# ktncktnc/diffusion-forcing-transformer

Hardware: AMD Instinct MI355X
Metric: denoised latent frames/sec, DFoT RE10K 8f & 200f rollout @1/2/4/8 GPU (higher is better)
Workload: dtype bf16

## Files before the change

diffusion-forcing-transformer_amd/backbone.py:

```python
from __future__ import annotations

import ctypes as C
import math
from typing import Dict, Optional, Sequence, Tuple

import torch
from torch import nn

from . import capi, ops


def _get(cfg, key, default=None):
    if isinstance(cfg, dict):
        return cfg.get(key, default)
    return getattr(cfg, key, default) if not hasattr(cfg, "get") else cfg.get(key, default)


class _Node(nn.Module):
    """Anonymous container so that dotted reference key names map onto a module tree."""


class UViT3DPose(nn.Module):
    def __init__(self, cfg, x_shape: Sequence[int], max_tokens: int, external_cond_dim: int = 0,
                 external_cond_type: str = "action", external_cond_num_classes: Optional[int] = None,
                 use_causal_mask: bool = False, **kwargs):
        super().__init__()
        block_types = list(_get(cfg, "block_types", ["ResBlock", "ResBlock", "TransformerBlock", "TransformerBlock"]))
        if block_types != ["ResBlock", "ResBlock", "TransformerBlock", "TransformerBlock"]:
            raise ValueError(f"unsupported block_types {block_types}")
        if _get(cfg, "pos_emb_type", "rope") != "rope":
            raise ValueError("only pos_emb_type='rope' is supported")
        if not _get(cfg, "use_fourier_noise_embedding", True):
            raise ValueError("only the Fourier noise-level embedding (continuous diffusion) is supported")
        cond = _get(cfg, "conditioning", None)
        cond_dim = _get(cond, "dim", None) if cond is not None else None
        self.cfg = cfg
        self.x_shape = tuple(x_shape)
        self.max_tokens = self.temporal_length = int(max_tokens)
        self.external_cond_dim = int(cond_dim or 180)
        self.use_causal_mask = use_causal_mask
        c = capi.UViTConfig()
        c.channels[:] = list(_get(cfg, "channels"))
        c.emb_channels = int(_get(cfg, "emb_channels"))
        c.num_updown_blocks[:] = list(_get(cfg, "num_updown_blocks"))
        c.num_mid_blocks = int(_get(cfg, "num_mid_blocks"))
        c.num_heads = int(_get(cfg, "num_heads"))
        c.in_channels = int(self.x_shape[0])
        c.resolution = int(self.x_shape[-1])
        c.max_tokens = self.max_tokens
        c.cond_dim = self.external_cond_dim
        c.noise_dim = 256
        c.rope_theta = 10000.0
        c.eps = 1e-6
        if int(_get(cfg, "patch_size", 2)) != 2:
            raise ValueError("only patch_size=2 is supported")
        self._ccfg = c
        self._handle = C.c_void_p()
        capi.check(capi.lib.dfot_uvit_create(C.byref(c), C.byref(self._handle)))
        self._names = []
        self._persistent_buffers = {"noise_level_pos_embedding.timesteps.freqs",
                                    "noise_level_pos_embedding.timesteps.phases"}
        shape = (C.c_int64 * 4)()
        ndim = C.c_int()
        for i in range(capi.lib.dfot_uvit_num_params(self._handle)):
            name = capi.lib.dfot_uvit_param_name(self._handle, i).decode()
            capi.check(capi.lib.dfot_uvit_param_shape(self._handle, i, shape, C.byref(ndim)))
            self._register(name, tuple(shape[k] for k in range(ndim.value)))
            self._names.append(name)
        self._synced: Optional[Tuple] = None
        self._reserved = 0
        self._op_key: Optional[int] = None
        self._cond_key = None
        self._cond_refs = None
        self._cond_gen = None
        self._cond_flag = None
        self.cond_cache_stats = {"builds": 0, "identity_hits": 0, "content_hits": 0}
        self._train_names = None
        self._trainer = None
        self._trainer_sig = None
        self.live_frames = None
        self.fresh_frames = None
        self._fresh_key = None
        self._train_stamp = 0
        self._dropout_generator: Optional[torch.Generator] = None

    def _register(self, name: str, shape: Tuple[int, ...]) -> None:
        *path, leaf = name.split(".")
        node: nn.Module = self
        for part in path:
            if part not in node._modules:
                node.add_module(part, _Node())
            node = node._modules[part]
        t = torch.zeros(shape, dtype=torch.float32)
        if name in self._persistent_buffers:
            node.register_buffer(leaf, t, persistent=True)
        else:
            node.register_parameter(leaf, nn.Parameter(t))

    def _tensors(self) -> Dict[str, torch.Tensor]:
        sd = dict(self.named_parameters())
        sd.update(dict(self.named_buffers()))
        return sd

    def reset_parameters(self, seed: int = 0) -> None:
        g = torch.Generator().manual_seed(seed)
        with torch.no_grad():
            for name, t in self._tensors().items():
                leaf = name.rsplit(".", 1)[-1]
                if leaf == "freqs":
                    t.copy_(2 * math.pi * torch.randn(t.shape, generator=g))
                elif leaf == "phases":
                    t.copy_(2 * math.pi * torch.rand(t.shape, generator=g))
                elif any(s in name for s in (".attn_out.", ".mlp_out.2.", ".out_rest.1.", "project_output")):
                    t.zero_()
                elif leaf == "bias":
                    t.zero_()
                elif t.ndim == 1:
                    t.fill_(1.0)
                else:
                    fan_in = math.prod(t.shape[1:])
                    bound = 1.0 / math.sqrt(fan_in)
                    t.copy_((torch.rand(t.shape, generator=g) * 2 - 1) * bound)

    def _signature(self) -> Tuple:
        return tuple((t.data_ptr(), t._version) for t in self._tensors().values())

    def sync_weights(self, force: bool = False) -> None:
        sig = self._signature()
        if not force and sig == self._synced:
            return
        tensors = self._tensors()
        s = capi.stream_ptr()
        for name in self._names:
            t = tensors[name]
            if not t.is_cuda:
                raise RuntimeError(f"parameter {name} is on {t.device}; move the module to the GPU first")
            src = t.detach().to(torch.float32).contiguous()
            shape = (C.c_int64 * src.ndim)(*src.shape)
            capi.check(capi.lib.dfot_uvit_load_weight(self._handle, name.encode(), capi.ptr(src), shape, src.ndim, s))
        capi.check(capi.lib.dfot_uvit_finalize(self._handle, s))
        self._synced = sig
        self.reserve_generation = getattr(self, "reserve_generation", 0) + 1

    def set_option(self, key: str, value: int) -> None:
        self.reserve_generation = getattr(self, "reserve_generation", 0) + 1
        capi.check(capi.lib.dfot_uvit_set_option(self._handle, key.encode(), int(value)))

    def query(self, key: str) -> float:
        self.sync_weights()
        val = C.c_double()
        capi.check(capi.lib.dfot_uvit_query(self._handle, key.encode(), C.byref(val)))
        return float(val.value)

    def attn_timing(self):
        tot, n = C.c_double(), C.c_int64()
        capi.check(capi.lib.dfot_uvit_attn_timing(self._handle, C.byref(tot), C.byref(n)))
        return tot.value, n.value

    def init_random(self, seed: int = 0, zero_init_scale: float = 0.3) -> None:
        g = torch.Generator().manual_seed(seed)
        with torch.no_grad():
            for name, t in self._tensors().items():
                leaf = name.rsplit(".", 1)[-1]
                if leaf == "freqs":
                    v = 2 * math.pi * torch.randn(t.shape, generator=g)
                elif leaf == "phases":
                    v = 2 * math.pi * torch.rand(t.shape, generator=g)
                elif leaf == "bias":
                    v = 0.02 * torch.randn(t.shape, generator=g)
                elif t.ndim == 1:
                    v = 1.0 + 0.1 * torch.randn(t.shape, generator=g)
                else:
                    fan_in = t.shape[0] if name.startswith("project_output") else math.prod(t.shape[1:])
                    v = torch.randn(t.shape, generator=g) / math.sqrt(fan_in)
                    if any(s in name for s in (".attn_out.", ".mlp_out.2.", ".out_rest.1.", "project_output")):
                        v = v * zero_init_scale
                t.copy_(v.to(t.device))

    def reserve(self, batch: int) -> None:
        if batch > self._reserved:
            torch.cuda.synchronize()
            capi.check(capi.lib.dfot_uvit_reserve(self._handle, int(batch)))
            self._reserved = batch
            self.reserve_generation = getattr(self, "reserve_generation", 0) + 1
            self._cond_key = None

    def forward(self, x: torch.Tensor, noise_levels: torch.Tensor, external_cond: Optional[torch.Tensor] = None,
                external_cond_mask: Optional[torch.Tensor] = None) -> torch.Tensor:
        assert external_cond is not None, "External condition (camera pose) is required for U-ViT3DPose model."
        if self._op_key is None:
            self._op_key = ops.register_model(self)
        if torch.is_grad_enabled() and (x.requires_grad or any(p.requires_grad for p in self.parameters())):
            if self._train_names is None:
                self._train_names = [n for n, _ in self.named_parameters()]
            params = [p for _, p in self.named_parameters()]
            return torch.ops.dfot.uvit3d_pose_forward_train(x, noise_levels, external_cond, external_cond_mask, params, self._op_key)
        return torch.ops.dfot.uvit3d_pose_forward(x, noise_levels, external_cond, external_cond_mask, self._op_key)

    def _train_engine(self, params):
        from . import uvit_train
        sig = tuple((t.data_ptr(), t._version) for t in params) + tuple((b.data_ptr(), b._version) for _, b in self.named_buffers())
        if self._trainer is None:
            cfg = dict(channels=list(self._ccfg.channels), emb_channels=int(self._ccfg.emb_channels), patch_size=2,
                       block_types=["ResBlock", "ResBlock", "TransformerBlock", "TransformerBlock"],
                       num_updown_blocks=list(self._ccfg.num_updown_blocks), num_mid_blocks=int(self._ccfg.num_mid_blocks),
                       num_heads=int(self._ccfg.num_heads), in_channels=int(self._ccfg.in_channels), resolution=int(self._ccfg.resolution),
                       max_tokens=self.max_tokens, cond_dim=self.external_cond_dim, noise_dim=int(self._ccfg.noise_dim),
                       eps=float(self._ccfg.eps), rope_theta=float(self._ccfg.rope_theta),
                       block_dropouts=list(_get(self.cfg, "block_dropouts", [0.0] * 4) or [0.0] * 4))
            sd = {n: t for n, t in zip(self._train_names, params)}
            sd.update(dict(self.named_buffers()))
            ordered = {n: sd[n] for n in self._names}
            self._trainer = uvit_train.UViT3DPoseTrainer(ordered, cfg)
            self._trainer_sig = sig
        elif sig != self._trainer_sig:
            with torch.no_grad():
                for n, t in zip(self._train_names, params):
                    self._trainer.p[n].copy_(t)
                for n, b in self.named_buffers():
                    self._trainer.p[n].copy_(b)
            self._trainer.sync()
            self._trainer_sig = sig
        return self._trainer

    def _train_forward_impl(self, x, noise_levels, external_cond, external_cond_mask, params):
        assert x.shape[1] == self.temporal_length, (
            f"Temporal length of U-ViT is set to {self.temporal_length}, but input has temporal length {x.shape[1]}.")
        dev = params[0].device
        if dev.type != "cuda":
            raise RuntimeError(f"the backbone's parameters are on {dev}; move the module to the GPU first (there is no CPU path)")
        capi.require_device(dev, x=x, noise_levels=noise_levels, external_cond=external_cond, external_cond_mask=external_cond_mask)
        eng = self._train_engine(params)
        drop = external_cond_mask
        pdrop = float(_get(self.cfg, "external_cond_dropout", 0.0) or 0.0)
        if drop is None and self.training and pdrop > 0:
            drop = torch.rand(x.shape[0], device=dev) < pdrop
        eng.dropout_generator = self._dropout_generator if self.training else None
        self._train_stamp += 1
        with torch.no_grad():
            return eng.forward(x, noise_levels, external_cond, drop).to(x.dtype)

    def _train_backward_impl(self, grad_out, params, stamp=None, want_dx=False):
        eng = self._trainer
        if eng is None:
            raise RuntimeError("backward without a training forward")
        if stamp is not None and stamp != self._train_stamp:
            raise RuntimeError(
                f"UViT3DPose: backward of training forward #{stamp}, but forward #{self._train_stamp} has run since and overwritten the "
                "saved activations (one engine per module). Run backward after each forward (accumulate gradients as forward/backward "
                "pairs); two forwards of one module inside one loss are not supported.")
        with torch.no_grad():
            grads = eng.backward(grad_out, input_grad=want_dx)
        out = [grads[n].to(p.dtype).reshape(p.shape) if n in grads else torch.zeros_like(p) for n, p in zip(self._train_names, params)]
        if want_dx:
            out.append(eng.dx_in.to(grad_out.dtype))
        return out

    def _cond_content_equal(self, cond: torch.Tensor, mask: Optional[torch.Tensor]) -> bool:
        if self._cond_key is None or self._cond_refs is None:
            return False
        kept, kept_mask = self._cond_refs
        _, version, shape, synced, mask_key = self._cond_key
        if synced != self._synced or self._cond_gen != self.reserve_generation:
            return False
        if kept._version != version or (kept_mask is not None and kept_mask._version != mask_key[1]):
            return False
        for t in (cond, kept):
            if t.dtype != torch.float32 or not t.is_contiguous():
                return False
        if cond.device != kept.device or tuple(cond.shape) != shape:
            return False
        if (mask is None) != (kept_mask is None):
            return False
        if mask is not None and (mask.dtype != kept_mask.dtype or mask.shape != kept_mask.shape or mask.device != kept_mask.device
                                 or not mask.is_contiguous() or not kept_mask.is_contiguous()):
            return False
        if torch.cuda.is_current_stream_capturing():
            return False
        if self._cond_flag is None or self._cond_flag.device != cond.device:
            self._cond_flag = torch.zeros(1, dtype=torch.int32, device=cond.device)
        flag = self._cond_flag
        flag.zero_()
        s = capi.stream_ptr()
        capi.check(capi.lib.dfot_op_equal_bits(capi.ptr(kept), capi.ptr(cond), cond.numel() * cond.element_size(), capi.ptr(flag), s))
        if mask is not None:
            capi.check(capi.lib.dfot_op_equal_bits(capi.ptr(kept_mask), capi.ptr(mask), mask.numel() * mask.element_size(), capi.ptr(flag), s))
        return int(flag.item()) == 0

    def _forward_impl(self, x: torch.Tensor, noise_levels: torch.Tensor, external_cond: Optional[torch.Tensor] = None,
                      external_cond_mask: Optional[torch.Tensor] = None) -> torch.Tensor:
        assert x.shape[1] == self.temporal_length, (
            f"Temporal length of U-ViT is set to {self.temporal_length}, but input has temporal length {x.shape[1]}.")
        assert external_cond is not None, "External condition (camera pose) is required for U-ViT3DPose model."
        b = x.shape[0]
        if tuple(x.shape[2:]) != self.x_shape:
            raise ValueError(f"x has frame shape {tuple(x.shape[2:])}, expected {self.x_shape}")
        if tuple(external_cond.shape) != (b, self.temporal_length, self.external_cond_dim, *self.x_shape[1:]):
            raise ValueError(f"external_cond has shape {tuple(external_cond.shape)}")
        if external_cond_mask is not None:
            assert external_cond_mask.ndim == 1, "embedding mask should be of shape (B,)"
        if tuple(noise_levels.shape) != (b, self.temporal_length):
            raise ValueError(f"noise_levels has shape {tuple(noise_levels.shape)}, expected {(b, self.temporal_length)}")
        dev = next(self.parameters()).device
        if dev.type != "cuda":
            raise RuntimeError(f"the backbone's parameters are on {dev}; move the module to the GPU first (there is no CPU path)")
        capi.require_device(dev, x=x, noise_levels=noise_levels, external_cond=external_cond, external_cond_mask=external_cond_mask)
        self.sync_weights()
        self.reserve(b)
        xf = x.detach().to(torch.float32).contiguous()
        kf = noise_levels.detach().to(torch.float32).contiguous()
        key = (external_cond.data_ptr(), external_cond._version, tuple(external_cond.shape), self._synced,
               None if external_cond_mask is None else (external_cond_mask.data_ptr(), external_cond_mask._version))
        if key == self._cond_key:
            self.cond_cache_stats["identity_hits"] += 1
        else:
            if self._cond_content_equal(external_cond, external_cond_mask):
                self.cond_cache_stats["content_hits"] += 1
            else:
                cf = external_cond.detach().to(torch.float32).contiguous()
                mf = None if external_cond_mask is None else external_cond_mask.to(torch.uint8).contiguous()
                capi.check(capi.lib.dfot_uvit_set_conditions(self._handle, capi.ptr(cf, torch.float32, "external_cond"),
                                                             capi.ptr(mf, torch.uint8, "external_cond_mask"), b, capi.stream_ptr()))
                self.cond_cache_stats["builds"] += 1
            self._cond_key = key
            self._cond_refs = (external_cond, external_cond_mask)
            self._cond_gen = self.reserve_generation
        out = torch.empty_like(xf)
        live = self.live_frames
        if live is not None:
            if tuple(live.shape) != (b, self.temporal_length) or live.dtype != torch.uint8 or not live.is_contiguous():
                raise ValueError(f"live_frames must be a contiguous uint8 tensor of shape {(b, self.temporal_length)}")
            capi.require_device(dev, live_frames=live)
        fresh = self.fresh_frames
        if fresh is not None:
            if tuple(fresh.shape) != (b, self.temporal_length) or fresh.dtype != torch.uint8 or not fresh.is_contiguous():
                raise ValueError(f"fresh_frames must be a contiguous uint8 tensor of shape {(b, self.temporal_length)}")
            capi.require_device(dev, fresh_frames=fresh)
            if key != self._fresh_key:
                fresh = None
        capi.check(capi.lib.dfot_uvit_forward_cached_masks(self._handle, capi.ptr(xf, torch.float32, "x"),
                                                           capi.ptr(kf, torch.float32, "noise_levels"), capi.ptr(out), b,
                                                           capi.ptr(live, torch.uint8, "live_frames"),
                                                           capi.ptr(fresh, torch.uint8, "fresh_frames"), capi.stream_ptr()))
        self._fresh_key = key
        return out.to(x.dtype)

    def read_tap(self, name: str, channels: int, level: int, batch: int) -> torch.Tensor:
        r = self.x_shape[-1] // 2 // (2 ** level)
        out = torch.empty(batch * self.temporal_length, channels, r, r, device="cuda", dtype=torch.float32)
        capi.check(capi.lib.dfot_uvit_read_tap(self._handle, name.encode(), capi.ptr(out), out.numel(), capi.stream_ptr()))
        return out

    def __del__(self):
        try:
            if getattr(self, "_handle", None) and self._handle.value:
                capi.lib.dfot_uvit_destroy(self._handle)
                self._handle = C.c_void_p()
        except Exception:
            pass
```

diffusion-forcing-transformer_amd/capi.py:

```python
from __future__ import annotations

import ctypes as C
import os

_HERE = os.path.dirname(os.path.abspath(__file__))
LIB_PATH = os.environ.get("DFOT_LIB", os.path.join(_HERE, "libdfot_hip.so"))

OK, ERR_ARG, ERR_SHAPE, ERR_HIP, ERR_STATE, ERR_NAME = range(6)


class DfotError(RuntimeError):
    def __init__(self, code: int, message: str):
        super().__init__(f"libdfot_hip error {code}: {message}")
        self.code = code


class UViTConfig(C.Structure):
    _fields_ = [
        ("channels", C.c_int32 * 4), ("emb_channels", C.c_int32), ("num_updown_blocks", C.c_int32 * 3),
        ("num_mid_blocks", C.c_int32), ("num_heads", C.c_int32), ("in_channels", C.c_int32),
        ("resolution", C.c_int32), ("max_tokens", C.c_int32), ("cond_dim", C.c_int32), ("noise_dim", C.c_int32),
        ("rope_theta", C.c_float), ("eps", C.c_float),
    ]


class DiTConfig(C.Structure):
    _fields_ = [
        ("hidden_size", C.c_int32), ("depth", C.c_int32), ("num_heads", C.c_int32), ("patch_size", C.c_int32),
        ("in_channels", C.c_int32), ("height", C.c_int32), ("width", C.c_int32), ("max_tokens", C.c_int32),
        ("mlp_hidden", C.c_int32), ("noise_dim", C.c_int32), ("timesteps", C.c_int32),
        ("rope_theta", C.c_float), ("eps", C.c_float),
        ("variant", C.c_int32), ("embed_col_dim", C.c_int32), ("num_col_heads", C.c_int32), ("num_row_heads", C.c_int32),
        ("temporal_mlp_hidden", C.c_int32), ("use_bias", C.c_int32),
        ("cond_type", C.c_int32), ("cond_dim", C.c_int32), ("num_classes", C.c_int32), ("cond_dropout", C.c_int32),
        ("use_temporal_rope", C.c_int32),
    ]


class DiTConfigF(DiTConfig):
    _fields_ = [("fourier_noise", C.c_int32)]


COND_NONE, COND_ACTION, COND_LABEL = 0, 1, 2


_P, _I, _L, _F = C.c_void_p, C.c_int, C.c_int64, C.c_float
_I32 = C.c_int32


class GemmDesc(C.Structure):
    _fields_ = [
        ("amode", _I32), ("epi", _I32), ("variant", _I32),
        ("A", _P), ("lda", _L), ("W", _P), ("ldw", _L),
        ("M", _I32), ("N", _I32), ("K", _I32), ("H", _I32), ("Wd", _I32), ("Cin", _I32),
        ("live", _P), ("bias", _P), ("bias_rows", _I32),
        ("out_f32", _P), ("out_bf16", _P), ("ldo", _L),
        ("resid", _P), ("resid_bf", _P),
        ("gate", _P), ("gate_index", _P), ("ldg", _L), ("gate_rows", _I32),
        ("act", _I32), ("pre_act", _P), ("raw", _P), ("ldraw", _L), ("tr_rows", _I32),
        ("gn_part", _P), ("gn_rows_per_bt", _I32), ("gn_cpg", _I32),
        ("out2", _P), ("ldo2", _L), ("split", _I32),
        ("q", _P), ("k", _P), ("v", _P),
        ("qw", _P), ("kw", _P), ("rope_cs", _P),
        ("heads", _I32), ("d", _I32), ("ntok", _I32), ("qscale", _F), ("dstride", _I32), ("eps", _F),
        ("ksplit", _I32), ("slice_stride", _L),
    ]


SIGNATURES = {
    "dfot_last_error": (C.c_char_p, []),
    "dfot_version": (_I, []),
    "dfot_uvit_create": (_I, [C.POINTER(UViTConfig), C.POINTER(_P)]),
    "dfot_uvit_destroy": (_I, [_P]),
    "dfot_uvit_num_params": (_I, [_P]),
    "dfot_uvit_param_name": (C.c_char_p, [_P, _I]),
    "dfot_uvit_param_shape": (_I, [_P, _I, C.POINTER(_L), C.POINTER(_I)]),
    "dfot_uvit_load_weight": (_I, [_P, C.c_char_p, _P, C.POINTER(_L), _I, _P]),
    "dfot_uvit_finalize": (_I, [_P, _P]),
    "dfot_uvit_reserve": (_I, [_P, _I]),
    "dfot_uvit_workspace_bytes": (C.c_size_t, [_P]),
    "dfot_uvit_set_option": (_I, [_P, C.c_char_p, _I]),
    "dfot_uvit_query": (_I, [_P, C.c_char_p, C.POINTER(C.c_double)]),
    "dfot_uvit_attn_timing": (_I, [_P, C.POINTER(C.c_double), C.POINTER(_L)]),
    "dfot_uvit_forward": (_I, [_P, _P, _P, _P, _P, _P, _I, _P]),
    "dfot_uvit_set_conditions": (_I, [_P, _P, _P, _I, _P]),
    "dfot_uvit_forward_cached": (_I, [_P, _P, _P, _P, _I, _P]),
    "dfot_uvit_forward_cached_live": (_I, [_P, _P, _P, _P, _I, _P, _P]),
    "dfot_uvit_forward_cached_masks": (_I, [_P, _P, _P, _P, _I, _P, _P, _P]),
    "dfot_uvit_read_tap": (_I, [_P, C.c_char_p, _P, C.c_size_t, _P]),
    "dfot_dit_create": (_I, [C.POINTER(DiTConfig), C.POINTER(_P)]),
    "dfot_dit_create_f": (_I, [C.POINTER(DiTConfigF), C.POINTER(_P)]),
    "dfot_dit_destroy": (_I, [_P]),
    "dfot_dit_num_params": (_I, [_P]),
    "dfot_dit_param_name": (C.c_char_p, [_P, _I]),
    "dfot_dit_param_shape": (_I, [_P, _I, C.POINTER(_L), C.POINTER(_I)]),
    "dfot_dit_load_weight": (_I, [_P, C.c_char_p, _P, C.POINTER(_L), _I, _P]),
    "dfot_dit_finalize": (_I, [_P, _P]),
    "dfot_dit_reserve": (_I, [_P, _I]),
    "dfot_dit_workspace_bytes": (C.c_size_t, [_P]),
    "dfot_dit_set_option": (_I, [_P, C.c_char_p, _I]),
    "dfot_dit_attn_timing": (_I, [_P, C.POINTER(C.c_double), C.POINTER(_L)]),
    "dfot_dit_forward": (_I, [_P, _P, _P, _P, _I, _I, _P]),
    "dfot_dit_forward_cond": (_I, [_P, _P, _P, _P, _P, _P, _P, _I, _I, _P]),
    "dfot_dit_forward_f": (_I, [_P, _P, _P, _P, _P, _P, _P, _I, _I, _P]),
    "dfot_dit_read_tap": (_I, [_P, C.c_char_p, _P, C.c_size_t, _P]),
    "dfot_dit_train_create": (_I, [C.POINTER(DiTConfig), C.POINTER(_P)]),
    "dfot_dit_train_create_f": (_I, [C.POINTER(DiTConfigF), C.POINTER(_P)]),
    "dfot_dit_train_destroy": (_I, [_P]),
    "dfot_dit_train_num_params": (_I, [_P]),
    "dfot_dit_train_param_name": (C.c_char_p, [_P, _I]),
    "dfot_dit_train_param_shape": (_I, [_P, _I, C.POINTER(_L), C.POINTER(_I)]),
    "dfot_dit_train_param_offset": (_L, [_P, _I]),
    "dfot_dit_train_total_numel": (_L, [_P]),
    "dfot_dit_train_workspace_bytes": (C.c_size_t, [_P]),
    "dfot_dit_train_attach": (_I, [_P, _P, _P]),
    "dfot_dit_train_reserve": (_I, [_P, _I]),
    "dfot_dit_train_sync_weights": (_I, [_P, _P]),
    "dfot_dit_train_forward": (_I, [_P, _P, _P, _P, _I, _I, _P]),
    "dfot_dit_train_forward_cond": (_I, [_P, _P, _P, _P, _P, _P, _P, _I, _I, _P]),
    "dfot_dit_train_load_buffer": (_I, [_P, C.c_char_p, _P, _L, _P]),
    "dfot_dit_train_forward_f": (_I, [_P, _P, _P, _P, _P, _P, _P, _I, _I, _P]),
    "dfot_dit_train_input_grad": (_I, [_P, _P, _P]),
    "dfot_dit_train_backward": (_I, [_P, _P, _P]),
    "dfot_vloss_grad": (_I, [_P] * 7 + [_I, _I, _L, _I, _P]),
    "dfot_sumsq": (_I, [_P, _L, _P, _P]),
    "dfot_adamw_step": (_I, [_P, _P, _P, _P, _L, _F, _F, _F, _F, _F, _I, _P, _F, _P, _F, _P]),
    "dfot_ray_encode": (_I, [_P, _P, _I, _I, _I, _P]),
    "dfot_ray_encode_normalized": (_I, [_P, _P, _I, _I, _I, _P]),
    "dfot_hg_prepare": (_I, [_P, _P, _P, _P, _P, _I, _I, _I, _L, _P]),
    "dfot_ddim_compose": (_I, [_P] * 11 + [_I, _I, _I, _L, _P]),
    "dfot_ddim_compose_tokw": (_I, [_P] * 11 + [_I, _I, _I, _L, _P]),
    "dfot_ddim_noise": (_I, [_P] * 5 + [_I, _I, _I, _L, _I, _P]),
    "dfot_vpred_loss": (_I, [_P] * 9 + [_I, _I, _L, _P]),
    "dfot_vpred_loss_scratch_floats": (_L, [_I, _I, _L]),
    "dfot_vspace_loss": (_I, [_P] * 9 + [_I, _I, _L, _P]),
    "dfot_op_gemm": (_I, [_P, _I, _P, _P, _P, _I, _I, _I, _I, _P]),
    "dfot_op_conv3x3": (_I, [_P, _P, _P, _P, _I, _I, _I, _I, _I, _I, _P]),
    "dfot_op_gemm_ex": (_I, [C.POINTER(GemmDesc), _P]),
    "dfot_op_gemm_desc_bytes": (_L, []),
    "dfot_op_attention": (_I, [_P, _P, _P, _P, _I, _I, _I, _I, _I, _I, _P]),
    "dfot_op_attention_padded": (_I, [_P, _P, _P, _P, _I, _I, _I, _I, _I, _P]),
    "dfot_op_attention_temporal": (_I, [_P, _P, _P, _P, _I, _I, _I, _I, _I, _I, _P]),
    "dfot_op_matrix_attention_rope": (_I, [_P, _P, _P, _I, _I, _I, _I, _I, _I, _F, _P]),
    "dfot_op_matrix_attention": (_I, [_P, _P, _I, _I, _I, _I, _I, _I, _F, _P]),
    "dfot_op_attention_bwd": (_I, [_P, _P, _P, _P, _P, _I, _P, _P, _P, _I, _I, _I, _I, _P]),
    "dfot_op_conv3x3_bwd": (_I, [_P, _P, _P, _P, _P, _P, _I, _I, _I, _I, _I, _P]),
    "dfot_op_conv3x3_bwd2": (_I, [_P, _P, _P, _P, _P, _P, _P, _I, _I, _I, _I, _I, _P]),
    "dfot_op_gn_silu_bwd": (_I, [_P, _P, _P, _P, _P, _F, _P, _P, _P, _P, _I, _I, _I, _P]),
    "dfot_op_rms_film_bwd": (_I, [_P, _P, _P, _P, _F, _P, _P, _P, _L, _I, _I, _P]),
    "dfot_op_rms_film_bwd_res": (_I, [_P, _P, _P, _P, _F, _P, _P, _P, _P, _P, _L, _I, _P]),
    "dfot_op_qknorm_rope_bwd": (_I, [_P, _I, _P, _P, _P, _P, _P, _P, _F, _P, _I, _P, _P, _L, _I, _I, _I, _P]),
    "dfot_op_wgrad_nt": (_I, [_P, _I, _P, _I, _P, _I, _I, _L, _I, _P]),
    "dfot_op_gemm_bf16": (_I, [_P, _I, _P, _P, _P, _I, _I, _I, _I, _P]),
    "dfot_op_gemm_f32": (_I, [_P, _I, _P, _P, _P, _P, _I, _I, _I, _I, _P]),
    "dfot_op_transpose_bf16": (_I, [_P, _P, _I, _I, _P]),
    "dfot_op_colsum_bf16": (_I, [_P, _I, _P, _L, _I, _P]),
    "dfot_op_rms_film_fwd": (_I, [_P, _P, _P, _F, _P, _L, _I, _P]),
    "dfot_op_qknorm_rope_fwd": (_I, [_P, _I, _P, _P, _P, _F, _F, _P, _P, _P, _L, _I, _I, _I, _P]),
    "dfot_op_fused_proj_train": (_I, [_P, _I, _P, _P, _P, _P, _P, _F, _F, _P, _P, _P, _P, _P, _I, _I, _L, _I, _I, _I, _P]),
    "dfot_op_silu_cols": (_I, [_P, _I, _I, _P, _I, _I, _P, _I, _I, _L, _I, _P]),
    "dfot_op_attention_fwd_lse": (_I, [_P, _P, _P, _P, _I, _P, _I, _I, _I, _I, _P]),
    "dfot_op_attention_fwd_lse_bounded": (_I, [_P, _P, _P, _P, _I, _P, _I, _I, _I, _I, C.c_float, _P, C.c_size_t, _P]),
    "dfot_op_attention_scratch_bytes": (C.c_size_t, [_I, _I, _I, _I]),
    "dfot_op_attention_bwd_lse": (_I, [_P, _P, _P, _P, _P, _I, _P, _P, _P, _P, _P, _I, _I, _I, _I, _P]),
    "dfot_op_gn_silu_fwd": (_I, [_P, _P, _P, _P, _F, _P, _P, _I, _I, _I, _P]),
    "dfot_op_gn_silu_bwd5": (_I, [_P, _P, _P, _P, _P, _P, _P, _P, _P, _P, _L, _P, _P, _I, _I, _I, _P]),
    "dfot_op_gn_silu_fwd2": (_I, [_P, _P, _P, _P, _L, _F, _P, _P, _I, _I, _I, _P]),
    "dfot_op_gn_silu_bwd6": (_I, [_P, _P, _P, _P, _P, _P, _L, _P, _P, _P, _P, _L, _P, _P, _I, _I, _I, _P]),
    "dfot_op_gemm_bf16_frame_bias": (_I, [_P, _I, _P, _P, _I, _P, _I, _I, _I, _I, _P]),
    "dfot_op_split_bf16": (_I, [_P, _P, _P, _L, _P]),
    "dfot_op_frame_sums_bf16": (_I, [_P, _L, _P, _I, _I, _I, _P]),
    "dfot_op_sgemm": (_I, [_P, _L, _L, _P, _L, _L, _P, _L, _I, _I, _I, _I, _P]),
    "dfot_op_pack_conv3": (_I, [_P, _P, _I, _I, _I, _P]),
    "dfot_op_conv3x3_f32": (_I, [_P, _P, _P, _P, _P, _I, _I, _I, _I, _I, _P]),
    "dfot_op_pool2_bf16": (_I, [_P, _P, _I, _I, _I, _I, _P]),
    "dfot_op_pool2_bwd": (_I, [_P, _P, _I, _I, _I, _I, _P]),
    "dfot_op_sub_bf16": (_I, [_P, _P, _P, _L, _P]),
    "dfot_op_upsample_add": (_I, [_P, _P, _P, _I, _I, _I, _I, _P]),
    "dfot_op_upsample_bwd": (_I, [_P, _P, _I, _I, _I, _I, _P]),
    "dfot_op_axpy": (_I, [_P, _P, _F, _L, _P]),
    "dfot_op_mul_cols": (_I, [_P, _I, _I, _P, _L, _I, _P]),
    "dfot_op_emb_pyramid": (_I, [_P, _P, _P, _P, _I, _I, _I, _P]),
    "dfot_op_cond_repack": (_I, [_P, _P, _I, _I, _I, _I, _P]),
    "dfot_op_embed_input": (_I, [_P, _P, _P, _P, _I, _I, _I, _I, _P]),
    "dfot_op_embed_input_wgrad": (_I, [_P, _P, _P, _P, _I, _I, _I, _I, _I, _P]),
    "dfot_op_embed_input_dgrad": (_I, [_P, _P, _P, _I, _I, _I, _I, _I, _P]),
    "dfot_op_project_output": (_I, [_P, _P, _P, _P, _I, _I, _I, _I, _P]),
    "dfot_op_outgrad_gather": (_I, [_P, _P, _I, _I, _I, _I, _P]),
    "dfot_op_groupnorm_scratch_floats": (_L, [_I, _I]),
    "dfot_op_groupnorm": (_I, [_P, _P, _P, _F, _P, _P, _I, _I, _I, _I, _P]),
    "dfot_op_frame_shift": (_I, [_P, _P, _I, _I, _L, _I, _P]),
    "dfot_op_upsample3d": (_I, [_P, _P, _I, _I, _I, _I, _I, _I, _P]),
    "dfot_op_softmax_rows": (_I, [_P, _P, _L, _I, _F, _P]),
    "dfot_op_conv3t_f32": (_I, [_P, _P, _P, _P, _P] + [_I] * 9 + [_P]),
    "dfot_op_vae_pixels": (_I, [_P, _L, _L, _L, _L, _L, _F, _F, _P, _I, _I, _I, _I, _P]),
    "dfot_op_vae_posterior": (_I, [_P, _I, _P, _P, _P, _P, _P, _P, _P, _I, _I, _I, _I, _P]),
    "dfot_op_ivae_attention": (_I, [_P, _P, _P, _P, _I, _I, _I, _P]),
    "dfot_op_conv3x3_s2_f32": (_I, [_P, _P, _P, _P] + [_I] * 5 + [_P]),
    "dfot_op_upconv3x3_f32": (_I, [_P, _P, _P, _P] + [_I] * 5 + [_P]),
    "dfot_op_f32_to_bf16": (_I, [_P, _P, _L, _P]),
    "dfot_op_bf16_to_f32": (_I, [_P, _P, _L, _P]),
    "dfot_op_equal_bits": (_I, [_P, _P, _L, _P, _P]),
}


def _load() -> C.CDLL:
    import torch
    if not os.path.exists(LIB_PATH):
        raise ImportError(
            f"{LIB_PATH} is missing: the HIP extension has not been built. There is no CPU fallback; "
            "run `python -c 'import __graft_entry__ as g; g.build()'` (needs hipcc).")
    lib = C.CDLL(LIB_PATH)
    for name, (res, args) in SIGNATURES.items():
        fn = getattr(lib, name)
        fn.restype, fn.argtypes = res, args
    return lib


lib = _load()


def check(code: int) -> None:
    if code != OK:
        raise DfotError(code, (lib.dfot_last_error() or b"").decode())


def ptr(t, dtype=None, name: str = "tensor") -> C.c_void_p:
    if t is None:
        return C.c_void_p(0)
    if not t.is_cuda:
        raise ValueError(f"{name} is on {t.device}: libdfot_hip takes GPU memory only (there is no CPU path)")
    if not t.is_contiguous():
        raise ValueError(f"{name} with shape {tuple(t.shape)} and strides {tuple(t.stride())} is not contiguous")
    if dtype is not None and t.dtype != dtype:
        raise ValueError(f"{name} has dtype {t.dtype}, expected {dtype}")
    return C.c_void_p(t.data_ptr())


def ptr_rows(t, dtype=None, name: str = "tensor") -> C.c_void_p:
    if t is None:
        return C.c_void_p(0)
# ... 19 lines not shown
```

diffusion-forcing-transformer_amd/csrc/common.h:

```cpp
#pragma once
#include <hip/hip_runtime.h>
#include <stdint.h>
#include <stdio.h>

#include "dfot_hip.h"

namespace dfot {

typedef __bf16 bf16;
typedef __attribute__((ext_vector_type(8))) __bf16 bf16x8;
typedef __attribute__((ext_vector_type(4))) __bf16 bf16x4;
typedef __attribute__((ext_vector_type(2))) __bf16 bf16x2;
typedef __attribute__((ext_vector_type(4))) float f32x4;
typedef __attribute__((ext_vector_type(16))) float f32x16;
typedef __attribute__((ext_vector_type(2))) unsigned u32x2;

#define DFOT_LDS_PTR(p) ((void __attribute__((address_space(3)))*)(p))
#define DFOT_GLOBAL_PTR(p) ((const void __attribute__((address_space(1)))*)(p))

__device__ __forceinline__ int xcd_remap(int orig, int nwg, int enable = 1) {
  if (!enable) return orig;
  const int q = nwg >> 3, r = nwg & 7, xcd = orig & 7;
  return (xcd < r ? xcd * (q + 1) : r * (q + 1) + (xcd - r) * q) + (orig >> 3);
}

__device__ __forceinline__ float silu_f(float x) { return x * __builtin_amdgcn_rcpf(1.0f + __expf(-x)); }

__device__ __forceinline__ float bf2f(bf16 v) { return (float)v; }
__device__ __forceinline__ bf16 f2bf(float v) { return (bf16)v; }

template <int OFF>
__device__ __forceinline__ u32x2 lds_read_tr16(unsigned addr) {
  u32x2 r;
  asm volatile("ds_read_b64_tr_b16 %0, %1 offset:%2" : "=v"(r) : "v"(addr), "n"(OFF));
  return r;
}
__device__ __forceinline__ void lds_wait(u32x2& a, u32x2& b, u32x2& c, u32x2& d, u32x2& e, u32x2& f, u32x2& g, u32x2& h) {
  asm volatile("s_waitcnt lgkmcnt(0)" : "+v"(a), "+v"(b), "+v"(c), "+v"(d), "+v"(e), "+v"(f), "+v"(g), "+v"(h));
}
__device__ __forceinline__ bf16x8 as_bf16x8(u32x2 lo, u32x2 hi) {
  typedef __attribute__((ext_vector_type(4))) unsigned u32x4;
  const u32x4 v = {lo[0], lo[1], hi[0], hi[1]};
  return __builtin_bit_cast(bf16x8, v);
}

int tuning_flag(const char* name, int dflt);

void set_error(const char* fmt, ...);
const char* get_error();

#define DFOT_CHECK_HIP(expr)                                                              \
  do {                                                                                    \
    hipError_t _e = (expr);                                                               \
    if (_e != hipSuccess) {                                                               \
      ::dfot::set_error("%s failed: %s (%s:%d)", #expr, hipGetErrorString(_e), __FILE__, __LINE__); \
      return DFOT_ERR_HIP;                                                                \
    }                                                                                     \
  } while (0)

#define DFOT_REQUIRE(cond, code, ...)      \
  do {                                     \
    if (!(cond)) {                         \
      ::dfot::set_error(__VA_ARGS__);      \
      return code;                         \
    }                                      \
  } while (0)

static inline int cdiv(long a, long b) { return (int)((a + b - 1) / b); }

template <auto Kern>
int ensure_dyn_lds(int bytes) {
  static bool done = false;
  if (!done) {
    DFOT_CHECK_HIP(hipFuncSetAttribute(reinterpret_cast<const void*>(Kern), hipFuncAttributeMaxDynamicSharedMemorySize, bytes));
    done = true;
  }
  return DFOT_OK;
}

}
```

diffusion-forcing-transformer_amd/csrc/gemm.h:

```cpp
#pragma once
#include "common.h"

namespace dfot {

enum AMode { A_DENSE = 0, A_CONV3 = 1, A_CONV3T = 2 };
enum Epi { E_F32 = 0, E_BF16 = 1, E_QKV = 2, E_QKV_DIT = 3 };

struct GemmArgs {
  const bf16* A = nullptr;
  long lda = 0;
  const bf16* W = nullptr;
  long ldw = 0;
  int M = 0, N = 0, K = 0;
  int H = 0, Wd = 0, Cin = 0;
  const bf16* zeros = nullptr;
  const uint8_t* live = nullptr;
  int To = 0, Tin = 0, Hin = 0, Win = 0;
  int cs = 1, ct = 1, ckt = 1;
  const float* bias = nullptr;
  float* out_f32 = nullptr;
  bf16* out_bf16 = nullptr;
  long ldo = 0;
  const float* resid = nullptr;
  const bf16* resid_bf = nullptr;
  const float* gate = nullptr;
  const int* gate_index = nullptr;
  long ldg = 0;
  int gate_rows = 0;
  int act = 0;
  bf16* pre_act = nullptr;
  bf16* raw = nullptr;
  long ldraw = 0;
  int bias_rows = 0;
  int tr_rows = 0;
  float* gn_part = nullptr;
  int gn_rows_per_bt = 0;
  int gn_cpg = 0;
  bf16* out2 = nullptr;
  long ldo2 = 0;
  int split = 0;
  bf16 *q = nullptr, *k = nullptr, *v = nullptr;
  const float *qw = nullptr, *kw = nullptr, *rope_cs = nullptr;
  int heads = 0, d = 0, ntok = 0;
  float qscale = 1.f;
  int dstride = 0;
  float eps = 1e-6f;
  int xcd = 1;
  int persist = 0;
  int ksplit = 1;
  long slice_stride = 0;
};

enum GemmVariant {
  GEMM_REGS_128 = 0,
  GEMM_DMA_128 = 1,
  GEMM_DMA_256x256 = 4,
  GEMM_DMA_512x128 = 6,
  GEMM_DMA_128_KS2 = 8,
  GEMM_DMA_256x192 = 9,
  GEMM_DMA_128x192 = 10,
  GEMM_DMA3_256x144 = 14,
  GEMM_AUTO = -1
};
int gemm_pick_variant(int amode, int m, int n, int k, bool plain_f32 = false);
int launch_gemm(int amode, int epi, int variant, const GemmArgs& g, hipStream_t stream);

}
```

diffusion-forcing-transformer_amd/csrc/gemm.hip:

```cpp
#include "gemm.h"
#include "dfot_hip.h"

namespace dfot {

constexpr int BK = 64;
constexpr int wave_cols(int bn) { return bn % 64 == 0 ? 64 : 48; }
constexpr int tile_threads(int bm, int bn, int wtm, int ks) { return (bm / wtm) * (bn / wave_cols(bn)) * 64 * ks; }
constexpr int EP_LD = 68;

template <int N>
__device__ __forceinline__ void wait_all_but() {
  static_assert(N == 2 || N == 4 || N == 6 || N == 8 || N == 12, "unexpected load count");
  if constexpr (N == 2) asm volatile("s_waitcnt vmcnt(2)\n\ts_barrier" ::: "memory");
  if constexpr (N == 4) asm volatile("s_waitcnt vmcnt(4)\n\ts_barrier" ::: "memory");
  if constexpr (N == 6) asm volatile("s_waitcnt vmcnt(6)\n\ts_barrier" ::: "memory");
  if constexpr (N == 8) asm volatile("s_waitcnt vmcnt(8)\n\ts_barrier" ::: "memory");
  if constexpr (N == 12) asm volatile("s_waitcnt vmcnt(12)\n\ts_barrier" ::: "memory");
}

__device__ __forceinline__ void wait_all_but_n(int n) {
  switch (n) {
    case 1: asm volatile("s_waitcnt vmcnt(1)\n\ts_barrier" ::: "memory"); break;
    case 2: asm volatile("s_waitcnt vmcnt(2)\n\ts_barrier" ::: "memory"); break;
    case 3: asm volatile("s_waitcnt vmcnt(3)\n\ts_barrier" ::: "memory"); break;
    case 4: asm volatile("s_waitcnt vmcnt(4)\n\ts_barrier" ::: "memory"); break;
    case 5: asm volatile("s_waitcnt vmcnt(5)\n\ts_barrier" ::: "memory"); break;
    case 6: asm volatile("s_waitcnt vmcnt(6)\n\ts_barrier" ::: "memory"); break;
    case 7: asm volatile("s_waitcnt vmcnt(7)\n\ts_barrier" ::: "memory"); break;
    case 8: asm volatile("s_waitcnt vmcnt(8)\n\ts_barrier" ::: "memory"); break;
    default: asm volatile("s_waitcnt vmcnt(0)\n\ts_barrier" ::: "memory"); break;
  }
}

template <int BM_T, int BN_T, int WTM, int NST, int AMODE, int EPI, bool DMA, int KS, int BKT>
__device__ __forceinline__ void gemm_tile(const GemmArgs& g, const int tile_index, const int tile_count) {
  static_assert(BKT == 64 || (BKT == 32 && AMODE == A_DENSE && DMA && KS == 1), "K-tile depth");
  constexpr int CPR = BKT / 8;
  constexpr int RPI = 64 / CPR;
  constexpr int ROWB = BKT * 2;
  constexpr int MI = WTM / 16;
  constexpr int WTN = wave_cols(BN_T);
  constexpr int NI = WTN / 16;
  constexpr int WN = BN_T / WTN;
  static_assert(WTN == 64 || (EPI == E_F32 || EPI == E_BF16), "48-column wave tiles: plain epilogues only");
  static_assert(WTN == 64 || KS == 1, "48-column wave tiles: no intra-workgroup split-K");
  constexpr int NW = (BM_T / WTM) * WN;
  constexpr int NT = NW * 64;
  constexpr int AINS = BM_T / RPI, WINS = BN_T / RPI;
  constexpr int ACH = (AINS + NW - 1) / NW;
  constexpr int WCH = (WINS + NW - 1) / NW;
  constexpr bool A_EVEN = AINS % NW == 0, W_EVEN = WINS % NW == 0;
  static_assert((A_EVEN && W_EVEN) || (DMA && KS == 1), "uneven staging: LDS-DMA kernels without intra-workgroup split-K only");
  constexpr int A_BYTES = BM_T * BKT * 2;
  constexpr int STAGE_BYTES = (BM_T + BN_T) * BKT * 2;
  constexpr int LOADS = ACH + WCH;
  static_assert(DMA || NST == 2, "register staging supports two stages only");
  static_assert(KS == 1 || (NST == 2 && DMA && EPI != E_QKV), "split-K: two-stage LDS-DMA kernels without in-epilogue barriers");
  extern __shared__ __attribute__((aligned(16))) char smem_all[];
  const int tid = threadIdx.x, lane = tid & 63;
  const int kgroup = KS == 1 ? 0 : (tid >> 6) / NW;
  const int wave = KS == 1 ? (tid >> 6) : (tid >> 6) % NW;
  char* smem = smem_all + kgroup * (NST * STAGE_BYTES);
  const int wm = wave / WN, wn = wave % WN;
  const int tiles_n = (g.N + BN_T - 1) / BN_T;
  const int ksplit = (EPI == E_F32 && (AMODE == A_DENSE || g.slice_stride > 0) && g.ksplit > 1) ? g.ksplit : 1;
  const int kslice = ksplit > 1 ? tile_index % ksplit : 0;
  const int bid = ksplit > 1 ? xcd_remap(tile_index / ksplit, tile_count / ksplit, g.xcd) : xcd_remap(tile_index, tile_count, g.xcd);
  const int tn = bid % tiles_n, tm = bid / tiles_n;
  const int m0 = tm * BM_T, n0 = tn * BN_T;
  if constexpr (AMODE == A_CONV3) {
    if (g.live && !g.live[(unsigned)m0 / (unsigned)(g.H * g.Wd)]) return;
  }
  int nk = g.K / BKT;
  long kbeg = 0;
  if (ksplit > 1) {
    const int per = nk / ksplit, rem = nk % ksplit;
    kbeg = (long)(kslice * per + (kslice < rem ? kslice : rem)) * BKT;
    nk = per + (kslice < rem ? 1 : 0);
  }
  auto swz = [](int r) { return BKT == 64 ? ((r >> 1) & 7) : ((r >> 2) & 2); };

  const int prow = lane / CPR;
  const int ppos = lane % CPR;
  const bf16* a_src[ACH];
  int a_y[ACH], a_x[ACH];
  [[maybe_unused]] int a_t[ACH];
  const bf16* w_src[WCH];
  int a_chunk[ACH];
#pragma unroll
  for (int i = 0; i < ACH; ++i) {
    const int r = RPI * (NW * i + wave) + prow;
    const int c = ppos ^ swz(r);
    a_chunk[i] = c;
    const long m = (long)m0 + r;
    if constexpr (AMODE == A_DENSE) {
      a_src[i] = g.A + m * g.lda + c * 8 + kbeg;
      a_y[i] = a_x[i] = 0;
    } else if constexpr (AMODE == A_CONV3) {
      const unsigned mu = (unsigned)m;
      const int xw = (int)(mu % (unsigned)g.Wd);
      const int yh = (int)((mu / (unsigned)g.Wd) % (unsigned)g.H);
      a_x[i] = xw;
      a_y[i] = yh;
      a_src[i] = g.A + m * (long)g.Cin + c * 8;
    } else {
      unsigned mu = (unsigned)m;
      const int xo = (int)(mu % (unsigned)g.Wd);
      mu /= (unsigned)g.Wd;
      const int yo = (int)(mu % (unsigned)g.H);
      mu /= (unsigned)g.H;
      const int to = (int)(mu % (unsigned)g.To);
      const unsigned bv = mu / (unsigned)g.To;
      const int pad = g.cs == 1 ? 1 : 0;
      a_x[i] = g.cs * xo - pad;
      a_y[i] = g.cs * yo - pad;
      a_t[i] = g.ct * to - (g.ckt - 1);
      a_src[i] = g.A + (long)bv * ((long)g.Tin * g.Hin * g.Win * g.Cin) + c * 8;
    }
  }
#pragma unroll
  for (int i = 0; i < WCH; ++i) {
    const int r = RPI * (NW * i + wave) + prow;
    const int c = ppos ^ swz(r);
    int n = n0 + r;
    n = n < g.N ? n : g.N - 1;
    w_src[i] = g.W + (long)n * (AMODE == A_DENSE && g.ldw ? g.ldw : (long)g.K) + c * 8 + kbeg;
  }

  [[maybe_unused]] int cv_c0 = 0, cv_dy = -1, cv_dx = -1, cv_dt = 0;
  if constexpr (AMODE == A_CONV3) {
    const int kbase = kgroup * BKT + (int)kbeg;
    const int tap = kbase / g.Cin;
    cv_c0 = kbase - tap * g.Cin;
    cv_dy = tap / 3 - 1;
    cv_dx = tap % 3 - 1;
  } else if constexpr (AMODE == A_CONV3T) {
    const int kbase = kgroup * BKT + (int)kbeg;
    const int tap = kbase / g.Cin;
    cv_c0 = kbase - tap * g.Cin;
    cv_dt = tap / 9;
    cv_dy = (tap % 9) / 3;
    cv_dx = tap % 3;
  }
  auto a_addr = [&](int i, int kt) -> const bf16* {
    if constexpr (AMODE == A_DENSE) {
      return a_src[i] + (long)kt * BKT;
    } else if constexpr (AMODE == A_CONV3) {
      const int yy = a_y[i] + cv_dy, xx = a_x[i] + cv_dx;
      const bool ok = (yy >= 0) && (yy < g.H) && (xx >= 0) && (xx < g.Wd);
      const bf16* p = a_src[i] + ((long)cv_dy * g.Wd + cv_dx) * g.Cin + cv_c0;
      return ok ? p : g.zeros + a_chunk[i] * 8;
    } else {
      int tt = a_t[i] + cv_dt;
      tt = tt < 0 ? 0 : tt;
      const int yy = a_y[i] + cv_dy, xx = a_x[i] + cv_dx;
      const bool ok = (yy >= 0) && (yy < g.Hin) && (xx >= 0) && (xx < g.Win);
      const bf16* p = a_src[i] + ((long)(tt * g.Hin + yy) * g.Win + xx) * g.Cin + cv_c0;
      return ok ? p : g.zeros + a_chunk[i] * 8;
    }
  };
  auto conv_advance = [&]() {
    if constexpr (AMODE == A_CONV3) {
      cv_c0 += KS * BKT;
      while (cv_c0 >= g.Cin) {
        cv_c0 -= g.Cin;
        if (++cv_dx > 1) {
          cv_dx = -1;
          ++cv_dy;
        }
      }
    } else if constexpr (AMODE == A_CONV3T) {
      cv_c0 += KS * BKT;
      while (cv_c0 >= g.Cin) {
        cv_c0 -= g.Cin;
        if (++cv_dx > 2) {
          cv_dx = 0;
          if (++cv_dy > 2) {
            cv_dy = 0;
            ++cv_dt;
          }
        }
      }
    }
  };

  bf16x8 ra[ACH], rw[WCH];

  auto issue = [&](int kt, int stage) {
    char* sa = smem + stage * STAGE_BYTES;
    char* sw = sa + A_BYTES;
#pragma unroll
    for (int i = 0; i < ACH; ++i) {
      if (!A_EVEN && NW * i + wave >= AINS) continue;
      const bf16* pa = a_addr(i, kt);
      if constexpr (DMA) {
        __builtin_amdgcn_global_load_lds(DFOT_GLOBAL_PTR(pa), DFOT_LDS_PTR(sa + (NW * i + wave) * 1024), 16, 0, 0);
      } else {
        ra[i] = *reinterpret_cast<const bf16x8*>(pa);
      }
    }
#pragma unroll
    for (int i = 0; i < WCH; ++i) {
      if (!W_EVEN && NW * i + wave >= WINS) continue;
      const bf16* pw = w_src[i] + (long)kt * BKT;
      if constexpr (DMA) {
        __builtin_amdgcn_global_load_lds(DFOT_GLOBAL_PTR(pw), DFOT_LDS_PTR(sw + (NW * i + wave) * 1024), 16, 0, 0);
      } else {
        rw[i] = *reinterpret_cast<const bf16x8*>(pw);
      }
    }
    conv_advance();
  };
  auto commit = [&](int stage) {
    char* sa = smem + stage * STAGE_BYTES;
    char* sw = sa + A_BYTES;
#pragma unroll
    for (int i = 0; i < ACH; ++i) *reinterpret_cast<bf16x8*>(sa + (NW * i + wave) * 1024 + lane * 16) = ra[i];
#pragma unroll
    for (int i = 0; i < WCH; ++i) *reinterpret_cast<bf16x8*>(sw + (NW * i + wave) * 1024 + lane * 16) = rw[i];
  };
// ... 486 lines not shown
      if constexpr (EPI == E_F32) {
        if (g.gn_cpg == 8) {
          gsum += __shfl_xor(gsum, 1);
          gsq += __shfl_xor(gsq, 1);
        }
        gsum += __shfl_xor(gsum, 16);
        gsq += __shfl_xor(gsq, 16);
        gsum += __shfl_xor(gsum, 32);
        gsq += __shfl_xor(gsq, 32);
        if (lane < 16 && live && (g.gn_cpg == 4 || (lane & 1) == 0)) {
          const int grp = col / g.gn_cpg;
          dst[grp * 2] = gsum;
          dst[grp * 2 + 1] = gsq;
        }
      } else {
        if (g.gn_cpg == 8) {
          gsum += gsum2;
          gsq += gsq2;
        }
#pragma unroll
        for (int o = 8; o < 64; o <<= 1) {
          gsum += __shfl_xor(gsum, o);
          gsq += __shfl_xor(gsq, o);
          gsum2 += __shfl_xor(gsum2, o);
          gsq2 += __shfl_xor(gsq2, o);
        }
        if (lane < 8 && live) {
          const int grp = col / g.gn_cpg;
          dst[grp * 2] = gsum;
          dst[grp * 2 + 1] = gsq;
          if (g.gn_cpg == 4) {
            dst[grp * 2 + 2] = gsum2;
            dst[grp * 2 + 3] = gsq2;
          }
        }
      }
    }
  }
}

template <int BM_T, int BN_T, int WTM, int NST, int AMODE, int EPI, bool DMA, int KS = 1, int BKT = BK>
__global__ __launch_bounds__(tile_threads(BM_T, BN_T, WTM, KS)) void gemm_kernel(GemmArgs g) {
  gemm_tile<BM_T, BN_T, WTM, NST, AMODE, EPI, DMA, KS, BKT>(g, blockIdx.x, gridDim.x);
}

template <int BM_T, int BN_T, int WTM, int NST, int AMODE, int EPI, bool DMA, int KS = 1, int BKT = BK>
__global__ __launch_bounds__(tile_threads(BM_T, BN_T, WTM, KS)) void gemm_kernel_persistent(GemmArgs g, int tile_count) {
  for (int tile = blockIdx.x; tile < tile_count; tile += gridDim.x) {
    gemm_tile<BM_T, BN_T, WTM, NST, AMODE, EPI, DMA, KS, BKT>(g, tile, tile_count);
    if (tile + (int)gridDim.x < tile_count) __syncthreads();
  }
}

template <int BM_T, int BN_T, int WTM, int NST, int AMODE, int EPI, bool DMA, int KS = 1, int BKT = BK>
static int launch_t(const GemmArgs& g, hipStream_t stream) {
  constexpr int nthreads = tile_threads(BM_T, BN_T, WTM, KS);
  constexpr int stage_lds = KS * NST * (BM_T + BN_T) * BKT * 2;
  constexpr int ep_lds = (nthreads / 64) * 16 * EP_LD * 4 + 2 * (nthreads / 64) * 16 * 4 +
                         (KS == 2 ? (nthreads / 128) * (WTM / 16) * 16 * 64 * 4 : 0);
  constexpr int lds = stage_lds > ep_lds ? stage_lds : ep_lds;
  const int ksplit = (EPI == E_F32 && (AMODE == A_DENSE || g.slice_stride > 0) && g.ksplit > 1) ? g.ksplit : 1;
  const int tiles = (g.M / BM_T) * ((g.N + BN_T - 1) / BN_T) * ksplit;
  GemmArgs ga = g;
  ga.xcd = 1;
  ga.persist = 1;
  constexpr bool kPersistOK = KS == 1 && nthreads <= 768;
  if constexpr (kPersistOK) {
    if (ga.persist > 0 && ksplit == 1) {
      const int resident = 256 * (lds <= 80 * 1024 ? 2 : 1);
      if (tiles > resident) {
        auto kp = gemm_kernel_persistent<BM_T, BN_T, WTM, NST, AMODE, EPI, DMA, KS, BKT>;
        static bool pattr_set = false;
        if (!pattr_set) {
          DFOT_CHECK_HIP(hipFuncSetAttribute(reinterpret_cast<const void*>(kp), hipFuncAttributeMaxDynamicSharedMemorySize, lds));
          pattr_set = true;
        }
        hipLaunchKernelGGL(kp, dim3(resident), dim3(nthreads), lds, stream, ga, tiles);
        DFOT_CHECK_HIP(hipGetLastError());
        return DFOT_OK;
      }
    }
  }
  auto kern = gemm_kernel<BM_T, BN_T, WTM, NST, AMODE, EPI, DMA, KS, BKT>;
  static bool attr_set = false;
  if (!attr_set) {
    DFOT_CHECK_HIP(hipFuncSetAttribute(reinterpret_cast<const void*>(kern), hipFuncAttributeMaxDynamicSharedMemorySize, lds));
    attr_set = true;
  }
  hipLaunchKernelGGL(kern, dim3(tiles), dim3(nthreads), lds, stream, ga);
  DFOT_CHECK_HIP(hipGetLastError());
  return DFOT_OK;
}

template <int AMODE, int EPI>
static int launch_v(int variant, const GemmArgs& g, hipStream_t s) {
  switch (variant) {
    case GEMM_REGS_128:
      if constexpr (AMODE == A_CONV3T) break;
      else return launch_t<128, 128, 64, 2, AMODE, EPI, false>(g, s);
    case GEMM_DMA_128: return launch_t<128, 128, 64, 2, AMODE, EPI, true>(g, s);
    case GEMM_DMA_256x256: return launch_t<256, 256, 64, 2, AMODE, EPI, true>(g, s);
    case GEMM_DMA_512x128: return launch_t<512, 128, 64, 2, AMODE, EPI, true>(g, s);
    case GEMM_DMA_256x192:
      if constexpr (AMODE != A_DENSE) break;
      else return launch_t<256, 192, 64, 2, AMODE, EPI, true>(g, s);
    case GEMM_DMA3_256x144:
      if constexpr ((EPI != E_F32 && !(EPI == E_BF16 && AMODE == A_DENSE)) || AMODE == A_CONV3T) break;
      else {
        if (g.gn_part) break;
        return launch_t<256, 144, 64, 3, AMODE, EPI, true>(g, s);
      }
    case GEMM_DMA_128x192:
      if constexpr (AMODE != A_DENSE || EPI == E_QKV) break;
      else return launch_t<128, 192, 64, 2, AMODE, EPI, true>(g, s);
    case GEMM_DMA_128_KS2:
      if constexpr (EPI == E_QKV) break;
      else return launch_t<128, 128, 64, 2, AMODE, EPI, true, 2>(g, s);
  }
  set_error("gemm: unknown variant %d", variant);
  return DFOT_ERR_ARG;
}

int gemm_pick_variant(int amode, int m, int n, int k, bool plain_f32) {
  const long tiles = (long)(m / 256) * ((n + 255) / 256);
  if (m % 256 == 0 && n >= 192 && amode == A_DENSE) {
    auto util = [&](int bn) {
      const long t = (long)(m / 256) * ((n + bn - 1) / bn);
      return (double)m * n / ((double)((t + 255) / 256) * 256 * 256 * bn);
    };
    if (plain_f32 && n % 144 == 0 && k >= 2304 && (long)(m / 256) * (n / 144) >= 256 && util(144) > 1.1 * util(192) && util(144) > 1.1 * util(256))
      return GEMM_DMA3_256x144;
    if (util(192) > 1.05 * util(256) && (long)(m / 256) * ((n + 191) / 192) >= 160) return GEMM_DMA_256x192;
  }
  if (m % 256 == 0 && n >= 192 && tiles >= 160) return GEMM_DMA_256x256;
  if (m % 512 == 0 && n <= 128 && m / 512 >= 256) return GEMM_DMA_512x128;
  const long tiles128 = (long)(m / 128) * ((n + 127) / 128);
  if (tiles128 <= 256 && k >= 2048) return GEMM_DMA_128_KS2;
  return GEMM_DMA_128;
}

int launch_gemm(int amode, int epi, int variant, const GemmArgs& g, hipStream_t stream) {
  DFOT_REQUIRE(g.A && g.W, DFOT_ERR_ARG, "gemm: null operand");
  if (variant == GEMM_AUTO) variant = gemm_pick_variant(amode, g.M, g.N, g.K, epi == E_F32 && !g.gn_part);
  if (variant == GEMM_DMA_128_KS2 && epi == E_QKV) variant = GEMM_DMA_128;
  if (variant == GEMM_DMA_128x192 && epi == E_QKV) variant = GEMM_DMA_128;
  if (variant == GEMM_DMA_256x192 && epi == E_QKV && g.d != 64) variant = GEMM_DMA_256x256;
  const int bm = variant == GEMM_DMA_512x128 ? 512 : (variant == GEMM_DMA_256x256 || variant == GEMM_DMA_256x192 || variant == GEMM_DMA3_256x144) ? 256 : 128;
  DFOT_REQUIRE(g.M > 0 && g.M % bm == 0, DFOT_ERR_SHAPE, "gemm: M=%d must be a positive multiple of %d", g.M, bm);
  DFOT_REQUIRE(g.K > 0 && g.K % BK == 0, DFOT_ERR_SHAPE, "gemm: K=%d must be a positive multiple of %d", g.K, BK);
  DFOT_REQUIRE(g.N > 0 && g.N % (epi == E_F32 ? 4 : 8) == 0, DFOT_ERR_SHAPE, "gemm: N=%d must be a multiple of %d", g.N, epi == E_F32 ? 4 : 8);
  DFOT_REQUIRE((epi == E_QKV || epi == E_QKV_DIT || g.ldo % (epi == E_F32 ? 4 : 8) == 0) && (epi != E_QKV || (g.ldo2 % 8 == 0 && g.split % 64 == 0)),
               DFOT_ERR_SHAPE, "gemm: output row strides must be multiples of %d", epi == E_F32 ? 4 : 8);
  DFOT_REQUIRE(g.ldw == 0 || (amode == A_DENSE && g.ldw >= g.K && g.ldw % 8 == 0), DFOT_ERR_SHAPE, "gemm: ldw=%ld must be >= K and a multiple of 8 (dense A only)", g.ldw);
  if (amode == A_CONV3) {
    DFOT_REQUIRE(g.Cin % BK == 0 && g.K == 9 * g.Cin, DFOT_ERR_SHAPE, "conv3x3: Cin=%d must be a multiple of %d", g.Cin, BK);
    DFOT_REQUIRE(g.zeros != nullptr, DFOT_ERR_ARG, "conv3x3: zero page missing");
    DFOT_REQUIRE(g.H > 0 && g.Wd > 0 && g.M % (g.H * g.Wd) == 0, DFOT_ERR_SHAPE, "conv3x3: M=%d not a whole number of %dx%d images", g.M, g.H, g.Wd);
    DFOT_REQUIRE(!g.live || (g.H * g.Wd) % bm == 0, DFOT_ERR_SHAPE, "conv3x3: live-image flags need whole %d-row tiles per %dx%d image", bm, g.H, g.Wd);
  }
  if (amode == A_CONV3T) {
    DFOT_REQUIRE(epi == E_F32 && g.ksplit <= 1 && !g.live && !g.gate && !g.bias_rows, DFOT_ERR_ARG, "conv3t: plain fp32 epilogue only");
    DFOT_REQUIRE(g.Cin % BK == 0 && (g.ckt == 1 || g.ckt == 3) && g.K == g.ckt * 9 * g.Cin && (g.cs == 1 || g.cs == 2) && (g.ct == 1 || g.ct == 2),
                 DFOT_ERR_SHAPE, "conv3t: Cin=%d (multiple of %d), kt=%d in {1,3}, K=%d = kt*9*Cin, strides s=%d t=%d in {1,2}", g.Cin, BK, g.ckt, g.K,
                 g.cs, g.ct);
    DFOT_REQUIRE(g.zeros != nullptr, DFOT_ERR_ARG, "conv3t: zero page missing");
    DFOT_REQUIRE(g.H > 0 && g.Wd > 0 && g.To > 0 && g.Hin == g.cs * g.H && g.Win == g.cs * g.Wd && g.Tin >= 1 && g.ct * (g.To - 1) <= g.Tin - 1 &&
                     g.To == (g.Tin - 1) / g.ct + 1,
                 DFOT_ERR_SHAPE, "conv3t: input %dx%dx%d, output %dx%dx%d do not match strides s=%d t=%d", g.Tin, g.Hin, g.Win, g.To, g.H, g.Wd, g.cs, g.ct);
    DFOT_REQUIRE(g.M % (g.To * g.H * g.Wd) == 0, DFOT_ERR_SHAPE, "conv3t: M=%d not a whole number of %dx%dx%d videos", g.M, g.To, g.H, g.Wd);
    DFOT_REQUIRE((long)g.Tin * g.Hin * g.Win * g.Cin < (1L << 31), DFOT_ERR_SHAPE, "conv3t: one input video must hold < 2^31 elements");
  }
  if (epi == E_QKV) {
    DFOT_REQUIRE(g.q && g.k && g.v && g.qw && g.kw && g.rope_cs && (g.out2 || g.N == g.split), DFOT_ERR_ARG, "qkv epilogue: null pointer");
    DFOT_REQUIRE(!g.raw || (g.ldraw >= g.N && g.ldraw % 8 == 0), DFOT_ERR_SHAPE, "qkv epilogue: raw copy needs ldraw >= N, a multiple of 8");
    DFOT_REQUIRE((g.d == 64 || g.d == 128) && g.heads > 0 && g.split == 3 * g.heads * g.d && g.ntok > 0 && g.M % g.ntok == 0,
                 DFOT_ERR_SHAPE, "qkv epilogue: heads=%d d=%d split=%d ntok=%d M=%d", g.heads, g.d, g.split, g.ntok, g.M);
  }
  if (epi == E_QKV_DIT) {
    DFOT_REQUIRE(g.q && g.k && g.v, DFOT_ERR_ARG, "dit qkv epilogue: null pointer");
    DFOT_REQUIRE(g.d > 0 && g.d % 8 == 0 && g.dstride >= g.d && g.dstride % 8 == 0 && g.heads > 0 && g.N == 3 * g.heads * g.d &&
                     g.ntok > 0 && g.M % g.ntok == 0,
                 DFOT_ERR_SHAPE, "dit qkv epilogue: heads=%d d=%d dstride=%d ntok=%d M=%d N=%d", g.heads, g.d, g.dstride, g.ntok, g.M, g.N);
  }
  if (g.gate) {
    DFOT_REQUIRE(epi == E_F32 && g.gate_rows > 0 && g.M % g.gate_rows == 0 && g.ldg % 4 == 0, DFOT_ERR_SHAPE,
                 "gemm: gate needs the fp32 epilogue, gate_rows dividing M and ldg %% 4 == 0");
  }
  if (g.ksplit > 1 && g.slice_stride > 0)
    DFOT_REQUIRE(!g.bias && !g.resid, DFOT_ERR_ARG, "gemm: split-K into partial outputs takes no bias / residual");
  if (g.ksplit > 1)
    DFOT_REQUIRE(epi == E_F32 && (amode == A_DENSE || g.slice_stride > 0) && !g.bias_rows && (!g.resid || g.resid == g.out_f32) && !g.gate &&
                     !g.gn_part && g.K / BK >= 2 * g.ksplit, DFOT_ERR_ARG,
                 "gemm: split-K over workgroups needs the fp32 epilogue with an in-place residual (or none), no gate, and K >= %d", 2 * g.ksplit * BK);
  if (g.bias_rows) DFOT_REQUIRE((epi == E_F32 || epi == E_BF16) && g.bias, DFOT_ERR_ARG, "gemm: 2-D bias needs a plain epilogue");
  if (g.resid_bf)
    DFOT_REQUIRE(epi == E_BF16 && (amode == A_CONV3 || variant == GEMM_DMA3_256x144) && !g.resid, DFOT_ERR_ARG,
                 "gemm: a bf16 residual needs the bf16 epilogue of a convolution or of the 256x144 ring");
  if (g.tr_rows) {
    DFOT_REQUIRE(epi == E_BF16 && !g.bias && !g.act && !g.gn_part && g.tr_rows % 4 == 0 && g.M % g.tr_rows == 0 && amode == A_DENSE,
                 DFOT_ERR_ARG, "gemm: transposed store needs the plain bf16 epilogue and tr_rows %% 4 == 0 dividing M");
  }
  if (g.gn_part) {
    DFOT_REQUIRE(epi != E_QKV && epi != E_QKV_DIT && (g.gn_cpg == 4 || g.gn_cpg == 8) && g.N == 32 * g.gn_cpg && g.gn_rows_per_bt % 64 == 0 &&
                     g.gn_rows_per_bt % bm == 0,
                 DFOT_ERR_SHAPE, "gemm: fused GroupNorm statistics need N = 32 groups of 4 or 8 channels and whole images per tile");
  }
  if (amode == A_DENSE) {
    switch (epi) {
      case E_F32: return launch_v<A_DENSE, E_F32>(variant, g, stream);
      case E_BF16: return launch_v<A_DENSE, E_BF16>(variant, g, stream);
      case E_QKV: return launch_v<A_DENSE, E_QKV>(variant, g, stream);
      case E_QKV_DIT: return launch_v<A_DENSE, E_QKV_DIT>(variant, g, stream);
    }
  } else if (amode == A_CONV3) {
    switch (epi) {
      case E_F32: return launch_v<A_CONV3, E_F32>(variant, g, stream);
      case E_BF16: return launch_v<A_CONV3, E_BF16>(variant, g, stream);
    }
  } else if (amode == A_CONV3T && epi == E_F32) {
    return launch_v<A_CONV3T, E_F32>(variant, g, stream);
  }
  set_error("gemm: unsupported mode/epilogue combination %d/%d", amode, epi);
  return DFOT_ERR_ARG;
}

}
```

diffusion-forcing-transformer_amd/csrc/uvit.hip:

```cpp
#include <algorithm>
#include <cmath>
#include <cstdarg>
#include <cstdlib>
#include <cstring>
#include <functional>
#include <map>
#include <string>
#include <vector>

#include "dfot_hip.h"
#include "gemm.h"
#include "kernels.h"

namespace dfot {

static thread_local char g_err[1024] = "";
void set_error(const char* fmt, ...) {
  va_list ap;
  va_start(ap, fmt);
  vsnprintf(g_err, sizeof(g_err), fmt, ap);
  va_end(ap);
}
const char* get_error() { return g_err; }

int tuning_flag(const char* name, int dflt) {
  std::string key = std::string("DFOT_") + name;
  const char* v = getenv(key.c_str());
  return v ? atoi(v) : dflt;
}

struct ResW {
  int c = 0;
  bf16* fcache = nullptr;
  long sv_off = 0;
  bf16 *w_film = nullptr, *w1 = nullptr, *w2 = nullptr;
  float *b_film_raw = nullptr, *b_film = nullptr, *g1 = nullptr, *be1 = nullptr, *bias1 = nullptr, *g2 = nullptr,
        *be2 = nullptr, *bias2 = nullptr;
};
struct TrW {
  int c = 0;
  bf16* fcache = nullptr;
  long sv_off = 0;
  bf16 *w_film = nullptr, *w_fused = nullptr, *w_out = nullptr;
  float *b_film_raw = nullptr, *b_film = nullptr, *nw = nullptr, *b_fused = nullptr, *qw = nullptr, *kw = nullptr,
        *b_attn = nullptr, *b_mlp = nullptr, *b_out = nullptr;
  float score_bound = INFINITY;
};
struct ConvW {
  int cin = 0, cout = 0;
  bf16* w = nullptr;
  float* b = nullptr;
};

struct Param {
  std::string name;
  std::vector<int64_t> shape;
  std::function<int(const float*, hipStream_t)> load;
  bool loaded = false;
};

}

using namespace dfot;

struct dfot_uvit_s {
  dfot_uvit_config cfg{};
  int T = 0, E = 0, heads = 0, r[4] = {0, 0, 0, 0}, ch[4] = {0, 0, 0, 0};
  int kpose = 0;
  std::vector<Param> params;
  std::map<std::string, int> index;
  std::vector<void*> owned;

  float *ne_freqs = nullptr, *ne_phases = nullptr, *ne_w1 = nullptr, *ne_b1 = nullptr, *ne_w2 = nullptr, *ne_b2 = nullptr;
  bf16* pose_w = nullptr;
  float* pose_b = nullptr;
  float *ein_w = nullptr, *ein_b = nullptr, *pout_w = nullptr, *pout_b = nullptr;
  std::vector<ResW> down_res[2], up_res[2];
  std::vector<TrW> down_tr, mid_tr, up_tr;
  ConvW down_conv[3], up_conv[3];
  int* film_map[4] = {nullptr, nullptr, nullptr, nullptr};
  float* rope_cs[4] = {nullptr, nullptr, nullptr, nullptr};
  bf16* zeros = nullptr;
  bool finalized = false;

  int max_batch = 0;
  size_t ws_bytes = 0;
  std::vector<void*> ws_owned;
  float *nemb = nullptr, *nhid = nullptr, *X[4] = {nullptr, nullptr, nullptr, nullptr}, *HSA[3] = {nullptr, nullptr, nullptr}, *tmp = nullptr,
        *gn_partial = nullptr, *gn_partial2 = nullptr, *gn_stats = nullptr, *sv = nullptr;
  int gn1_nblk = 0;
  FilmChunk* film_table = nullptr;
  int film_chunks = 0;
  uint8_t* cond_mask = nullptr;
  bool have_mask = false;
  int cond_batch = 0;
  int64_t cond_builds = 0;
  bf16 *acond = nullptr, *emb[4] = {nullptr, nullptr, nullptr, nullptr}, *s1 = nullptr, *hbf = nullptr,
       *cat = nullptr, *q = nullptr, *k = nullptr, *v = nullptr;
  AttnScratch attn_scratch;
  const float* pend_part = nullptr;
  float* out_part = nullptr;
  size_t out_part_elems = 0;
  const float* pend_bias = nullptr;
  int pend_lvl = 0, pend_c = 0, pend_slices = 2;
  long pend_m = 0;
  int last_batch = 0;
  const float* xin[4] = {nullptr, nullptr, nullptr, nullptr};
  bf16* XB[4] = {nullptr, nullptr, nullptr, nullptr};
  bool xin_bf[4] = {false, false, false, false};
  int gemm_variant = GEMM_AUTO;
  int attn_variant = 2;
  bool attn_force_safe = false;
  bool time_attn = false;
  std::vector<hipEvent_t> ev_start, ev_stop;
  size_t ev_used = 0;
};

namespace dfot {

template <typename T>
static int dev_alloc(dfot_uvit_s* h, T** out, size_t count, bool workspace = false) {
  void* p = nullptr;
  const size_t bytes = count * sizeof(T);
  DFOT_CHECK_HIP(hipMalloc(&p, bytes ? bytes : 16));
  (workspace ? h->ws_owned : h->owned).push_back(p);
  if (workspace) h->ws_bytes += bytes;
  *out = reinterpret_cast<T*>(p);
  return DFOT_OK;
}

static int copy_f32(float* dst, const float* src, size_t n, hipStream_t s) {
  DFOT_CHECK_HIP(hipMemcpyAsync(dst, src, n * sizeof(float), hipMemcpyDeviceToDevice, s));
  return DFOT_OK;
}

static void add_param(dfot_uvit_s* h, const std::string& name, std::vector<int64_t> shape,
                      std::function<int(const float*, hipStream_t)> load) {
  h->index[name] = (int)h->params.size();
  h->params.push_back(Param{name, std::move(shape), std::move(load), false});
}

static int add_f32(dfot_uvit_s* h, const std::string& name, std::vector<int64_t> shape, float** dst) {
  size_t n = 1;
  for (auto d : shape) n *= (size_t)d;
  int rc = dev_alloc(h, dst, n);
  if (rc) return rc;
  float* d = *dst;
  add_param(h, name, shape, [d, n](const float* src, hipStream_t s) { return copy_f32(d, src, n, s); });
  return DFOT_OK;
}

static int add_res_block(dfot_uvit_s* h, const std::string& pre, int c, ResW* w) {
  const int e = h->E;
  w->c = c;
  int rc = 0;
  if ((rc = dev_alloc(h, &w->w_film, (size_t)2 * c * e))) return rc;
  if ((rc = dev_alloc(h, &w->b_film_raw, (size_t)2 * c))) return rc;
  if ((rc = dev_alloc(h, &w->b_film, (size_t)2 * c))) return rc;
  if ((rc = dev_alloc(h, &w->w1, (size_t)c * 9 * c))) return rc;
  if ((rc = dev_alloc(h, &w->w2, (size_t)c * 9 * c))) return rc;
  const int lvl = c == h->ch[0] ? 0 : 1;
  int* map = h->film_map[lvl];
  bf16* wf = w->w_film;
  add_param(h, pre + ".emb_layer.weight", {2 * c, e, 1, 1}, [=](const float* src, hipStream_t s) {
    return launch_pack_rows(src, wf, map, 2 * c, e, e, e, 0, s);
  });
  float *braw = w->b_film_raw, *bre = w->b_film;
  add_param(h, pre + ".emb_layer.bias", {2 * c}, [=](const float* src, hipStream_t s) {
    int r2 = copy_f32(braw, src, 2 * c, s);
    return r2 ? r2 : launch_gather_f32(braw, bre, map, 2 * c, s);
  });
  if ((rc = add_f32(h, pre + ".in_layers.0.weight", {c}, &w->g1))) return rc;
  if ((rc = add_f32(h, pre + ".in_layers.0.bias", {c}, &w->be1))) return rc;
  bf16* w1 = w->w1;
  add_param(h, pre + ".in_layers.2.weight", {c, c, 3, 3}, [=](const float* src, hipStream_t s) { return launch_pack_conv3(src, w1, c, c, s); });
  if ((rc = add_f32(h, pre + ".in_layers.2.bias", {c}, &w->bias1))) return rc;
  if ((rc = add_f32(h, pre + ".out_norm.weight", {c}, &w->g2))) return rc;
  if ((rc = add_f32(h, pre + ".out_norm.bias", {c}, &w->be2))) return rc;
  bf16* w2 = w->w2;
  add_param(h, pre + ".out_rest.1.weight", {c, c, 3, 3}, [=](const float* src, hipStream_t s) { return launch_pack_conv3(src, w2, c, c, s); });
  if ((rc = add_f32(h, pre + ".out_rest.1.bias", {c}, &w->bias2))) return rc;
  return DFOT_OK;
}

static int add_tr_block(dfot_uvit_s* h, const std::string& pre, int lvl, TrW* w) {
  const int e = h->E, c = h->ch[lvl], d = c / h->heads;
  w->c = c;
  int rc = 0;
  if ((rc = dev_alloc(h, &w->w_film, (size_t)2 * c * e))) return rc;
  if ((rc = dev_alloc(h, &w->b_film_raw, (size_t)2 * c))) return rc;
  if ((rc = dev_alloc(h, &w->b_film, (size_t)2 * c))) return rc;
  if ((rc = dev_alloc(h, &w->w_fused, (size_t)7 * c * c))) return rc;
  if ((rc = dev_alloc(h, &w->w_out, (size_t)c * 5 * c))) return rc;
  if ((rc = dev_alloc(h, &w->b_out, (size_t)c))) return rc;
  int* map = h->film_map[lvl];
  bf16* wf = w->w_film;
  add_param(h, pre + ".norm.emb_layer.weight", {2 * c, e}, [=](const float* src, hipStream_t s) {
    return launch_pack_rows(src, wf, map, 2 * c, e, e, e, 0, s);
  });
  float *braw = w->b_film_raw, *bre = w->b_film;
  add_param(h, pre + ".norm.emb_layer.bias", {2 * c}, [=](const float* src, hipStream_t s) {
    int r2 = copy_f32(braw, src, 2 * c, s);
    return r2 ? r2 : launch_gather_f32(braw, bre, map, 2 * c, s);
  });
  if ((rc = add_f32(h, pre + ".norm.norm.weight", {c}, &w->nw))) return rc;
  bf16* wfu = w->w_fused;
  add_param(h, pre + ".fused_attn_mlp_proj.weight", {7 * c, c}, [=](const float* src, hipStream_t s) {
    return launch_pack_rows(src, wfu, nullptr, 7 * c, c, c, c, 0, s);
  });
  if ((rc = add_f32(h, pre + ".fused_attn_mlp_proj.bias", {7 * c}, &w->b_fused))) return rc;
  if ((rc = add_f32(h, pre + ".q_norm.weight", {d}, &w->qw))) return rc;
  if ((rc = add_f32(h, pre + ".k_norm.weight", {d}, &w->kw))) return rc;
  bf16* wo = w->w_out;
  add_param(h, pre + ".attn_out.weight", {c, c}, [=](const float* src, hipStream_t s) {
    return launch_pack_rows(src, wo, nullptr, c, c, c, 5 * c, 0, s);
  });
  if ((rc = add_f32(h, pre + ".attn_out.bias", {c}, &w->b_attn))) return rc;
  add_param(h, pre + ".mlp_out.2.weight", {c, 4 * c}, [=](const float* src, hipStream_t s) {
    return launch_pack_rows(src, wo, nullptr, c, 4 * c, 4 * c, 5 * c, c, s);
  });
  if ((rc = add_f32(h, pre + ".mlp_out.2.bias", {c}, &w->b_mlp))) return rc;
  return DFOT_OK;
}

static int add_conv(dfot_uvit_s* h, const std::string& pre, int cin, int cout, ConvW* w) {
  w->cin = cin;
  w->cout = cout;
  int rc = 0;
  if ((rc = dev_alloc(h, &w->w, (size_t)cout * 9 * cin))) return rc;
  bf16* dst = w->w;
  add_param(h, pre + ".weight", {cout, cin, 3, 3}, [=](const float* src, hipStream_t s) { return launch_pack_conv3(src, dst, cout, cin, s); });
  return add_f32(h, pre + ".bias", {cout}, &w->b);
}

static int build(dfot_uvit_s* h) {
  const dfot_uvit_config& c = h->cfg;
  h->T = c.max_tokens;
  h->E = c.emb_channels;
  h->heads = c.num_heads;
  for (int l = 0; l < 4; ++l) {
    h->ch[l] = c.channels[l];
    h->r[l] = c.resolution / 2 / (1 << l);
  }
  h->kpose = ((c.cond_dim * 4 + 63) / 64) * 64;
  int rc = 0;
  for (int l = 0; l < 4; ++l) {
    const int cc = h->ch[l];
    std::vector<int> m(2 * cc);
    for (int n = 0; n < 2 * cc; ++n) {
      const int g = n / 64, t = n % 64;
      m[n] = t < 32 ? 32 * g + t : cc + 32 * g + (t - 32);
    }
    if ((rc = dev_alloc(h, &h->film_map[l], (size_t)2 * cc))) return rc;
    DFOT_CHECK_HIP(hipMemcpy(h->film_map[l], m.data(), m.size() * sizeof(int), hipMemcpyHostToDevice));
  }
  if ((rc = dev_alloc(h, &h->zeros, 256))) return rc;
  DFOT_CHECK_HIP(hipMemset(h->zeros, 0, 256 * sizeof(bf16)));

  const int e = h->E, nd = c.noise_dim;
  const std::string ne = "noise_level_pos_embedding.";
  if ((rc = add_f32(h, ne + "timesteps.freqs", {nd}, &h->ne_freqs))) return rc;
  if ((rc = add_f32(h, ne + "timesteps.phases", {nd}, &h->ne_phases))) return rc;
  if ((rc = add_f32(h, ne + "embedding.linear_1.weight", {e, nd}, &h->ne_w1))) return rc;
  if ((rc = add_f32(h, ne + "embedding.linear_1.bias", {e}, &h->ne_b1))) return rc;
  if ((rc = add_f32(h, ne + "embedding.linear_2.weight", {e, e}, &h->ne_w2))) return rc;
  if ((rc = add_f32(h, ne + "embedding.linear_2.bias", {e}, &h->ne_b2))) return rc;
  if ((rc = dev_alloc(h, &h->pose_w, (size_t)e * h->kpose))) return rc;
  {
    bf16* pw = h->pose_w;
    const int k = c.cond_dim * 4, kp = h->kpose;
    add_param(h, "external_cond_embedding.patch_embedder.proj.weight", {e, c.cond_dim, 2, 2},
              [=](const float* src, hipStream_t s) { return launch_pack_rows(src, pw, nullptr, e, k, kp, kp, 0, s); });
  }
  if ((rc = add_f32(h, "external_cond_embedding.patch_embedder.proj.bias", {e}, &h->pose_b))) return rc;
  if ((rc = add_f32(h, "embed_input.proj.weight", {h->ch[0], c.in_channels, 2, 2}, &h->ein_w))) return rc;
  if ((rc = add_f32(h, "embed_input.proj.bias", {h->ch[0]}, &h->ein_b))) return rc;
  if ((rc = add_f32(h, "project_output.proj.weight", {h->ch[0], c.in_channels, 2, 2}, &h->pout_w))) return rc;
  if ((rc = add_f32(h, "project_output.proj.bias", {c.in_channels}, &h->pout_b))) return rc;

  for (int l = 0; l < 3; ++l) {
    const int n = c.num_updown_blocks[l];
    const std::string pre = "down_blocks." + std::to_string(l) + ".";
    if (l < 2) {
      h->down_res[l].resize(n);
      for (int i = 0; i < n; ++i)
        if ((rc = add_res_block(h, pre + std::to_string(i), h->ch[l], &h->down_res[l][i]))) return rc;
    } else {
      h->down_tr.resize(n);
      for (int i = 0; i < n; ++i)
        if ((rc = add_tr_block(h, pre + std::to_string(i), l, &h->down_tr[i]))) return rc;
    }
    if ((rc = add_conv(h, pre + std::to_string(n) + ".conv", h->ch[l], h->ch[l + 1], &h->down_conv[l]))) return rc;
  }
  h->mid_tr.resize(c.num_mid_blocks);
  for (int i = 0; i < c.num_mid_blocks; ++i)
    if ((rc = add_tr_block(h, "mid_blocks." + std::to_string(i), 3, &h->mid_tr[i]))) return rc;
  for (int j = 0; j < 3; ++j) {
    const int l = 2 - j;
    const int n = c.num_updown_blocks[l];
    const std::string pre = "up_blocks." + std::to_string(j) + ".";
    if ((rc = add_conv(h, pre + "0.conv", h->ch[l + 1], h->ch[l], &h->up_conv[l]))) return rc;
    if (l < 2) {
      h->up_res[l].resize(n);
      for (int i = 0; i < n; ++i)
        if ((rc = add_res_block(h, pre + std::to_string(i + 1), h->ch[l], &h->up_res[l][i]))) return rc;
    } else {
      h->up_tr.resize(n);
      for (int i = 0; i < n; ++i)
        if ((rc = add_tr_block(h, pre + std::to_string(i + 1), l, &h->up_tr[i]))) return rc;
    }
  }
  return DFOT_OK;
}

static int build_rope(dfot_uvit_s* h, int lvl) {
  const int d = h->ch[lvl] / h->heads, half = d / 2;
  const int q = half / 3, rem = half % 3;
  int parts[3] = {q, q, q};
  if (rem == 1) parts[0] = q + 1;
  if (rem == 2) parts[1] = parts[2] = q + 1;
  const int rr = h->r[lvl], n = h->T * rr * rr;
  std::vector<float> cs((size_t)n * half * 2);
  for (int tok = 0; tok < n; ++tok) {
    const int pos[3] = {tok / (rr * rr), (tok / rr) % rr, tok % rr};
    int pair = 0;
    for (int ax = 0; ax < 3; ++ax) {
      const int dim = 2 * parts[ax];
      for (int j = 0; j < parts[ax]; ++j, ++pair) {
        const float inv = 1.0f / powf(h->cfg.rope_theta, (float)(2 * j) / (float)dim);
        const float ang = (float)pos[ax] * inv;
        cs[((size_t)tok * half + pair) * 2 + 0] = cosf(ang);
        cs[((size_t)tok * half + pair) * 2 + 1] = sinf(ang);
      }
    }
  }
  int rc = dev_alloc(h, &h->rope_cs[lvl], cs.size());
  if (rc) return rc;
  DFOT_CHECK_HIP(hipMemcpy(h->rope_cs[lvl], cs.data(), cs.size() * sizeof(float), hipMemcpyHostToDevice));
  return DFOT_OK;
}

__global__ void add_vec_kernel(const float* a, const float* b, float* o, int n) {
  const int i = blockIdx.x * blockDim.x + threadIdx.x;
  if (i < n) o[i] = a[i] + b[i];
}

static int run_res_block(dfot_uvit_s* h, const ResW& w, int lvl, int bt, hipStream_t s, const uint8_t* live = nullptr) {
  const int c = w.c, rr = h->r[lvl], pix = rr * rr;
  const int m = bt * pix;
  const int slots = pix / 64;
  bf16* xb = h->XB[lvl];
  int rc = 0;
  if (!h->xin_bf[lvl]) {
    if ((rc = launch_f32_to_bf16(h->xin[lvl], xb, (long)m * c, s))) return rc;
    h->xin_bf[lvl] = true;
  }
  if (h->gn1_nblk == 0) {
    if ((rc = launch_gn_partial_bf16(xb, h->gn_partial, bt, pix, c, s))) return rc;
    h->gn1_nblk = gn_partial_blocks(pix);
  }
  if ((rc = launch_gn_finalize(h->gn_partial, h->gn_stats, bt, h->gn1_nblk, pix, c, h->cfg.eps, s))) return rc;
  h->gn1_nblk = 0;
  if ((rc = launch_gn_apply_silu_bf16in(xb, h->gn_stats, w.g1, w.be1, h->s1, bt, pix, c, s, live))) return rc;
  GemmArgs g;
  g.A = h->s1; g.W = w.w1; g.M = m; g.N = c; g.K = 9 * c; g.H = rr; g.Wd = rr; g.Cin = c; g.zeros = h->zeros;
  g.bias = w.bias1; g.out_bf16 = h->hbf; g.ldo = c; g.live = live;
  g.gn_part = h->gn_partial2; g.gn_rows_per_bt = pix; g.gn_cpg = c / 32;
  if ((rc = launch_gemm(A_CONV3, E_BF16, h->gemm_variant, g, s))) return rc;
  if ((rc = launch_gn_finalize(h->gn_partial2, h->gn_stats, bt, slots, pix, c, h->cfg.eps, s))) return rc;
  if ((rc = launch_gn_film_silu(h->hbf, h->gn_stats, w.g2, w.be2, w.fcache, h->sv + w.sv_off,
                                h->have_mask ? h->cond_mask : nullptr, h->s1, bt, pix, c, h->T, s, live)))
    return rc;
  GemmArgs o;
  o.A = h->s1; o.W = w.w2; o.M = m; o.N = c; o.K = 9 * c; o.H = rr; o.Wd = rr; o.Cin = c; o.zeros = h->zeros;
  o.bias = w.bias2; o.out_bf16 = xb; o.ldo = c; o.live = live;
  o.resid_bf = xb;
  o.gn_part = h->gn_partial; o.gn_rows_per_bt = pix; o.gn_cpg = c / 32;
  if ((rc = launch_gemm(A_CONV3, E_BF16, h->gemm_variant, o, s))) return rc;
  h->xin_bf[lvl] = true;
  h->gn1_nblk = slots;
  return DFOT_OK;
}

__global__ void out_reduce_kernel(bf16* x, const float* __restrict__ bias, const float* __restrict__ s0, const float* __restrict__ s1,
                                  const float* __restrict__ s2, long total4, int cq) {
  typedef __attribute__((ext_vector_type(4))) float f4;
  const long i = (long)blockIdx.x * blockDim.x + threadIdx.x;
  if (i >= total4) return;
  f4 b = reinterpret_cast<const f4*>(bias)[i % cq] + reinterpret_cast<const f4*>(s0)[i] + reinterpret_cast<const f4*>(s1)[i];
  if (s2) b += reinterpret_cast<const f4*>(s2)[i];
  const bf16x4 xv = reinterpret_cast<const bf16x4*>(x)[i];
  reinterpret_cast<bf16x4*>(x)[i] = bf16x4{f2bf(bf2f(xv[0]) + b[0]), f2bf(bf2f(xv[1]) + b[1]), f2bf(bf2f(xv[2]) + b[2]), f2bf(bf2f(xv[3]) + b[3])};
}
__global__ void add_f32_into_bf16_kernel(bf16* x, const float* __restrict__ y, long total4) {
  typedef __attribute__((ext_vector_type(4))) float f4;
  const long i = (long)blockIdx.x * blockDim.x + threadIdx.x;
  if (i >= total4) return;
  const f4 b = reinterpret_cast<const f4*>(y)[i];
  const bf16x4 xv = reinterpret_cast<const bf16x4*>(x)[i];
  reinterpret_cast<bf16x4*>(x)[i] = bf16x4{f2bf(bf2f(xv[0]) + b[0]), f2bf(bf2f(xv[1]) + b[1]), f2bf(bf2f(xv[2]) + b[2]), f2bf(bf2f(xv[3]) + b[3])};
}

static void swap_out_part(dfot_uvit_s* h) { h->pend_part = h->out_part; }

static int flush_pending(dfot_uvit_s* h, hipStream_t s) {
  if (!h->pend_bias) return DFOT_OK;
  const long total4 = h->pend_m * h->pend_c / 4;
  hipLaunchKernelGGL(out_reduce_kernel, dim3(cdiv(total4, 256)), dim3(256), 0, s, h->XB[h->pend_lvl], h->pend_bias, h->pend_part,
                     h->pend_part + h->pend_m * h->pend_c, h->pend_slices == 3 ? h->pend_part + 2 * h->pend_m * h->pend_c : nullptr, total4,
                     h->pend_c / 4);
  h->pend_bias = nullptr;
  DFOT_CHECK_HIP(hipGetLastError());
  return DFOT_OK;
}

static int run_tr_block(dfot_uvit_s* h, const TrW& w, int lvl, int batch, hipStream_t s) {
  const int c = w.c, rr = h->r[lvl], n = h->T * rr * rr, d = c / h->heads;
  const int m = batch * n;
  bf16* xb = h->XB[lvl];
  int rc = 0;
  if (h->pend_bias && (h->pend_lvl != lvl || h->pend_m != m || h->pend_c != c) && (rc = flush_pending(h, s))) return rc;
  if (!h->xin_bf[lvl]) {
    if ((rc = launch_f32_to_bf16(h->xin[lvl], xb, (long)m * c, s))) return rc;
    h->xin_bf[lvl] = true;
  }
  RmsPending pend{xb, h->pend_bias, h->pend_part, h->pend_part + (long)m * c, h->pend_slices == 3 ? h->pend_part + 2L * m * c : nullptr};
  if ((rc = launch_rms_film_bf16(xb, w.nw, w.fcache, h->sv + w.sv_off, h->have_mask ? h->cond_mask : nullptr, h->s1, m, c, rr * rr, h->T,
                                 h->cfg.eps, s, h->pend_bias ? &pend : nullptr)))
    return rc;
  h->pend_bias = nullptr;
  GemmArgs p;
  p.A = h->s1; p.lda = c; p.W = w.w_fused; p.M = m; p.N = 7 * c; p.K = c; p.bias = w.b_fused;
  p.out2 = h->cat + c; p.ldo2 = 5 * c; p.split = 3 * c;
  p.q = h->q; p.k = h->k; p.v = h->v; p.qw = w.qw; p.kw = w.kw; p.rope_cs = h->rope_cs[lvl]; p.heads = h->heads; p.d = d;
  p.ntok = n; p.qscale = 1.4426950408889634f / sqrtf((float)d); p.eps = h->cfg.eps;
  if ((rc = launch_gemm(A_DENSE, E_QKV, h->gemm_variant, p, s))) return rc;
  const bool timed = h->time_attn && lvl == 2 && h->ev_used < h->ev_start.size();
  if (timed) DFOT_CHECK_HIP(hipEventRecord(h->ev_start[h->ev_used], s));
  int av = h->attn_variant;
  if (av == 2 && d == 64 && n % 256 == 0) av = (attention_v5_applies(n, d, w.score_bound) && !h->attn_force_safe) ? 14 : 5;
  if ((rc = launch_attention(h->q, h->k, h->v, h->cat, 5 * c, batch, h->heads, n, d, av, s, &h->attn_scratch))) return rc;
  if (timed) DFOT_CHECK_HIP(hipEventRecord(h->ev_stop[h->ev_used++], s));
  GemmArgs o;
  o.A = h->cat; o.lda = 5 * c; o.W = w.w_out; o.M = m; o.N = c; o.K = 5 * c; o.bias = w.b_out; o.ldo = c;
  if (h->gemm_variant == GEMM_AUTO && h->out_part && (size_t)2 * m * c <= h->out_part_elems && m % 256 == 0 && c % 144 == 0 &&
      (long)(m / 256) * (c / 144) * 2 <= 256 && (5 * c / 64) >= 8) {
    GemmArgs p2 = o;
    p2.bias = nullptr; p2.out_f32 = h->out_part; p2.ksplit = 2; p2.slice_stride = (long)m * c;
    if ((rc = launch_gemm(A_DENSE, E_F32, GEMM_DMA3_256x144, p2, s))) return rc;
    h->pend_bias = w.b_out;
    h->pend_lvl = lvl; h->pend_m = m; h->pend_c = c; h->pend_slices = 2;
    swap_out_part(h);
    return DFOT_OK;
  }
  if (h->gemm_variant == GEMM_AUTO && c % 144 == 0 && m % 256 == 0 && (long)(m / 256) * ((c + 191) / 192) < 256 &&
      (long)(m / 256) * (c / 144) >= 200 && (long)(m / 256) * (c / 144) <= 256) {
    o.out_bf16 = xb;
    o.resid_bf = xb;
    return launch_gemm(A_DENSE, E_BF16, GEMM_DMA3_256x144, o, s);
  }
  o.out_f32 = h->X[lvl];
  if ((rc = launch_gemm(A_DENSE, E_F32, h->gemm_variant, o, s))) return rc;
  hipLaunchKernelGGL(add_f32_into_bf16_kernel, dim3(cdiv((long)m * c / 4, 256)), dim3(256), 0, s, xb, h->X[lvl], (long)m * c / 4);
  DFOT_CHECK_HIP(hipGetLastError());
  return DFOT_OK;
}


__global__ void slab_reduce_kernel(float* __restrict__ out, const float* __restrict__ bias, const float* __restrict__ slabs, int nslab, long stride4,
                                   long total4, int cq, const uint8_t* __restrict__ live, unsigned img4) {
  typedef __attribute__((ext_vector_type(4))) float f4;
  const long i = (long)blockIdx.x * blockDim.x + threadIdx.x;
  if (i >= total4) return;
  if (live && !live[(unsigned)i / img4]) return;
  f4 v = reinterpret_cast<const f4*>(bias)[i % cq];
  for (int sl = 0; sl < nslab; ++sl) v += reinterpret_cast<const f4*>(slabs)[sl * stride4 + i];
  reinterpret_cast<f4*>(out)[i] = v;
}

static int conv_between_levels(dfot_uvit_s* h, GemmArgs g, hipStream_t s) {
  const long px = (long)g.H * g.Wd;
  if (h->gemm_variant == GEMM_AUTO && h->out_part && !g.gn_part && g.M % 256 == 0 && px % 256 == 0 && (g.N % 144 == 0 || g.N == 256) &&
      (long)g.M * g.N < (1L << 31)) {
    const int bn = g.N % 144 == 0 ? 144 : 256;
    const int variant = bn == 144 ? GEMM_DMA3_256x144 : GEMM_DMA_256x256;
    const int tiles = (g.M / 256) * (g.N / bn);
    int ks = 1;
    while (tiles * ks * 2 <= 256 && g.K / 64 / (ks * 2) >= 16) ks *= 2;
    if (tiles * ks >= 192 && tiles * ks <= 256) {
      if (ks == 1) return launch_gemm(A_CONV3, E_F32, variant, g, s);
      if ((size_t)ks * g.M * g.N <= h->out_part_elems) {
        GemmArgs p = g;
        float* out = g.out_f32;
        const float* bias = g.bias;
        p.bias = nullptr; p.resid = nullptr; p.out_f32 = h->out_part; p.ksplit = ks; p.slice_stride = (long)g.M * g.N;
        int rc = launch_gemm(A_CONV3, E_F32, variant, p, s);
        if (rc) return rc;
        const long total4 = (long)g.M * g.N / 4;
        hipLaunchKernelGGL(slab_reduce_kernel, dim3(cdiv(total4, 256)), dim3(256), 0, s, out, bias, h->out_part, ks, total4, total4, g.N / 4, g.live,
                           (unsigned)(px * g.N / 4));
        DFOT_CHECK_HIP(hipGetLastError());
        return DFOT_OK;
      }
    }
  }
  return launch_gemm(A_CONV3, E_F32, h->gemm_variant, g, s);
}

static int run_down(dfot_uvit_s* h, int l, int bt, hipStream_t s, const uint8_t* live = nullptr) {
  const int rr = h->r[l], cin = h->ch[l], cout = h->ch[l + 1];
  int rc = 0;
  if ((rc = h->xin_bf[l] ? launch_pool2_bf16_bf16in(h->XB[l], h->s1, bt, rr, rr, cin, s) : launch_pool2_bf16(h->xin[l], h->s1, bt, rr, rr, cin, s)))
    return rc;
  GemmArgs g;
  g.A = h->s1; g.W = h->down_conv[l].w; g.M = bt * (rr / 2) * (rr / 2); g.N = cout; g.K = 9 * cin; g.H = rr / 2; g.Wd = rr / 2;
  g.Cin = cin; g.zeros = h->zeros; g.bias = h->down_conv[l].b; g.out_f32 = h->HSA[l]; g.ldo = cout;
  g.live = live;
  const bool next_is_res = l + 1 < 2;
  if (next_is_res) {
    g.gn_part = h->gn_partial; g.gn_rows_per_bt = (rr / 2) * (rr / 2); g.gn_cpg = cout / 32;
  }
  if ((rc = conv_between_levels(h, g, s))) return rc;
  h->gn1_nblk = next_is_res ? g.gn_rows_per_bt / 64 : 0;
  h->xin[l + 1] = h->HSA[l];
  h->xin_bf[l + 1] = false;
  return DFOT_OK;
}

static int run_up(dfot_uvit_s* h, int l, int bt, hipStream_t s, const uint8_t* live = nullptr) {
  const int rr = h->r[l + 1], cin = h->ch[l + 1], cout = h->ch[l];
  const long n_in = (long)bt * rr * rr * cin;
  int rc = 0;
  if ((rc = h->xin_bf[l + 1] ? launch_sub_bf16_bf16in(h->XB[l + 1], h->HSA[l], h->s1, n_in, s, live, (long)rr * rr * cin)
                             : launch_sub_bf16(h->xin[l + 1], h->HSA[l], h->s1, n_in, s, live, (long)rr * rr * cin)))
    return rc;
  GemmArgs g;
  g.A = h->s1; g.W = h->up_conv[l].w; g.M = bt * rr * rr; g.N = cout; g.K = 9 * cin; g.H = rr; g.Wd = rr; g.Cin = cin;
  g.zeros = h->zeros; g.bias = h->up_conv[l].b; g.out_f32 = h->tmp; g.ldo = cout;
  if (live && (rr * rr) % 256 == 0 && h->gemm_variant == GEMM_AUTO) g.live = live;
  if ((rc = conv_between_levels(h, g, s))) return rc;
  h->gn1_nblk = 0;
  if (!h->xin_bf[l]) {
    set_error("run_up: level %d stream is not in its bf16 buffer", l);
    return DFOT_ERR_STATE;
  }
  return launch_upsample_add_bf16(h->tmp, h->XB[l], h->XB[l], bt, rr, rr, cout, s, live);
}

}

extern "C" {

const char* dfot_last_error(void) { return get_error(); }
int dfot_version(void) { return 1; }

int dfot_uvit_create(const dfot_uvit_config* cfg, dfot_uvit_t* out) {
  DFOT_REQUIRE(cfg && out, DFOT_ERR_ARG, "dfot_uvit_create: null argument");
  DFOT_REQUIRE(cfg->resolution % 16 == 0 && cfg->resolution >= 32, DFOT_ERR_SHAPE, "resolution %d must be a multiple of 16", cfg->resolution);
  DFOT_REQUIRE(cfg->emb_channels % 64 == 0, DFOT_ERR_SHAPE, "emb_channels %d must be a multiple of 64", cfg->emb_channels);
  DFOT_REQUIRE(cfg->in_channels <= 3 && cfg->cond_dim % 20 == 0, DFOT_ERR_SHAPE, "in_channels %d / cond_dim %d unsupported", cfg->in_channels, cfg->cond_dim);
  for (int l = 0; l < 4; ++l)
    DFOT_REQUIRE(cfg->channels[l] % 64 == 0, DFOT_ERR_SHAPE, "channels[%d]=%d must be a multiple of 64", l, cfg->channels[l]);
  DFOT_REQUIRE(cfg->channels[0] % 128 == 0 && cfg->channels[1] % 128 == 0, DFOT_ERR_SHAPE, "ResBlock channels must be multiples of 128");
  for (int l = 2; l < 4; ++l) {
    const int d = cfg->channels[l] / cfg->num_heads;
    DFOT_REQUIRE(d * cfg->num_heads == cfg->channels[l] && (d == 64 || d == 128), DFOT_ERR_SHAPE,
                 "level %d head dim %d must be 64 or 128", l, d);
  }
  const int r3 = cfg->resolution / 16;
  DFOT_REQUIRE((cfg->max_tokens * r3 * r3) % 128 == 0, DFOT_ERR_SHAPE, "tokens at the coarsest level (%d) must be a multiple of 128", cfg->max_tokens * r3 * r3);
  auto* h = new dfot_uvit_s();
  h->cfg = *cfg;
  int rc = build(h);
  if (rc) {
    dfot_uvit_destroy(h);
    return rc;
  }
  *out = h;
  return DFOT_OK;
}

int dfot_uvit_destroy(dfot_uvit_t h) {
  if (!h) return DFOT_OK;
  for (void* p : h->owned) (void)hipFree(p);
  for (void* p : h->ws_owned) (void)hipFree(p);
  for (hipEvent_t e : h->ev_start) (void)hipEventDestroy(e);
  for (hipEvent_t e : h->ev_stop) (void)hipEventDestroy(e);
  delete h;
  return DFOT_OK;
}

int dfot_uvit_num_params(dfot_uvit_t h) { return h ? (int)h->params.size() : 0; }
const char* dfot_uvit_param_name(dfot_uvit_t h, int i) {
  return (h && i >= 0 && i < (int)h->params.size()) ? h->params[i].name.c_str() : nullptr;
}
int dfot_uvit_param_shape(dfot_uvit_t h, int i, int64_t shape[4], int* ndim) {
  DFOT_REQUIRE(h && shape && ndim && i >= 0 && i < (int)h->params.size(), DFOT_ERR_ARG, "param_shape: bad argument");
  *ndim = (int)h->params[i].shape.size();
  for (int k = 0; k < *ndim; ++k) shape[k] = h->params[i].shape[k];
  return DFOT_OK;
}

int dfot_uvit_load_weight(dfot_uvit_t h, const char* name, const float* data, const int64_t* shape, int ndim, void* stream) {
  DFOT_REQUIRE(h && name && data && shape, DFOT_ERR_ARG, "load_weight: null argument");
  auto it = h->index.find(name);
  DFOT_REQUIRE(it != h->index.end(), DFOT_ERR_NAME, "load_weight: unexpected key '%s'", name);
  Param& p = h->params[it->second];
  bool same = (int)p.shape.size() == ndim;
  for (int k = 0; same && k < ndim; ++k) same = p.shape[k] == shape[k];
  DFOT_REQUIRE(same, DFOT_ERR_SHAPE, "load_weight: size mismatch for '%s'", name);
  int rc = p.load(data, (hipStream_t)stream);
  if (rc) return rc;
  p.loaded = true;
  h->finalized = false;
  return DFOT_OK;
}

int dfot_uvit_finalize(dfot_uvit_t h, void* stream) {
  DFOT_REQUIRE(h, DFOT_ERR_ARG, "finalize: null handle");
  for (const Param& p : h->params) DFOT_REQUIRE(p.loaded, DFOT_ERR_STATE, "finalize: missing key '%s'", p.name.c_str());
  hipStream_t s = (hipStream_t)stream;
  auto fuse = [&](std::vector<TrW>& v) -> int {
    for (TrW& w : v) {
      hipLaunchKernelGGL(add_vec_kernel, dim3(cdiv(w.c, 256)), dim3(256), 0, s, w.b_attn, w.b_mlp, w.b_out, w.c);
      DFOT_CHECK_HIP(hipGetLastError());
    }
    return DFOT_OK;
  };
  int rc = 0;
  if ((rc = fuse(h->down_tr)) || (rc = fuse(h->mid_tr)) || (rc = fuse(h->up_tr))) return rc;
  for (int l = 2; l < 4; ++l)
    if (!h->rope_cs[l] && (rc = build_rope(h, l))) return rc;
  DFOT_CHECK_HIP(hipStreamSynchronize(s));
  auto bound = [&](std::vector<TrW>& v) -> int {
    std::vector<float> qk;
    for (TrW& w : v) {
      const int d = w.c / h->heads;
      qk.resize(2 * d);
      DFOT_CHECK_HIP(hipMemcpy(qk.data(), w.qw, d * sizeof(float), hipMemcpyDeviceToHost));
      DFOT_CHECK_HIP(hipMemcpy(qk.data() + d, w.kw, d * sizeof(float), hipMemcpyDeviceToHost));
      float mqk = 0.f;
      for (int i = 0; i + 1 < d; i += 2)
        mqk = fmaxf(mqk, fmaxf(fabsf(qk[i]), fabsf(qk[i + 1])) * fmaxf(fabsf(qk[d + i]), fabsf(qk[d + i + 1])));
      w.score_bound = sqrtf((float)d) * mqk * 1.4426950408889634f;
      if (!(w.score_bound == w.score_bound)) w.score_bound = INFINITY;
    }
    return DFOT_OK;
  };
  if ((rc = bound(h->down_tr)) || (rc = bound(h->mid_tr)) || (rc = bound(h->up_tr))) return rc;
  h->finalized = true;
  return DFOT_OK;
}

int dfot_uvit_reserve(dfot_uvit_t h, int max_batch) {
  DFOT_REQUIRE(h && max_batch > 0, DFOT_ERR_ARG, "reserve: bad argument");
  if (max_batch <= h->max_batch) return DFOT_OK;
  for (void* p : h->ws_owned) (void)hipFree(p);
  h->ws_owned.clear();
  h->ws_bytes = 0;
  h->max_batch = 0;
  h->out_part = nullptr;
  h->pend_part = nullptr;
  h->out_part_elems = 0;
  h->attn_scratch = AttnScratch{};
  const size_t bt = (size_t)max_batch * h->T;
  size_t pix[4];
  for (int l = 0; l < 4; ++l) pix[l] = (size_t)h->r[l] * h->r[l];
  int rc = 0;
  if ((rc = dev_alloc(h, &h->nemb, bt * h->E, true))) return rc;
  if ((rc = dev_alloc(h, &h->nhid, bt * h->E, true))) return rc;
  for (int l = 0; l < 4; ++l) {
    if ((rc = dev_alloc(h, &h->XB[l], bt * pix[l] * h->ch[l], true))) return rc;
    if (l >= 2 && (rc = dev_alloc(h, &h->X[l], bt * pix[l] * h->ch[l], true))) return rc;
    if ((rc = dev_alloc(h, &h->emb[l], bt * pix[l] * h->E, true))) return rc;
  }
  for (int l = 0; l < 3; ++l)
    if ((rc = dev_alloc(h, &h->HSA[l], bt * pix[l + 1] * h->ch[l + 1], true))) return rc;
  if ((rc = dev_alloc(h, &h->acond, bt * pix[0] * h->kpose, true))) return rc;
  DFOT_CHECK_HIP(hipMemset(h->acond, 0, bt * pix[0] * h->kpose * sizeof(bf16)));
  size_t act = 0, tmpn = 0;
  for (int l = 0; l < 4; ++l) act = std::max(act, bt * pix[l] * h->ch[l]);
  for (int l = 0; l < 3; ++l) tmpn = std::max(tmpn, bt * pix[l + 1] * h->ch[l]);
  if ((rc = dev_alloc(h, &h->s1, act, true))) return rc;
  if ((rc = dev_alloc(h, &h->hbf, act, true))) return rc;
  if ((rc = dev_alloc(h, &h->tmp, tmpn, true))) return rc;
  if ((rc = dev_alloc(h, &h->gn_partial, bt * (pix[0] / 64) * 64, true))) return rc;
  if ((rc = dev_alloc(h, &h->gn_partial2, bt * (pix[0] / 64) * 64, true))) return rc;
  if ((rc = dev_alloc(h, &h->gn_stats, bt * 64, true))) return rc;
  size_t mtr = 0, mc = 0;
  for (int l = 2; l < 4; ++l) {
    mtr = std::max(mtr, bt * pix[l]);
    mc = std::max(mc, bt * pix[l] * h->ch[l]);
  }
  (void)mtr;
  {
    std::vector<FilmChunk> table;
    long sv_off = 0;
    auto add = [&](bf16** fc, long* off, const bf16* wf, const float* bf_, int c, int lvl) -> int {
      int r2 = dev_alloc(h, fc, bt * pix[lvl] * 2 * c, true);
      if (r2) return r2;
      *off = sv_off;
      for (int r0 = 0; r0 < 2 * c; r0 += 64) table.push_back(FilmChunk{wf + (long)r0 * h->E, bf_ + r0, sv_off + r0, 2 * c});
      sv_off += (long)bt * 2 * c;
      return DFOT_OK;
    };
    for (int l = 0; l < 2; ++l) {
      for (ResW& w : h->down_res[l]) if ((rc = add(&w.fcache, &w.sv_off, w.w_film, w.b_film, w.c, l))) return rc;
      for (ResW& w : h->up_res[l]) if ((rc = add(&w.fcache, &w.sv_off, w.w_film, w.b_film, w.c, l))) return rc;
    }
    for (TrW& w : h->down_tr) if ((rc = add(&w.fcache, &w.sv_off, w.w_film, w.b_film, w.c, 2))) return rc;
    for (TrW& w : h->up_tr) if ((rc = add(&w.fcache, &w.sv_off, w.w_film, w.b_film, w.c, 2))) return rc;
    for (TrW& w : h->mid_tr) if ((rc = add(&w.fcache, &w.sv_off, w.w_film, w.b_film, w.c, 3))) return rc;
    if ((rc = dev_alloc(h, &h->sv, (size_t)sv_off, true))) return rc;
    if ((rc = dev_alloc(h, &h->film_table, table.size(), true))) return rc;
    DFOT_CHECK_HIP(hipMemcpy(h->film_table, table.data(), table.size() * sizeof(FilmChunk), hipMemcpyHostToDevice));
    h->film_chunks = (int)table.size();
    if ((rc = dev_alloc(h, &h->cond_mask, (size_t)max_batch, true))) return rc;
    h->cond_batch = 0;
  }
  if ((rc = dev_alloc(h, &h->cat, mc * 5, true))) return rc;
  if ((rc = dev_alloc(h, &h->q, mc, true))) return rc;
  if ((rc = dev_alloc(h, &h->k, mc, true))) return rc;
  if ((rc = dev_alloc(h, &h->v, mc, true))) return rc;
  {
    const size_t e2 = bt * pix[2] * h->ch[2], e3 = bt * pix[3] * h->ch[3];
    h->out_part_elems = 3 * (e2 > e3 ? e2 : e3);
    if ((rc = dev_alloc(h, &h->out_part, h->out_part_elems, true))) return rc;
  }
  {
    size_t need = 16;
    for (int b = 1; b <= max_batch; ++b)
      for (int l = 2; l < 4; ++l) need = std::max(need, attention_scratch_bytes(b, h->heads, h->T * h->r[l] * h->r[l], h->ch[l] / h->heads));
    if ((rc = dev_alloc(h, &h->attn_scratch.p, need / sizeof(float), true))) return rc;
    h->attn_scratch.bytes = need;
  }
  h->max_batch = max_batch;
  return DFOT_OK;
}

size_t dfot_uvit_workspace_bytes(dfot_uvit_t h) { return h ? h->ws_bytes : 0; }

int dfot_uvit_attn_timing(dfot_uvit_t h, double* total_ms, int64_t* launches) {
  DFOT_REQUIRE(h && total_ms && launches, DFOT_ERR_ARG, "attn_timing: null argument");
  double tot = 0.0;
  for (size_t i = 0; i < h->ev_used; ++i) {
    DFOT_CHECK_HIP(hipEventSynchronize(h->ev_stop[i]));
    float ms = 0.f;
    DFOT_CHECK_HIP(hipEventElapsedTime(&ms, h->ev_start[i], h->ev_stop[i]));
    tot += ms;
  }
  *total_ms = tot;
  *launches = (int64_t)h->ev_used;
  h->ev_used = 0;
  return DFOT_OK;
}

int dfot_uvit_set_option(dfot_uvit_t h, const char* key, int value) {
  DFOT_REQUIRE(h && key, DFOT_ERR_ARG, "set_option: null argument");
  if (!strcmp(key, "gemm_variant")) h->gemm_variant = value;
  else if (!strcmp(key, "attn_variant")) h->attn_variant = value;
  else if (!strcmp(key, "attn_force_safe")) h->attn_force_safe = value != 0;
  else if (!strcmp(key, "time_attn")) {
    h->time_attn = value > 0;
    h->ev_used = 0;
    while ((int)h->ev_start.size() < value) {
      hipEvent_t a, b;
      DFOT_CHECK_HIP(hipEventCreate(&a));
      DFOT_CHECK_HIP(hipEventCreate(&b));
      h->ev_start.push_back(a);
      h->ev_stop.push_back(b);
    }
  }
  else {
    set_error("set_option: unknown key '%s'", key);
    return DFOT_ERR_ARG;
  }
  return DFOT_OK;
}

int dfot_uvit_query(dfot_uvit_t h, const char* key, double* value) {
  DFOT_REQUIRE(h && key && value, DFOT_ERR_ARG, "query: null argument");
  DFOT_REQUIRE(h->finalized, DFOT_ERR_STATE, "query: weights not finalized");
  float bound = 0.f;
  for (const TrW& w : h->down_tr) bound = fmaxf(bound, w.score_bound);
  for (const TrW& w : h->up_tr) bound = fmaxf(bound, w.score_bound);
  if (!strcmp(key, "score_bound_l2")) *value = bound;
  else if (!strcmp(key, "attn_kernel_l2")) *value = (bound < 64.0f && !h->attn_force_safe) ? 14 : 5;
  else if (!strcmp(key, "cond_builds")) *value = (double)h->cond_builds;
  else {
    set_error("query: unknown key '%s'", key);
    return DFOT_ERR_ARG;
  }
  return DFOT_OK;
}

int dfot_uvit_set_conditions(dfot_uvit_t h, const float* external_cond, const uint8_t* external_cond_mask, int batch,
                             void* stream) {
  DFOT_REQUIRE(h, DFOT_ERR_ARG, "set_conditions: null handle");
  DFOT_REQUIRE(external_cond != nullptr, DFOT_ERR_ARG, "External condition (camera pose) is required for U-ViT3DPose model.");
  DFOT_REQUIRE(h->finalized, DFOT_ERR_STATE, "set_conditions: weights not finalized");
  DFOT_REQUIRE(batch > 0 && batch <= h->max_batch, DFOT_ERR_STATE, "set_conditions: batch %d exceeds reserved %d", batch, h->max_batch);
  hipStream_t s = (hipStream_t)stream;
  const dfot_uvit_config& c = h->cfg;
  const int bt = batch * h->T, e = h->E;
  int rc = 0;
  h->cond_batch = 0;
  ++h->cond_builds;
  if ((rc = launch_cond_repack(external_cond, h->acond, bt, c.resolution, c.cond_dim, h->kpose, s))) return rc;
  {
    GemmArgs g;
    g.A = h->acond; g.lda = h->kpose; g.W = h->pose_w; g.M = bt * h->r[0] * h->r[0]; g.N = e; g.K = h->kpose;
    g.bias = h->pose_b; g.out_bf16 = h->emb[0]; g.ldo = e;
    if ((rc = launch_gemm(A_DENSE, E_BF16, h->gemm_variant, g, s))) return rc;
  }
  if ((rc = launch_emb_pyramid(h->emb[0], h->emb[1], h->emb[2], h->emb[3], bt, h->r[0], e, s))) return rc;
  auto fill = [&](bf16* fcache, const bf16* wf, int cc, int lvl) -> int {
    GemmArgs g;
    g.A = h->emb[lvl]; g.lda = e; g.W = wf; g.M = bt * h->r[lvl] * h->r[lvl]; g.N = 2 * cc; g.K = e;
    g.out_bf16 = fcache; g.ldo = 2 * cc;
    return launch_gemm(A_DENSE, E_BF16, h->gemm_variant, g, s);
  };
  for (int l = 0; l < 2; ++l) {
    for (ResW& w : h->down_res[l]) if ((rc = fill(w.fcache, w.w_film, w.c, l))) return rc;
    for (ResW& w : h->up_res[l]) if ((rc = fill(w.fcache, w.w_film, w.c, l))) return rc;
  }
  for (TrW& w : h->down_tr) if ((rc = fill(w.fcache, w.w_film, w.c, 2))) return rc;
  for (TrW& w : h->up_tr) if ((rc = fill(w.fcache, w.w_film, w.c, 2))) return rc;
  for (TrW& w : h->mid_tr) if ((rc = fill(w.fcache, w.w_film, w.c, 3))) return rc;
  h->have_mask = external_cond_mask != nullptr;
  if (h->have_mask) DFOT_CHECK_HIP(hipMemcpyAsync(h->cond_mask, external_cond_mask, batch, hipMemcpyDeviceToDevice, s));
  h->cond_batch = batch;
  return DFOT_OK;
}

int dfot_uvit_forward_cached(dfot_uvit_t h, const float* x, const float* noise_levels, float* out, int batch, void* stream) {
  return dfot_uvit_forward_cached_live(h, x, noise_levels, out, batch, nullptr, stream);
}

int dfot_uvit_forward_cached_live(dfot_uvit_t h, const float* x, const float* noise_levels, float* out, int batch, const uint8_t* live_frames,
                                  void* stream) {
  return dfot_uvit_forward_cached_masks(h, x, noise_levels, out, batch, live_frames, nullptr, stream);
}

int dfot_uvit_forward_cached_masks(dfot_uvit_t h, const float* x, const float* noise_levels, float* out, int batch, const uint8_t* live_frames,
                                   const uint8_t* fresh_frames, void* stream) {
  DFOT_REQUIRE(h && x && noise_levels && out, DFOT_ERR_ARG, "forward: null argument");
  DFOT_REQUIRE(!fresh_frames || h->last_batch == batch, DFOT_ERR_STATE,
               "forward: frozen frames need the previous forward of this handle to have run the same batch (%d, now %d)", h->last_batch, batch);
  DFOT_REQUIRE(!fresh_frames || live_frames, DFOT_ERR_ARG, "forward: frozen frames must also be dead frames (live_frames is null)");
  DFOT_REQUIRE(h->finalized, DFOT_ERR_STATE, "forward: weights not finalized");
  DFOT_REQUIRE(batch > 0 && batch == h->cond_batch, DFOT_ERR_STATE,
               "forward_cached: batch %d does not match the cached conditions (%d)", batch, h->cond_batch);
  hipStream_t s = (hipStream_t)stream;
  const dfot_uvit_config& c = h->cfg;
  const int bt = batch * h->T, e = h->E;
  int rc = 0;
  if ((rc = launch_noise_emb(noise_levels, h->ne_freqs, h->ne_phases, h->ne_w1, h->ne_b1, h->ne_w2, h->ne_b2, h->nhid,
                             h->nemb, bt, c.noise_dim, e, s)))
    return rc;
  if ((rc = launch_film_vec(h->film_table, h->film_chunks, h->nemb, h->sv, bt, e, s))) return rc;
  if ((rc = launch_embed_input_bf16(x, h->ein_w, h->ein_b, h->XB[0], bt, c.resolution, c.in_channels, h->ch[0], s))) return rc;
  h->gn1_nblk = 0;
  for (int l = 0; l < 4; ++l) h->xin[l] = h->X[l];
  h->xin_bf[0] = true;
  h->xin_bf[1] = h->xin_bf[2] = h->xin_bf[3] = false;

  if (fresh_frames && (h->gemm_variant != GEMM_AUTO || (h->r[2] * h->r[2]) % 512 != 0)) fresh_frames = nullptr;
  for (int l = 0; l < 2; ++l) {
    for (const ResW& w : h->down_res[l])
      if ((rc = run_res_block(h, w, l, bt, s, fresh_frames))) return rc;
    if ((rc = run_down(h, l, bt, s, fresh_frames))) return rc;
  }
  h->pend_bias = nullptr;
  for (const TrW& w : h->down_tr)
    if ((rc = run_tr_block(h, w, 2, batch, s))) return rc;
  if ((rc = flush_pending(h, s))) return rc;
  if ((rc = run_down(h, 2, bt, s))) return rc;
  for (const TrW& w : h->mid_tr)
    if ((rc = run_tr_block(h, w, 3, batch, s))) return rc;
  if ((rc = flush_pending(h, s))) return rc;
  if ((rc = run_up(h, 2, bt, s))) return rc;
  for (const TrW& w : h->up_tr)
    if ((rc = run_tr_block(h, w, 2, batch, s))) return rc;
  if ((rc = flush_pending(h, s))) return rc;
  for (int l = 1; l >= 0; --l) {
    if ((rc = run_up(h, l, bt, s, live_frames))) return rc;
    for (const ResW& w : h->up_res[l])
      if ((rc = run_res_block(h, w, l, bt, s, live_frames))) return rc;
  }
  h->last_batch = batch;
  return launch_project_output_bf16(h->XB[0], h->pout_w, h->pout_b, out, bt, c.resolution, h->ch[0], c.in_channels, s, live_frames);
}

int dfot_uvit_forward(dfot_uvit_t h, const float* x, const float* noise_levels, const float* external_cond,
                      const uint8_t* external_cond_mask, float* out, int batch, void* stream) {
  DFOT_REQUIRE(h && x && noise_levels && out, DFOT_ERR_ARG, "forward: null argument");
  int rc = dfot_uvit_set_conditions(h, external_cond, external_cond_mask, batch, stream);
  if (rc) return rc;
  return dfot_uvit_forward_cached(h, x, noise_levels, out, batch, stream);
}

int dfot_uvit_read_tap(dfot_uvit_t h, const char* name, float* out, size_t capacity, void* stream) {
  DFOT_REQUIRE(h && name && out, DFOT_ERR_ARG, "read_tap: null argument");
  DFOT_REQUIRE(h->last_batch > 0, DFOT_ERR_STATE, "read_tap: no forward has run");
  hipStream_t s = (hipStream_t)stream;
  const int bt = h->last_batch * h->T;
  auto pixels = [&](int l) { return h->r[l] * h->r[l]; };
  struct Tap { const char* n; int lvl; int c; const float* f; const bf16* b; };
  const Tap taps[] = {
      {"pose_emb0", 0, h->E, nullptr, h->emb[0]}, {"down0", 1, h->ch[1], h->HSA[0], nullptr},
      {"down1", 2, h->ch[2], h->HSA[1], nullptr}, {"down2", 3, h->ch[3], h->HSA[2], nullptr},
      {"mid", 3, h->ch[3], nullptr, h->XB[3]}, {"up2", 2, h->ch[2], nullptr, h->XB[2]},
      {"up1", 1, h->ch[1], nullptr, h->XB[1]}, {"up0", 0, h->ch[0], nullptr, h->XB[0]},
  };
  for (const Tap& t : taps) {
    if (strcmp(t.n, name)) continue;
    const size_t need = (size_t)bt * pixels(t.lvl) * t.c;
    DFOT_REQUIRE(capacity >= need, DFOT_ERR_SHAPE, "read_tap: need %zu floats, got %zu", need, capacity);
    return t.f ? launch_nhwc_to_nchw(t.f, out, bt, pixels(t.lvl), t.c, s)
               : launch_bf16_nhwc_to_nchw(t.b, out, bt, pixels(t.lvl), t.c, s);
  }
  set_error("read_tap: unknown tap '%s'", name);
  return DFOT_ERR_NAME;
}

int dfot_ray_encode(const float* raw_poses, float* out, int batch, int tokens, int resolution, void* stream) {
  DFOT_REQUIRE(raw_poses && out && batch > 0 && tokens > 0 && resolution > 0, DFOT_ERR_ARG, "ray_encode: bad argument");
  return launch_ray_encode(raw_poses, out, batch, tokens, resolution, 0, (hipStream_t)stream);
}

int dfot_ray_encode_normalized(const float* poses, float* out, int batch, int tokens, int resolution, void* stream) {
  DFOT_REQUIRE(poses && out && batch > 0 && tokens > 0 && resolution > 0, DFOT_ERR_ARG, "ray_encode_normalized: bad argument");
  return launch_ray_encode(poses, out, batch, tokens, resolution, 1, (hipStream_t)stream);
}

int dfot_hg_prepare(const float* x, const float* noise, const float* qa, const float* qb, float* x_in, int batch, int nfe,
                    int tokens, int64_t frame_elems, void* stream) {
  DFOT_REQUIRE(x && qa && qb && x_in, DFOT_ERR_ARG, "hg_prepare: null argument");
  return launch_hg_prepare(x, noise, qa, qb, x_in, batch, nfe, tokens, (long)frame_elems, (hipStream_t)stream);
}

int dfot_ddim_compose(const float* x, const float* x_in, const float* v, const float* sa, const float* s1, const float* an,
                      const float* cn, const float* keep, const float* weight, const uint8_t* gen, float* x_next, int batch,
                      int nfe, int tokens, int64_t frame_elems, void* stream) {
  DFOT_REQUIRE(x && x_in && v && sa && s1 && an && cn && keep && weight && gen && x_next, DFOT_ERR_ARG, "ddim_compose: null argument");
  return launch_ddim_compose(x, x_in, v, sa, s1, an, cn, keep, weight, gen, x_next, batch, nfe, tokens, (long)frame_elems, false,
                             (hipStream_t)stream);
}
int dfot_ddim_compose_tokw(const float* x, const float* x_in, const float* v, const float* sa, const float* s1, const float* an,
                           const float* cn, const float* keep, const float* weight, const uint8_t* gen, float* x_next, int batch,
                           int nfe, int tokens, int64_t frame_elems, void* stream) {
  DFOT_REQUIRE(x && x_in && v && sa && s1 && an && cn && keep && weight && gen && x_next, DFOT_ERR_ARG, "ddim_compose_tokw: null argument");
  return launch_ddim_compose(x, x_in, v, sa, s1, an, cn, keep, weight, gen, x_next, batch, nfe, tokens, (long)frame_elems, true,
                             (hipStream_t)stream);
}

int dfot_ddim_noise(const float* noise, const float* sigma, const float* weight, const uint8_t* gen, float* x_next, int batch, int nfe,
                    int tokens, int64_t frame_elems, int weight_per_token, void* stream) {
  DFOT_REQUIRE(noise && sigma && weight && gen && x_next, DFOT_ERR_ARG, "ddim_noise: null argument");
  return launch_ddim_noise(noise, sigma, weight, gen, x_next, batch, nfe, tokens, (long)frame_elems, weight_per_token != 0, (hipStream_t)stream);
}

int dfot_vpred_loss(const float* x, const float* noise, const float* v, const float* alpha, const float* sigma,
                    const float* weight, float* x_pred, float* scratch, float* loss, int batch, int tokens, int64_t frame_elems,
                    void* stream) {
  DFOT_REQUIRE(x && noise && v && alpha && sigma && weight && scratch && loss, DFOT_ERR_ARG, "vpred_loss: null argument");
  return launch_vloss(x, noise, v, alpha, sigma, weight, x_pred, scratch, loss, batch, tokens, (long)frame_elems, false,
                      (hipStream_t)stream);
}
int dfot_vspace_loss(const float* x, const float* noise, const float* v, const float* alpha, const float* sigma,
                     const float* weight, float* x_pred, float* scratch, float* loss, int batch, int tokens, int64_t frame_elems,
                     void* stream) {
  DFOT_REQUIRE(x && noise && v && alpha && sigma && weight && scratch && loss, DFOT_ERR_ARG, "vspace_loss: null argument");
  return launch_vloss(x, noise, v, alpha, sigma, weight, x_pred, scratch, loss, batch, tokens, (long)frame_elems, true,
                      (hipStream_t)stream);
}
int64_t dfot_vpred_loss_scratch_floats(int batch, int tokens, int64_t frame_elems) {
  return (int64_t)batch * tokens * vloss_chunks((long)frame_elems);
}

static bf16* g_zero_page = nullptr;
static int zero_page(bf16** out) {
  if (!g_zero_page) {
    DFOT_CHECK_HIP(hipMalloc((void**)&g_zero_page, 512));
    DFOT_CHECK_HIP(hipMemset(g_zero_page, 0, 512));
  }
  *out = g_zero_page;
  return DFOT_OK;
}

int dfot_op_gemm(const void* a, int lda, const void* w, const float* bias, float* c, int m, int n, int k, int variant,
                 void* stream) {
  GemmArgs g;
  g.A = (const bf16*)a; g.lda = lda; g.W = (const bf16*)w; g.M = m; g.N = n; g.K = k; g.bias = bias; g.out_f32 = c; g.ldo = n;
  DFOT_REQUIRE(c, DFOT_ERR_ARG, "op_gemm: null output");
  return launch_gemm(A_DENSE, E_F32, variant, g, (hipStream_t)stream);
}

int dfot_op_conv3x3(const void* a, const void* w, const float* bias, float* y, int bt, int hh, int ww, int cin, int cout,
                    int variant, void* stream) {
  GemmArgs g;
  int rc = zero_page(const_cast<bf16**>(&g.zeros));
  if (rc) return rc;
  g.A = (const bf16*)a; g.W = (const bf16*)w; g.M = bt * hh * ww; g.N = cout; g.K = 9 * cin; g.H = hh; g.Wd = ww; g.Cin = cin;
  g.bias = bias; g.out_f32 = y; g.ldo = cout;
  DFOT_REQUIRE(y, DFOT_ERR_ARG, "op_conv3x3: null output");
  return launch_gemm(A_CONV3, E_F32, variant, g, (hipStream_t)stream);
}

int dfot_op_gemm_ex(const dfot_gemm_desc* d, void* stream) {
  DFOT_REQUIRE(d, DFOT_ERR_ARG, "op_gemm_ex: null descriptor");
  GemmArgs g;
  if (d->amode == A_CONV3) {
    int rc = zero_page(const_cast<bf16**>(&g.zeros));
    if (rc) return rc;
  }
  g.A = (const bf16*)d->A; g.lda = d->lda; g.W = (const bf16*)d->W; g.ldw = d->ldw;
  g.M = d->M; g.N = d->N; g.K = d->K; g.H = d->H; g.Wd = d->Wd; g.Cin = d->Cin;
  g.live = d->live; g.bias = d->bias; g.bias_rows = d->bias_rows;
  g.out_f32 = d->out_f32; g.out_bf16 = (bf16*)d->out_bf16; g.ldo = d->ldo;
  g.resid = d->resid; g.resid_bf = (const bf16*)d->resid_bf;
  g.gate = d->gate; g.gate_index = d->gate_index; g.ldg = d->ldg; g.gate_rows = d->gate_rows;
  g.act = d->act; g.pre_act = (bf16*)d->pre_act; g.raw = (bf16*)d->raw; g.ldraw = d->ldraw; g.tr_rows = d->tr_rows;
  g.gn_part = d->gn_part; g.gn_rows_per_bt = d->gn_rows_per_bt; g.gn_cpg = d->gn_cpg;
  g.out2 = (bf16*)d->out2; g.ldo2 = d->ldo2; g.split = d->split;
// ... 25 lines not shown
```

diffusion-forcing-transformer_amd/sampler.py:

```python
from __future__ import annotations

from dataclasses import dataclass, field
from typing import Callable, Dict, List, Optional, Tuple

import numpy as np
import torch

from . import capi, parallel
from .diffusion import DiffusionConfig, Schedule
from .guidance import HistoryGuidance


@dataclass
class SamplerConfig:
    x_shape: Tuple[int, int, int] = (3, 256, 256)
    max_tokens: int = 8
    diffusion: DiffusionConfig = field(default_factory=DiffusionConfig)
    scheduling_matrix: str = "full_sequence"
    is_full_sequence: bool = False
    prediction_guidance: Dict = field(default_factory=lambda: {"name": "conditional"})
    interpolation_guidance: Dict = field(default_factory=lambda: {"name": "conditional"})
    keyframe_density: Optional[float] = None
    sliding_context_len: Optional[int] = None
    interpolation_max_batch_size: Optional[int] = None
    refinement_sampling: Optional[Dict] = None
    camera_pose_normalize_by: str = "first"
    camera_pose_bound: Optional[float] = None
    external_cond_type: str = "action"
    external_cond_dim: int = 0
    external_cond_processing: Optional[str] = None


NoiseFn = Callable[[str, tuple], torch.Tensor]


def device_noise_fn(generator: Optional[torch.Generator] = None, clip: float = 20.0) -> NoiseFn:
    def fn(tag: str, shape: tuple) -> torch.Tensor:
        return torch.randn(shape, device="cuda", generator=generator).clamp_(-clip, clip)
    return fn


class DFoTVideoPoseSampler:
    def __init__(self, cfg: SamplerConfig, backbone, noise_fn: Optional[NoiseFn] = None):
        self.cfg = cfg
        self.model = backbone
        self.schedule = Schedule(cfg.diffusion)
        self.noise_fn = noise_fn or device_noise_fn(clip=cfg.diffusion.clip_noise)
        self.timesteps = cfg.diffusion.timesteps
        self.sampling_timesteps = cfg.diffusion.sampling_timesteps
        self.max_tokens = cfg.max_tokens
        self.x_shape = tuple(cfg.x_shape)
        self.trace: List[dict] = []
        self.window_forwards = 0
        self.shard_windows = False
        self.branch_parallel = False
        self._branch_split_active = False
        self.device = "cuda"
        self.dry_run = False
        self.use_graph = True
        self.skip_frozen_frames = True
        self.skip_dead_frames = True
        self.graph_replays = 0
        self.graph_captures = 0
        self._graphs: Dict[tuple, dict] = {}
        self._graphs_generation = 0
        if cfg.diffusion.sampling_timesteps > cfg.diffusion.timesteps:
            raise ValueError("sampling_timesteps must be <= timesteps")

    @torch.no_grad()
    def _process_conditions(self, conditions: Optional[torch.Tensor], noise_levels=None) -> Optional[torch.Tensor]:
        if conditions is None:
            return None
        if conditions.shape[-1] != 16:
            raise ValueError(f"raw camera poses must have 16 values per frame, got {conditions.shape[-1]}")
        cfg = self.cfg
        if cfg.camera_pose_normalize_by not in ("first", "mean"):
            raise ValueError(f"Unknown camera pose normalization method: {cfg.camera_pose_normalize_by}")
        interp = None
        if noise_levels is not None and getattr(self, "_interpolate_masked_poses", False):
            interp = np.asarray(noise_levels.detach().cpu().numpy() if torch.is_tensor(noise_levels) else noise_levels) == self.timesteps - 1
        if cfg.camera_pose_normalize_by == "first" and cfg.camera_pose_bound is None and interp is None:
            return torch.ops.dfot.ray_encoding(conditions, int(self.x_shape[-1]))
        from . import pose
        world = pose.normalize_poses(conditions.detach().float().cpu().numpy(), cfg.camera_pose_normalize_by, cfg.camera_pose_bound, interp)
        return torch.ops.dfot.ray_encoding(torch.from_numpy(world), int(self.x_shape[-1]), True)

    def _select_conditions(self, conditions: Optional[torch.Tensor], index) -> Optional[torch.Tensor]:
        return None if conditions is None else conditions[:, index]

    def _padded_conditions(self, conditions: Optional[torch.Tensor], index) -> Optional[torch.Tensor]:
        return None if conditions is None else self._pad_to_max_tokens(conditions[:, index])

    def _window_conditions(self, conditions: Optional[torch.Tensor]) -> Optional[torch.Tensor]:
        return self._process_conditions(conditions)

    def _check_conditions(self, conditions: Optional[torch.Tensor], length: int) -> None:
        pass

    _static_graph_cond = False

    @torch.no_grad()
    def denoising_loss(self, xs: torch.Tensor, conditions: Optional[torch.Tensor], t: torch.Tensor,
                       noise: Optional[torch.Tensor] = None, masks: Optional[torch.Tensor] = None):
        b, tk = xs.shape[:2]
        f = int(np.prod(xs.shape[2:]))
        logsnr, alpha, sigma, weight = self.cfg.diffusion.training_logsnr_tables(t)
        tab = torch.stack([alpha, sigma, weight, self.cfg.diffusion.precond_scale * logsnr]).float().cuda().contiguous()
        x = xs.to(device="cuda", dtype=torch.float32).contiguous()
        if noise is None:
            noise = self.noise_fn("train", tuple(x.shape))
        eps = noise.to(device="cuda", dtype=torch.float32).clamp(-self.cfg.diffusion.clip_noise, self.cfg.diffusion.clip_noise).contiguous()
        ones = torch.ones(b, tk, device="cuda")
        x_t = torch.empty_like(x)
        capi.check(capi.lib.dfot_hg_prepare(capi.ptr(x), capi.ptr(eps), capi.ptr(tab[0]), capi.ptr(tab[1]), capi.ptr(x_t),
                                            b, 1, tk, f, capi.stream_ptr()))
        v = self.model(x_t, tab[3], self._process_conditions(conditions), None)
        x_pred = torch.empty_like(x)
        per_token = torch.empty(b, tk, device="cuda")
        scratch = torch.empty(int(capi.lib.dfot_vpred_loss_scratch_floats(b, tk, f)), device="cuda")
        capi.check(capi.lib.dfot_vpred_loss(capi.ptr(x), capi.ptr(eps), capi.ptr(v), capi.ptr(tab[0]), capi.ptr(tab[1]),
                                            capi.ptr(tab[2]), capi.ptr(x_pred), capi.ptr(scratch), capi.ptr(per_token), b, tk, f,
                                            capi.stream_ptr()))
        del ones
        if masks is not None:
            per_token = per_token * masks.to(device="cuda", dtype=torch.float32).view(b, tk)
        return x_pred, per_token.mean(), per_token

    @torch.no_grad()
    def discrete_denoising_loss(self, xs: torch.Tensor, k: torch.Tensor, noise: Optional[torch.Tensor] = None,
                                masks: Optional[torch.Tensor] = None, loss_weighting: Optional[Dict] = None):
        if self.cfg.diffusion.is_continuous:
            raise ValueError("discrete_denoising_loss needs DiffusionConfig(is_continuous=False)")
        b, tk = xs.shape[:2]
        f = int(np.prod(xs.shape[2:]))
        kk = k.detach().cpu().numpy().astype(np.int64)
        sch = self.schedule
        tab = np.stack([sch.sqrt_alphas_cumprod[kk], sch.sqrt_one_minus_alphas_cumprod[kk],
                        sch.loss_weights(kk, **(loss_weighting or {}))]).astype(np.float32)
        tab = torch.from_numpy(tab).cuda().contiguous()
        x = xs.to(device="cuda", dtype=torch.float32).contiguous()
        if noise is None:
            noise = self.noise_fn("train", tuple(x.shape))
        eps = noise.to(device="cuda", dtype=torch.float32).clamp(-self.cfg.diffusion.clip_noise, self.cfg.diffusion.clip_noise).contiguous()
        x_k = torch.empty_like(x)
        capi.check(capi.lib.dfot_hg_prepare(capi.ptr(x), capi.ptr(eps), capi.ptr(tab[0]), capi.ptr(tab[1]), capi.ptr(x_k),
                                            b, 1, tk, f, capi.stream_ptr()))
        v = self.model(x_k, k.to(device="cuda", dtype=torch.int32), None, None)
        x_pred = torch.empty_like(x)
        per_token = torch.empty(b, tk, device="cuda")
        scratch = torch.empty(int(capi.lib.dfot_vpred_loss_scratch_floats(b, tk, f)), device="cuda")
        capi.check(capi.lib.dfot_vspace_loss(capi.ptr(x), capi.ptr(eps), capi.ptr(v), capi.ptr(tab[0]), capi.ptr(tab[1]),
                                             capi.ptr(tab[2]), capi.ptr(x_pred), capi.ptr(scratch), capi.ptr(per_token), b, tk, f,
                                             capi.stream_ptr()))
        if masks is not None:
            per_token = per_token * masks.to(device="cuda", dtype=torch.float32).view(b, tk)
        return x_pred, per_token.mean(), per_token

    def _normalize_x(self, xs: torch.Tensor, mean, std) -> torch.Tensor:
        m = torch.as_tensor(mean, dtype=xs.dtype, device=xs.device).view(-1, 1, 1)
        s = torch.as_tensor(std, dtype=xs.dtype, device=xs.device).view(-1, 1, 1)
        return (xs - m) / s

    def _unnormalize_x(self, xs: torch.Tensor, mean, std) -> torch.Tensor:
        m = torch.as_tensor(mean, dtype=xs.dtype, device=xs.device).view(-1, 1, 1)
        s = torch.as_tensor(std, dtype=xs.dtype, device=xs.device).view(-1, 1, 1)
        return xs * s + m

    def _pad_to_max_tokens(self, y: Optional[torch.Tensor]) -> Optional[torch.Tensor]:
        if y is None or y.shape[1] >= self.max_tokens:
            return y
        tail = y[:, -1:].expand(-1, self.max_tokens - y.shape[1], *y.shape[2:])
        return torch.cat([y, tail], dim=1)

    @torch.no_grad()
    def _sample_sequence(self, batch_size: int, length: Optional[int] = None, context: Optional[torch.Tensor] = None,
                         context_mask: Optional[torch.Tensor] = None, conditions: Optional[torch.Tensor] = None,
                         history_guidance: Optional[HistoryGuidance] = None, _refine: Optional[Tuple[int, int]] = None,
                         **_) -> Tuple[torch.Tensor, None]:
        cfg, sch = self.cfg, self.schedule
        x_shape = self.x_shape
        pose_interp = conditions is not None and history_guidance is not None and history_guidance.needs_pose_interpolation
        if length is None:
            length = self.max_tokens if context is None else context.shape[1]
        if length > self.max_tokens:
            raise ValueError(f"length is expected to <={self.max_tokens}, got {length}.")
        if context is not None:
            if context_mask is None:
                raise ValueError("context_mask must be provided if context is given.")
            if context.shape[0] != batch_size:
                raise ValueError(f"context batch size is expected to be {batch_size} but got {context.shape[0]}.")
            if context.shape[1] != length:
                raise ValueError(f"context length is expected to be {length} but got {context.shape[1]}.")
            if tuple(context.shape[2:]) != tuple(x_shape):
                raise ValueError(f"context shape not compatible with x_stacked_shape {x_shape}.")
        if context_mask is not None:
            if context is None:
                raise ValueError("context must be provided if context_mask is given. ")
            if tuple(context.shape[:2]) != tuple(context_mask.shape):
                raise ValueError("context and context_mask must have the same shape.")
        self._check_conditions(conditions, length)
        horizon = self.max_tokens
        padding = horizon - length
        f = int(np.prod(x_shape))
        dev = self.device
        if dev != "cuda" and not self.dry_run:
            raise RuntimeError("the sampler runs on the GPU; device='cpu' is only valid together with dry_run (no CPU fallback)")
        xs = self.noise_fn("init", (batch_size, horizon, *x_shape)).to(device=dev, dtype=torch.float32)
        xs = xs.clamp(-cfg.diffusion.clip_noise, cfg.diffusion.clip_noise)
        if context is None:
            mask = np.zeros((batch_size, horizon), np.int64)
        else:
            mask = context_mask.detach().cpu().numpy().astype(np.int64)
            ctx = context.to(device=dev, dtype=torch.float32)
            if padding > 0:
                ctx = torch.cat([ctx, ctx.new_zeros(batch_size, padding, *x_shape)], 1)
                mask = np.concatenate([mask, -np.ones((batch_size, padding), np.int64)], 1)
            keep = torch.from_numpy(mask >= 1).to(dev).view(batch_size, horizon, 1, 1, 1)
            xs = torch.where(keep, ctx, xs)
        rg = float(getattr(cfg.diffusion, "reconstruction_guidance", 0.0) or 0.0)
        if rg > 0 and not sch.is_ddim_sampling:
            raise ValueError("reconstruction guidance is a DDIM-step feature (discrete_diffusion.py:455-513); sampling_timesteps == timesteps selects DDPM")
        rg_ctx = (ctx if context is not None else torch.zeros_like(xs)) if rg > 0 and not self.dry_run else None
        if history_guidance is None:
            history_guidance = HistoryGuidance.conditional(timesteps=self.timesteps)

        if _refine is None:
            sm = sch.scheduling_matrix(cfg.scheduling_matrix, horizon - padding, padding)
            sm = np.repeat(sm[:, None, :], batch_size, axis=1)
            if not cfg.is_full_sequence:
                sm = np.where(mask[None] >= 1, -1, sm)
            changed = ~(sm[1:] == sm[:-1]).reshape(sm.shape[0] - 1, -1).all(axis=1)
            sm = sm[int(np.argmax(changed)):]
        else:
            if cfg.scheduling_matrix != "full_sequence":
                raise ValueError("Refining only support full_sequence scheduling matrix")
            sm = sch.refine_scheduling_matrix(horizon - padding, _refine[0], _refine[1], padding)
            sm = np.repeat(sm[:, None, :], batch_size, axis=1)
            sm = np.where(mask[None] >= 1, -1, sm)
        self.trace.append({"context_mask": mask.copy(), "batch": batch_size, "rows": sm.shape[0]})

        plans = []
        for m in range(sm.shape[0] - 1):
            frm, to = sm[m], sm[m + 1]
            if _refine is not None and not frm[0, -1] > to[0, -1]:
                ac = sch.alphas_cumprod.astype(np.float32)
                with np.errstate(divide="ignore", invalid="ignore"):
                    scale = np.where(to == self.timesteps - 1, np.float32(1), ac[to] / ac[frm]).astype(np.float32)
                if not (np.isfinite(scale).all() and (scale <= 1).all()):
                    raise ValueError("refinement sampling: this window / schedule makes q_sample_from_x_k produce NaN in the reference "
                                     "(alphas_cumprod ratio not in [0, 1]); refused instead of returning NaN")
                tables = np.zeros((8, batch_size, horizon), np.float32)
                tables[0], tables[1] = np.sqrt(scale), np.sqrt(np.float32(1) - scale)
                plans.append(dict(renoise=True, nfe=1, bm=batch_size, tables=tables, gen=(mask == 0).astype(np.uint8), cmask=None))
                continue
            mask = np.where((mask == 0) & (frm == -1), 2, mask)
            plan = history_guidance.plan(mask, frm, to, replacement_only=cfg.is_full_sequence)
            bm = batch_size * plan.nfe
            lv = plan.levels.reshape(bm, horizon)
            tl = plan.to_levels.reshape(bm, horizon)
            repl = plan.replace.reshape(bm, horizon)
            qa_c, qb_c = sch.q_sample_coef(lv)
            qa = np.where(repl, qa_c, np.float32(1)).astype(np.float32)
            qb = np.where(repl, qb_c, np.float32(0)).astype(np.float32)
            excl = None
            if plan.excluded is not None:
                excl = plan.excluded.reshape(bm, horizon)
                qa, qb = np.where(excl, np.float32(0), qa), np.where(excl, np.float32(1), qb)
            sa, s1, an, cn, keepf, sigma = sch.ddim_coef(lv, tl) if sch.is_ddim_sampling else sch.ddpm_coef(lv)
            sigma = np.where(keepf != 0, np.float32(0), sigma).astype(np.float32)
            tables = np.stack([qa, qb, sa, s1, an, cn, keepf, sch.model_level(lv)]).astype(np.float32)
            plans.append(dict(plan=plan, nfe=plan.nfe, bm=bm, need_noise=bool(repl.any()) or excl is not None, excl=excl, tables=tables,
                              sigma=sigma if bool((sigma != 0).any()) else None,
                              gen=(mask == 0).astype(np.uint8),
                              cmask=None if plan.cond_masked is None else np.tile(plan.cond_masked, batch_size)))
        if not plans:
            return (xs[:, :-padding] if padding > 0 else xs), None
        strict = bool(getattr(self.noise_fn, "strict_order", False))

        def draw_noise(p_):
            nfe, bm, need = p_["nfe"], p_["bm"], p_["need_noise"]
            noise = None
            if history_guidance.is_simple:
                if nfe == 2 and (need or strict):
                    drawn = self.noise_fn("q_sample", (batch_size, horizon, *x_shape))
                    noise = torch.zeros(batch_size, 2, horizon, *x_shape, device=dev, dtype=torch.float32)
                    noise[:, 0] = drawn.to(device=dev, dtype=torch.float32)
            else:
                g = p_["plan"].n_gen
                bh = bm // g
                if need or strict:
                    noise = self.noise_fn("q_sample", (bh, horizon, *x_shape)).to(device=dev, dtype=torch.float32)
                    if g > 1:
                        noise = noise.repeat_interleave(g, dim=0)
                if strict or p_["excl"] is not None:
                    fresh = self.noise_fn("excluded", (bh, g, horizon, *x_shape))
                    if p_["excl"] is not None:
                        fresh = fresh.to(device=dev, dtype=torch.float32).reshape(bm, horizon, *x_shape)
                        em = torch.from_numpy(p_["excl"]).to(dev).view(bm, horizon, *([1] * len(x_shape)))
                        noise = torch.where(em, fresh, noise if noise is not None else torch.zeros_like(fresh))
            return None if noise is None else noise.contiguous().view(bm, horizon, *x_shape)

        split_nfe = set()
        if self._branch_split_active:
            world_n = parallel.world_info()[0]
            for n_ in sorted({p_["nfe"] for p_ in plans if not p_.get("renoise")}):
                if n_ > 1 and world_n > 1 and world_n % n_ == 0:
                    parallel.branch_group(n_)
                    split_nfe.add(n_)
        if self.dry_run:
            for p_ in plans:
                if p_["nfe"] in split_nfe:
                    hb = parallel.world_info()[1] % p_["nfe"]
                    got = parallel.exchange_branches(torch.full((batch_size, 1), float(hb)), p_["nfe"])
                    if not torch.equal(got.view(batch_size, p_["nfe"]), torch.arange(p_["nfe"], dtype=got.dtype).repeat(batch_size, 1)):
                        raise RuntimeError("branch exchange returned the branches out of (sample, branch) order")
                    self.branch_exchanges = getattr(self, "branch_exchanges", 0) + 1
                if p_.get("renoise"):
                    self.noise_fn("renoise", (batch_size, horizon, *x_shape))
                    continue
                draw_noise(p_)
                if strict or p_["sigma"] is not None:
                    self.noise_fn("ddim", (p_["bm"], horizon, *x_shape))
                    if _refine is not None:
                        self.noise_fn("refine_context", (batch_size, horizon, *x_shape))
            self.window_forwards += sum(p_["bm"] for p_ in plans if not p_.get("renoise"))
            return (xs[:, :-padding] if padding > 0 else xs), None
        flat_dev = torch.from_numpy(np.concatenate([p_["tables"].ravel() for p_ in plans])).cuda()
        gens_dev = torch.from_numpy(np.stack([p_["gen"] for p_ in plans])).cuda()
        off = 0
        cmask_cache: Dict[bytes, torch.Tensor] = {}
        weight_cache: Dict[bytes, torch.Tensor] = {}
        lives_by_nfe: Dict[int, torch.Tensor] = {}
        for i, p_ in enumerate(plans):
            n = p_["tables"].size
            p_["tables_dev"] = flat_dev[off:off + n].view(8, p_["bm"], horizon)
            off += n
            p_["gen_dev"] = gens_dev[i]
            if p_.get("renoise"):
                continue
            if p_["nfe"] not in lives_by_nfe:
                lives_by_nfe[p_["nfe"]] = gens_dev if p_["nfe"] == 1 else gens_dev.repeat_interleave(p_["nfe"], dim=1)
            p_["live_dev"] = lives_by_nfe[p_["nfe"]][i]
            wsrc = p_["plan"].weights if p_["plan"].tok_weights is None else p_["plan"].tok_weights
            wkey = wsrc.tobytes()
            if wkey not in weight_cache:
                weight_cache[wkey] = torch.from_numpy(np.ascontiguousarray(wsrc, dtype=np.float32)).cuda()
            p_["weights_dev"] = weight_cache[wkey]
            p_["tokw"] = p_["plan"].tok_weights is not None
            p_["sigma_dev"] = None if p_["sigma"] is None else torch.from_numpy(p_["sigma"]).cuda()
            p_["cmask_dev"] = None
            if p_["cmask"] is not None:
                ckey = p_["cmask"].tobytes()
                if ckey not in cmask_cache:
                    cmask_cache[ckey] = torch.from_numpy(p_["cmask"]).cuda()
                p_["cmask_dev"] = cmask_cache[ckey]

        cond_full = None if pose_interp else self._window_conditions(conditions)
        cond_rep, cond_nfe = None, 0
        if pose_interp:
            by_mask: Dict[bytes, torch.Tensor] = {}
            self._interpolate_masked_poses = True
            try:
                for p_ in plans:
                    if p_.get("renoise"):
                        continue
                    lv = p_["plan"].levels.reshape(p_["bm"], horizon)
                    key = (lv == self.timesteps - 1).tobytes() + bytes([p_["nfe"]])
                    if key not in by_mask:
                        by_mask[key] = self._process_conditions(conditions.repeat_interleave(p_["nfe"], dim=0), lv)
                    p_["cond"] = by_mask[key]
            finally:
                self._interpolate_masked_poses = False
        fresh_dev = torch.from_numpy(np.concatenate([a.ravel() for a in self._fresh_flags(plans, batch_size, horizon)])).cuda()
        foff = 0
        for p_ in plans:
            p_["fresh_dev"] = fresh_dev[foff:foff + p_["bm"] * horizon].view(p_["bm"], horizon)
            foff += p_["bm"] * horizon
        xs = xs.contiguous()
        s = capi.stream_ptr
        branch_cache: Dict[tuple, tuple] = {}

        skip_dead = self.skip_dead_frames and hasattr(self.model, "live_frames")
        skip_frozen = skip_dead and self.skip_frozen_frames and hasattr(self.model, "fresh_frames")

        def step(p_, xs, noise, tables, gen_dev, xs_next=None, live_dev=None, fresh_dev=None):
            nonlocal cond_rep, cond_nfe
            nfe, bm = p_["nfe"], p_["bm"]
            x_in = torch.empty(bm, horizon, *x_shape, device="cuda", dtype=torch.float32)
            capi.check(capi.lib.dfot_hg_prepare(capi.ptr(xs), capi.ptr(noise), capi.ptr(tables[0]), capi.ptr(tables[1]),
                                                capi.ptr(x_in), batch_size, nfe, horizon, f, s()))
            if cond_full is not None and cond_nfe != nfe:
                cond_rep = cond_full if nfe == 1 else cond_full.repeat_interleave(nfe, dim=0)
                cond_nfe = nfe
            if "cond" in p_:
                cond_rep = p_["cond"]
            lvl = tables[7] if cfg.diffusion.is_continuous else tables[7].to(torch.int32)
            world, rank = parallel.world_info()
            if nfe in split_nfe:
                hb = rank % nfe
                key = (id(cond_rep), id(p_["cmask_dev"]), hb)
                if key not in branch_cache:
                    c_h = None if cond_rep is None else cond_rep.view(batch_size, nfe, *cond_rep.shape[1:])[:, hb].contiguous()
                    m_h = None if p_["cmask_dev"] is None else p_["cmask_dev"].view(batch_size, nfe)[:, hb].contiguous()
                    branch_cache[key] = (c_h, m_h, cond_rep, p_["cmask_dev"])
                c_h, m_h = branch_cache[key][:2]
                x_h = x_in.view(batch_size, nfe, horizon, *x_shape)[:, hb].contiguous()
                l_h = lvl.view(batch_size, nfe, horizon)[:, hb].contiguous()
                if skip_dead:
                    self.model.live_frames = gen_dev
                try:
                    v = parallel.exchange_branches(self.model(x_h, l_h, c_h, m_h), nfe)
                    self.branch_exchanges = getattr(self, "branch_exchanges", 0) + 1
                finally:
                    if skip_dead:
                        self.model.live_frames = None
            elif rg > 0:
                v = self._reconstruction_guided_v(x_in, lvl, cond_rep, p_["cmask_dev"], tables, gen_dev, rg_ctx, rg, nfe)
            else:
                if skip_dead:
                    self.model.live_frames = live_dev if live_dev is not None else p_["live_dev"]
                if skip_frozen:
                    self.model.fresh_frames = fresh_dev if fresh_dev is not None else p_["fresh_dev"]
                try:
                    v = self.model(x_in, lvl, cond_rep, p_["cmask_dev"])
                finally:
                    if skip_dead:
                        self.model.live_frames = None
                    if skip_frozen:
                        self.model.fresh_frames = None
            step_noise = None
            if strict or p_["sigma"] is not None:
                step_noise = self.noise_fn("ddim", (bm, horizon, *x_shape))
            if xs_next is None:
                xs_next = torch.empty_like(xs)
            compose = capi.lib.dfot_ddim_compose_tokw if p_["tokw"] else capi.lib.dfot_ddim_compose
            capi.check(compose(capi.ptr(xs), capi.ptr(x_in), capi.ptr(v), capi.ptr(tables[2]),
                                                  capi.ptr(tables[3]), capi.ptr(tables[4]), capi.ptr(tables[5]),
                                                  capi.ptr(tables[6]), capi.ptr(p_["weights_dev"]), capi.ptr(gen_dev),
                                                  capi.ptr(xs_next), batch_size, nfe, horizon, f, s()))
            if p_["sigma"] is not None:
                nz = step_noise.to(device="cuda", dtype=torch.float32).clamp(-cfg.diffusion.clip_noise, cfg.diffusion.clip_noise).contiguous()
                capi.check(capi.lib.dfot_ddim_noise(capi.ptr(nz), capi.ptr(p_["sigma_dev"]), capi.ptr(p_["weights_dev"]), capi.ptr(gen_dev),
                                                    capi.ptr(xs_next), batch_size, nfe, horizon, f, int(p_["tokw"]), s()))
            return xs_next

        def renoise(p_, xs):
            noise = self.noise_fn("renoise", (batch_size, horizon, *x_shape)).to(device="cuda", dtype=torch.float32)
            noise = noise.clamp(-cfg.diffusion.clip_noise, cfg.diffusion.clip_noise).contiguous()
            out = torch.empty_like(xs)
            capi.check(capi.lib.dfot_hg_prepare(capi.ptr(xs), capi.ptr(noise), capi.ptr(p_["tables_dev"][0]), capi.ptr(p_["tables_dev"][1]),
                                                capi.ptr(out), batch_size, 1, horizon, f, s()))
            return out

        if _refine is not None:
            for p_ in plans:
                if p_.get("renoise"):
                    xs = renoise(p_, xs)
                    continue
                xs = step(p_, xs, draw_noise(p_), p_["tables_dev"], p_["gen_dev"])
                if strict:
                    self.noise_fn("refine_context", (batch_size, horizon, *x_shape))
            self.window_forwards += sum(p_["bm"] for p_ in plans if not p_.get("renoise"))
            return (xs[:, :-padding] if padding > 0 else xs), None
        uniform = all(p_["bm"] == plans[0]["bm"] and p_["cmask_dev"] is plans[0]["cmask_dev"]
                      and p_["weights_dev"] is plans[0]["weights_dev"] and p_.get("cond") is plans[0].get("cond") for p_ in plans)
        hook = getattr(self, "step_hook", None)
        if (self.use_graph and uniform and not strict and len(plans) > 2 and all(p_["sigma"] is None for p_ in plans) and not self._branch_split_active
                and rg == 0 and hook is None):
            if self._static_graph_cond and cond_full is not None:
                nfe0 = plans[0]["nfe"]
                plans[0]["cond_src"] = cond_full if nfe0 == 1 else cond_full.repeat_interleave(nfe0, dim=0)
            xs = self._run_steps_graph(plans, xs, draw_noise, step, flat_dev, gens_dev, horizon)
        else:
            for i, p_ in enumerate(plans):
                xs = step(p_, xs, draw_noise(p_), p_["tables_dev"], p_["gen_dev"])
                if hook is not None:
                    hook(i, xs)
        self.window_forwards += sum(p_["bm"] for p_ in plans)
        if padding > 0:
            xs = xs[:, :-padding]
        return xs, None

    @torch.no_grad()
    def _sample_sequence_refine(self, batch_size: int, goback_length: int, n_goback: int, length: Optional[int] = None,
                                context: Optional[torch.Tensor] = None, context_mask: Optional[torch.Tensor] = None,
                                conditions: Optional[torch.Tensor] = None, history_guidance: Optional[HistoryGuidance] = None,
                                **_) -> Tuple[torch.Tensor, None]:
        return self._sample_sequence(batch_size, length=length, context=context, context_mask=context_mask, conditions=conditions,
                                     history_guidance=history_guidance, _refine=(int(goback_length), int(n_goback)))

    def _window_sampler(self):
        return self._sample_sequence

    def _reconstruction_guided_v(self, x_in, lvl, cond, cmask, tables, gen_dev, ctx, rg: float, nfe: int):
        if nfe != 1:
            raise ValueError("reconstruction guidance needs one-branch history guidance (the reference's loss compares the "
                             "(B * NFE, ...) prediction with the (B, ...) context)")
        if self.cfg.diffusion.objective != "pred_v":
            raise ValueError("reconstruction guidance is implemented for the v objective")
        nd = x_in.ndim
        ext = lambda a: a.reshape(*a.shape, *([1] * (nd - a.ndim)))
        sa, s1 = ext(tables[2]), ext(tables[3])
        with torch.enable_grad():
            x = x_in.detach().requires_grad_(True)
            v = self.model(x, lvl, cond, cmask)
            pred_x0 = sa * x - s1 * v
            cm = ext((gen_dev == 0).to(torch.float32))
            loss = torch.sum((pred_x0 - ctx) ** 2 * sa * cm / cm.sum(dim=1, keepdim=True).clamp(min=1))
            grad = torch.nan_to_num(-torch.autograd.grad(-rg * 0.5 * loss, x)[0], nan=0.0)
        an, cn = ext(tables[4]), ext(tables[5])
        scale = torch.where(sa > 0, s1 / sa.clamp(min=1e-30), torch.where(an > 0, -cn / an.clamp(min=1e-30), torch.zeros_like(sa)))
        return (v.detach() + scale * grad).contiguous()

    @staticmethod
    def _fresh_flags(plans, batch_size: int, horizon: int):
        out, prev = [], None
        for p_ in plans:
            fresh = np.ones((p_["bm"], horizon), np.uint8)
            if p_.get("renoise"):
                out.append(fresh)
                prev = None
                continue
            if (prev is not None and prev["bm"] == p_["bm"] and prev["nfe"] == p_["nfe"] and prev.get("cond") is p_.get("cond")
                    and ((prev["cmask"] is None and p_["cmask"] is None)
                         or (prev["cmask"] is not None and p_["cmask"] is not None and np.array_equal(prev["cmask"], p_["cmask"])))):
                a, b = prev["tables"], p_["tables"]
                same_in = (a[0] == 1) & (a[1] == 0) & (b[0] == 1) & (b[1] == 0) & (a[7] == b[7])
                untouched = np.repeat(prev["gen"].reshape(batch_size, horizon) == 0, p_["nfe"], axis=0)
                fresh = np.where(same_in & untouched, 0, 1).astype(np.uint8)
            out.append(fresh)
            prev = p_
        return out

    def _run_steps_graph(self, plans, xs, draw_noise, step, flat_dev, gens_dev, horizon):
        p0 = plans[0]
        bm, n_steps, nfe = p0["bm"], len(plans), p0["nfe"]
        need_noise = any(p_["need_noise"] for p_ in plans)
        self.model.reserve(bm)
        if hasattr(self.model, "sync_weights"):
            self.model.sync_weights()
        gen = getattr(self.model, "reserve_generation", 0)
        if gen != self._graphs_generation:
            self._graphs.clear()
            self._graphs_generation = gen
        cond_src = p0.get("cond_src")
        key = (bm, n_steps, nfe, horizon, tuple(xs.shape), need_noise, None if p0["cmask"] is None else p0["cmask"].tobytes(),
               id(self.model), None if cond_src is None else (tuple(cond_src.shape), cond_src.dtype))
        ent = self._graphs.get(key)
        if ent is None:
            ent = dict(tables=torch.empty(n_steps, 8, bm, horizon, device="cuda", dtype=torch.float32),
                       gens=torch.empty_like(gens_dev), weights=torch.empty_like(p0["weights_dev"]),
                       lives=torch.empty(n_steps, bm, horizon, device="cuda", dtype=torch.uint8),
                       fresh=torch.empty(n_steps, bm, horizon, device="cuda", dtype=torch.uint8),
                       noise=torch.empty(n_steps, bm, *xs.shape[1:], device="cuda") if need_noise else None,
                       xs=torch.empty_like(xs), out=None, graph=None,
                       cond=None if cond_src is None else torch.empty_like(cond_src))
        ent["tables"].copy_(flat_dev.view(n_steps, 8, bm, horizon))
        ent["gens"].copy_(gens_dev)
        ent["lives"].copy_(gens_dev if nfe == 1 else gens_dev.repeat_interleave(nfe, dim=1))
        ent["fresh"].copy_(torch.stack([p_["fresh_dev"] for p_ in plans]))
        ent["weights"].copy_(p0["weights_dev"])
        if need_noise:
            for i, p_ in enumerate(plans):
                if p_["need_noise"]:
                    ent["noise"][i].copy_(draw_noise(p_))
                else:
                    ent["noise"][i].zero_()
        p_static = dict(p0, weights_dev=ent["weights"])
        if cond_src is not None:
            ent["cond"].copy_(cond_src)
            p_static["cond"] = ent["cond"]
        ent["xs"].copy_(step(p_static, xs, None if not need_noise else ent["noise"][0], ent["tables"][0], ent["gens"][0], live_dev=ent["lives"][0],
                            fresh_dev=ent["fresh"][0]))
        if ent["graph"] is None:
            torch.cuda.synchronize()
            graph = torch.cuda.CUDAGraph()
            with torch.cuda.graph(graph, capture_error_mode="thread_local"):
                x = ent["xs"]
                for i in range(1, n_steps):
                    x = step(p_static, x, ent["noise"][i] if need_noise else None, ent["tables"][i], ent["gens"][i], live_dev=ent["lives"][i],
                             fresh_dev=ent["fresh"][i])
                ent["out"] = x
            ent["graph"] = graph
            if len(self._graphs) >= 4:
                self._graphs.pop(next(iter(self._graphs)))
            self._graphs[key] = ent
            self.graph_captures += 1
        ent["graph"].replay()
        self.graph_replays += n_steps - 1
        return ent["out"].clone()

    @torch.no_grad()
    def _predict_sequence(self, context: torch.Tensor, length: Optional[int] = None,
                          conditions: Optional[torch.Tensor] = None, history_guidance: Optional[HistoryGuidance] = None,
                          sliding_context_len: Optional[int] = None, **_) -> Tuple[torch.Tensor, None]:
        mt = self.max_tokens
        if length is None:
            length = mt
        if sliding_context_len is None:
            if mt < length:
                raise ValueError("when length > max_tokens, sliding_context_len must be specified.")
            sliding_context_len = mt - 1
        if sliding_context_len == -1:
            sliding_context_len = mt - 1
        batch_size, gt_len = context.shape[:2]
        if sliding_context_len < gt_len:
            raise ValueError("sliding_context_len is expected to be >= length of initial context,"
                             f"got {sliding_context_len}. If you are trying to use max context, "
                             "consider specifying sliding_context_len=-1.")
        xs = context.to(device=self.device, dtype=torch.float32)
        cur = gt_len
        n_window = 0
        while cur < length:
            c = min(sliding_context_len, cur)
            h = min(length - cur, mt - c)
            window = torch.cat([xs[:, -c:], xs.new_zeros(batch_size, h, *self.x_shape)], 1)
            generated = cur - max(cur - c, gt_len)
            cmask = torch.ones(batch_size, c, dtype=torch.long)
            if generated > 0:
                cmask[:, -generated:] = 2
            cmask = torch.cat([cmask, torch.zeros(batch_size, h, dtype=torch.long)], 1)
            cond = self._select_conditions(conditions, slice(cur - c, cur - c + mt))
            if hasattr(self.noise_fn, "set_windows"):
                self.noise_fn.set_windows([n_window])
            n_window += 1
            new, _ = self._window_sampler()(batch_size, length=c + h, context=window, context_mask=cmask,
                                           conditions=cond, history_guidance=history_guidance)
            xs = torch.cat([xs, new[:, -h:]], 1)
            cur = xs.shape[1]
        return xs, None

    def _interpolation_plan(self, known: np.ndarray) -> List[List[np.ndarray]]:
        mt = self.max_tokens
        known = known.copy()
        plan: List[List[np.ndarray]] = []
        while not known.all():
            keys = np.where(known)[0]
            stage: List[np.ndarray] = []
            chunk: Optional[np.ndarray] = None
            for left, right in zip(keys[:-1], keys[1:]):
                left, right = int(left), int(right)
                if chunk is not None:
                    if len(chunk) + right - left <= mt:
                        chunk = np.concatenate([chunk, np.arange(left + 1, right + 1)])
                        continue
                    stage.append(chunk)
                    chunk = None
                if right - left == 1:
                    continue
                if right - left >= mt - 1:
                    stage.append(torch.linspace(left, right, mt).round().long().numpy())
                else:
                    chunk = np.arange(left, right + 1)
            if chunk is not None:
                stage.append(chunk)
            for w in stage:
                known[w] = True
            plan.append(stage)
        return plan

    @torch.no_grad()
    def _interpolate_videos(self, context: torch.Tensor, context_mask: Optional[torch.Tensor] = None,
                            conditions: Optional[torch.Tensor] = None, **_) -> torch.Tensor:
        cfg = self.cfg
        if context_mask is None:
            context_mask = torch.zeros(context.shape[0], context.shape[1], dtype=torch.bool)
            context_mask[:, [0, -1]] = True
        else:
            context_mask = context_mask.detach().cpu().bool()
            assert bool(context_mask[:, [0, -1]].all()), "The first and last frames must be known to interpolate."
        hg = HistoryGuidance.from_config(cfg.interpolation_guidance, timesteps=self.timesteps)
        xs = context.to(device=self.device, dtype=torch.float32).clone()
        known = context_mask.clone()
        for si, stage in enumerate(self._interpolation_plan(context_mask[0].numpy())):
            ctx = torch.cat([self._pad_to_max_tokens(xs[:, w]) for w in stage], 0)
            msk = torch.cat([self._pad_to_max_tokens(known[:, w]) for w in stage], 0)
            cnd = None if conditions is None else torch.cat([self._padded_conditions(conditions, w) for w in stage], 0)

            def sample_batch(ids, ctx=ctx, msk=msk, cnd=cnd, si=si):
                if not ids:
                    return ctx.new_zeros((0, *ctx.shape[1:]))
                if hasattr(self.noise_fn, "set_windows"):
                    self.noise_fn.set_windows([(si + 1) * 100000 + i for i in ids])
                o, _ = self._window_sampler()(len(ids), context=ctx[ids], context_mask=msk[ids].long(),
                                             conditions=None if cnd is None else cnd[ids], history_guidance=hg)
                return o

            mb = cfg.interpolation_max_batch_size or ctx.shape[0]
            if self.shard_windows:
                out = parallel.run_sharded(ctx.shape[0], sample_batch, mb)
            else:
                out = torch.cat([sample_batch(list(range(i, min(i + mb, ctx.shape[0])))) for i in range(0, ctx.shape[0], mb)], 0)
            for w, pred in zip(stage, out.chunk(len(stage), 0)):
                xs[:, w] = pred[:, : len(w)]
                known[:, w] = True
        return xs

    @torch.no_grad()
    def _predict_videos(self, xs: torch.Tensor, n_context_tokens: int,
                        conditions: Optional[torch.Tensor] = None) -> torch.Tensor:
        cfg = self.cfg
        out = xs.to(device=self.device, dtype=torch.float32).clone()
        hg = HistoryGuidance.from_config(cfg.prediction_guidance, timesteps=self.timesteps)
        density = cfg.keyframe_density or 1
        if density > 1:
            raise ValueError("tasks.prediction.keyframe_density must be <= 1")
        n = out.shape[1]
        keys = torch.linspace(0, n - 1, round(density * n)).round().long()
        keys = torch.cat([torch.arange(n_context_tokens), keys]).unique()
        kc = self._select_conditions(conditions, keys)
        if self.branch_parallel and parallel.world_info()[0] > 1 and not (hasattr(self.noise_fn, "set_windows") or getattr(self.noise_fn, "replicated", False)):
            raise ValueError("branch_parallel needs a rank-independent noise source: parallel.WindowKeyedNoise (set_windows) or a noise_fn "
                             "whose attribute `replicated` is True (every rank draws the same tensors)")
        self._branch_split_active = bool(self.branch_parallel)
        try:
            pred, _ = self._predict_sequence(out[:, :n_context_tokens], length=len(keys), conditions=kc, history_guidance=hg,
                                             sliding_context_len=cfg.sliding_context_len or self.max_tokens // 2)
        finally:
            self._branch_split_active = False
        out[:, keys.to(self.device)] = pred
        if len(keys) < n:
            known = torch.zeros(out.shape[0], n, dtype=torch.bool)
            known[:, keys] = True
            out = self._interpolate_videos(out, known, conditions)
        return out


class DFoTVideoSampler(DFoTVideoPoseSampler):

    _static_graph_cond = True

    def _cond_type(self) -> str:
        t = self.cfg.external_cond_type
        if t not in ("label", "action"):
# ... 68 lines not shown
```

include/dfot_hip.h:

```cpp
#ifndef DFOT_HIP_H_
#define DFOT_HIP_H_

#include <stddef.h>
#include <stdint.h>

#ifdef __cplusplus
extern "C" {
#endif

enum {
  DFOT_OK = 0,
  DFOT_ERR_ARG = 1,
  DFOT_ERR_SHAPE = 2,
  DFOT_ERR_HIP = 3,
  DFOT_ERR_STATE = 4,
  DFOT_ERR_NAME = 5
};

typedef struct dfot_uvit_s* dfot_uvit_t;

typedef struct {
  int32_t channels[4];
  int32_t emb_channels;
  int32_t num_updown_blocks[3];
  int32_t num_mid_blocks;
  int32_t num_heads;
  int32_t in_channels;
  int32_t resolution;
  int32_t max_tokens;
  int32_t cond_dim;
  int32_t noise_dim;
  float rope_theta;
  float eps;
} dfot_uvit_config;

const char* dfot_last_error(void);
int dfot_version(void);

int dfot_uvit_create(const dfot_uvit_config* cfg, dfot_uvit_t* out);
int dfot_uvit_destroy(dfot_uvit_t h);
int dfot_uvit_num_params(dfot_uvit_t h);
const char* dfot_uvit_param_name(dfot_uvit_t h, int index);
int dfot_uvit_param_shape(dfot_uvit_t h, int index, int64_t shape[4], int* ndim);
int dfot_uvit_load_weight(dfot_uvit_t h, const char* name, const float* data, const int64_t* shape, int ndim,
                          void* stream);
int dfot_uvit_finalize(dfot_uvit_t h, void* stream);
int dfot_uvit_reserve(dfot_uvit_t h, int max_batch);
size_t dfot_uvit_workspace_bytes(dfot_uvit_t h);
int dfot_uvit_set_option(dfot_uvit_t h, const char* key, int value);
int dfot_uvit_query(dfot_uvit_t h, const char* key, double* value);
int dfot_uvit_attn_timing(dfot_uvit_t h, double* total_ms, int64_t* launches);

int dfot_uvit_forward(dfot_uvit_t h, const float* x, const float* noise_levels, const float* external_cond,
                      const uint8_t* external_cond_mask, float* out, int batch, void* stream);
int dfot_uvit_set_conditions(dfot_uvit_t h, const float* external_cond, const uint8_t* external_cond_mask, int batch,
                             void* stream);
int dfot_uvit_forward_cached(dfot_uvit_t h, const float* x, const float* noise_levels, float* out, int batch,
                             void* stream);
int dfot_uvit_forward_cached_live(dfot_uvit_t h, const float* x, const float* noise_levels, float* out, int batch,
                                  const uint8_t* live_frames, void* stream);
int dfot_uvit_forward_cached_masks(dfot_uvit_t h, const float* x, const float* noise_levels, float* out, int batch,
                                   const uint8_t* live_frames, const uint8_t* fresh_frames, void* stream);
int dfot_uvit_read_tap(dfot_uvit_t h, const char* name, float* out, size_t capacity_floats, void* stream);

typedef struct dfot_dit_s* dfot_dit_t;

typedef struct {
  int32_t hidden_size;
  int32_t depth;
  int32_t num_heads;
  int32_t patch_size;
  int32_t in_channels;
  int32_t height;
  int32_t width;
  int32_t max_tokens;
  int32_t mlp_hidden;
  int32_t noise_dim;
  int32_t timesteps;
  float rope_theta;
  float eps;
  int32_t variant;
  int32_t embed_col_dim;
  int32_t num_col_heads;
  int32_t num_row_heads;
  int32_t temporal_mlp_hidden;
  int32_t use_bias;
  int32_t cond_type;
  int32_t cond_dim;
  int32_t num_classes;
  int32_t cond_dropout;
  int32_t use_temporal_rope;
} dfot_dit_config;
enum { DFOT_COND_NONE = 0, DFOT_COND_ACTION = 1, DFOT_COND_LABEL = 2 };

typedef struct {
  dfot_dit_config base;
  int32_t fourier_noise;
} dfot_dit_config_f;

int dfot_dit_create(const dfot_dit_config* cfg, dfot_dit_t* out);
int dfot_dit_create_f(const dfot_dit_config_f* cfg, dfot_dit_t* out);
int dfot_dit_destroy(dfot_dit_t h);
int dfot_dit_num_params(dfot_dit_t h);
const char* dfot_dit_param_name(dfot_dit_t h, int index);
int dfot_dit_param_shape(dfot_dit_t h, int index, int64_t shape[4], int* ndim);
int dfot_dit_load_weight(dfot_dit_t h, const char* name, const float* data, const int64_t* shape, int ndim, void* stream);
int dfot_dit_finalize(dfot_dit_t h, void* stream);
int dfot_dit_reserve(dfot_dit_t h, int max_batch);
size_t dfot_dit_workspace_bytes(dfot_dit_t h);
int dfot_dit_set_option(dfot_dit_t h, const char* key, int value);
int dfot_dit_attn_timing(dfot_dit_t h, double* total_ms, int64_t* launches);
int dfot_dit_forward(dfot_dit_t h, const float* x, const int32_t* noise_levels, float* out, int batch, int tokens,
                     void* stream);
int dfot_dit_forward_cond(dfot_dit_t h, const float* x, const int32_t* noise_levels, const float* cond, const int32_t* labels,
                          const uint8_t* cond_mask, float* out, int batch, int tokens, void* stream);
int dfot_dit_forward_f(dfot_dit_t h, const float* x, const float* noise_levels, const float* cond, const int32_t* labels,
                       const uint8_t* cond_mask, float* out, int batch, int tokens, void* stream);
int dfot_dit_read_tap(dfot_dit_t h, const char* name, float* out, size_t capacity_floats, void* stream);

typedef struct dfot_dit_train_s* dfot_dit_train_t;
int dfot_dit_train_create(const dfot_dit_config* cfg, dfot_dit_train_t* out);
int dfot_dit_train_create_f(const dfot_dit_config_f* cfg, dfot_dit_train_t* out);
int dfot_dit_train_destroy(dfot_dit_train_t h);
int dfot_dit_train_num_params(dfot_dit_train_t h);
const char* dfot_dit_train_param_name(dfot_dit_train_t h, int i);
int dfot_dit_train_param_shape(dfot_dit_train_t h, int i, int64_t shape[4], int* ndim);
int64_t dfot_dit_train_param_offset(dfot_dit_train_t h, int i);
int64_t dfot_dit_train_total_numel(dfot_dit_train_t h);
size_t dfot_dit_train_workspace_bytes(dfot_dit_train_t h);
int dfot_dit_train_attach(dfot_dit_train_t h, float* params, float* grads);
int dfot_dit_train_reserve(dfot_dit_train_t h, int max_batch);
int dfot_dit_train_sync_weights(dfot_dit_train_t h, void* stream);
int dfot_dit_train_forward(dfot_dit_train_t h, const float* x, const int32_t* noise_levels, float* out, int batch, int tokens, void* stream);
int dfot_dit_train_forward_cond(dfot_dit_train_t h, const float* x, const int32_t* noise_levels, const float* cond, const int32_t* labels,
                                const uint8_t* cond_mask, float* out, int batch, int tokens, void* stream);
int dfot_dit_train_load_buffer(dfot_dit_train_t h, const char* name, const float* data, int64_t numel, void* stream);
int dfot_dit_train_forward_f(dfot_dit_train_t h, const float* x, const float* noise_levels, const float* cond, const int32_t* labels,
                             const uint8_t* cond_mask, float* out, int batch, int tokens, void* stream);
int dfot_dit_train_backward(dfot_dit_train_t h, const float* d_out, void* stream);
int dfot_dit_train_input_grad(dfot_dit_train_t h, float* dx, void* stream);
int dfot_vloss_grad(const float* x, const float* noise, const float* v, const float* a, const float* sigma, const float* coef, float* dv,
                    int batch, int tokens, int64_t frame_elems, int vspace, void* stream);
int dfot_sumsq(const float* x, int64_t n, float* out, void* stream);
int dfot_adamw_step(float* params, const float* grads, float* exp_avg, float* exp_avg_sq, int64_t n, float lr, float beta1, float beta2,
                    float eps, float weight_decay, int step, const float* grad_sumsq, float max_grad_norm, float* ema, float ema_decay,
                    void* stream);

int dfot_ray_encode(const float* raw_poses, float* out, int batch, int tokens, int resolution, void* stream);
int dfot_ray_encode_normalized(const float* poses, float* out, int batch, int tokens, int resolution, void* stream);

int dfot_hg_prepare(const float* x, const float* noise, const float* qa, const float* qb, float* x_in, int batch,
                    int nfe, int tokens, int64_t frame_elems, void* stream);
int dfot_ddim_compose(const float* x, const float* x_in, const float* v, const float* sa, const float* s1,
                      const float* an, const float* cn, const float* keep, const float* weight, const uint8_t* gen,
                      float* x_next, int batch, int nfe, int tokens, int64_t frame_elems, void* stream);

int dfot_ddim_compose_tokw(const float* x, const float* x_in, const float* v, const float* sa, const float* s1,
                           const float* an, const float* cn, const float* keep, const float* weight, const uint8_t* gen,
                           float* x_next, int batch, int nfe, int tokens, int64_t frame_elems, void* stream);

int dfot_ddim_noise(const float* noise, const float* sigma, const float* weight, const uint8_t* gen, float* x_next, int batch,
                    int nfe, int tokens, int64_t frame_elems, int weight_per_token, void* stream);

int dfot_vpred_loss(const float* x, const float* noise, const float* v, const float* alpha, const float* sigma,
                    const float* weight, float* x_pred, float* scratch, float* loss, int batch, int tokens,
                    int64_t frame_elems, void* stream);
int64_t dfot_vpred_loss_scratch_floats(int batch, int tokens, int64_t frame_elems);
int dfot_vspace_loss(const float* x, const float* noise, const float* v, const float* alpha, const float* sigma,
                     const float* weight, float* x_pred, float* scratch, float* loss, int batch, int tokens,
                     int64_t frame_elems, void* stream);

int dfot_op_gemm(const void* a_bf16, int lda, const void* w_bf16, const float* bias, float* c, int m, int n, int k,
                 int variant, void* stream);
int dfot_op_conv3x3(const void* a_bf16, const void* w_bf16, const float* bias, float* y, int bt, int h, int w,
                    int cin, int cout, int variant, void* stream);
typedef struct {
  int32_t amode, epi, variant;
  const void* A; int64_t lda;
  const void* W; int64_t ldw;
  int32_t M, N, K, H, Wd, Cin;
  const uint8_t* live;
  const float* bias; int32_t bias_rows;
  float* out_f32; void* out_bf16; int64_t ldo;
  const float* resid; const void* resid_bf;
  const float* gate; const int32_t* gate_index; int64_t ldg; int32_t gate_rows;
  int32_t act; void* pre_act; void* raw; int64_t ldraw; int32_t tr_rows;
  float* gn_part; int32_t gn_rows_per_bt, gn_cpg;
  void* out2; int64_t ldo2; int32_t split;
  void *q, *k, *v;
  const float *qw, *kw, *rope_cs;
  int32_t heads, d, ntok; float qscale; int32_t dstride; float eps;
  int32_t ksplit; int64_t slice_stride;
} dfot_gemm_desc;
int dfot_op_gemm_ex(const dfot_gemm_desc* desc, void* stream);
int64_t dfot_op_gemm_desc_bytes(void);
int dfot_op_attention(const void* q, const void* k, const void* v, void* o, int ldo, int batch, int heads, int n,
                      int d, int variant, void* stream);
int dfot_op_attention_padded(const void* q, const void* k, const void* v, void* o, int ldo, int batch, int heads, int n,
                             int d, void* stream);
int dfot_op_attention_temporal(const void* q, const void* k, const void* v, void* o, int ldo, int batch, int tokens, int patches,
                               int heads, int d, void* stream);
int dfot_op_matrix_attention_rope(const void* z, void* o, const float* rope_cs, int batch, int L, int E, int h, int cc, int rr,
                                  float scale, void* stream);
int dfot_op_matrix_attention(const void* z, void* o, int batch, int L, int E, int h, int cc, int rr, float scale, void* stream);
int dfot_op_attention_bwd(const void* q, const void* k, const void* v, const void* d_o, void* o, int ldo, void* dq, void* dk, void* dv,
                          int batch, int heads, int n, int d, void* stream);
int dfot_op_conv3x3_bwd(const void* x, const void* dy, const float* w, float* dx, float* dw, float* db, int bt, int h, int w_, int cin, int cout,
                        void* stream);
int dfot_op_conv3x3_bwd2(const void* x, const void* dy, const float* w, float* dx, void* dx_bf, float* dw, float* db, int bt, int h, int w_, int cin,
                         int cout, void* stream);
int dfot_op_gn_silu_bwd(const float* x, const float* dy, const float* gamma, const float* beta, const void* film, float eps, float* dx, void* dfilm,
                        float* dgamma, float* dbeta, int bt, int pixels, int channels, void* stream);
int dfot_op_rms_film_bwd(const float* x, const float* dxn, const float* w, const void* film, float eps, float* dx, void* dfilm, float* dw,
                         int64_t rows, int channels, int accumulate_dx, void* stream);
int dfot_op_rms_film_bwd_res(const float* x, const float* dxn, const float* w, const void* film, float eps, const float* dres, float* dx, void* dx_bf,
// ... 88 lines not shown
```

Baseline: 9.961.

## Share down-path conv results across guidance branches with identical frame inputs

Detects, per guidance/NFE branch, frames whose noise level, input and condition mask match an earlier branch, and skips the down-path res-block and downsample convolutions for them. After the down path, their activations are copied from the source frame. A per-image XCD tile remap spreads the remaining active images' conv tiles across XCDs. The cost is host-side pairing logic, a prepare kernel, and a copy kernel per forward. Correctness depends on the branches really having bit-identical inputs up to that point.

After: 9.956. About the same (-0.0%).

```diff
diff --git a/diffusion-forcing-transformer_amd/backbone.py b/diffusion-forcing-transformer_amd/backbone.py
--- a/diffusion-forcing-transformer_amd/backbone.py
+++ b/diffusion-forcing-transformer_amd/backbone.py
@@ -80,6 +80,8 @@
         self._trainer_sig = None
         self.live_frames = None
         self.fresh_frames = None
+        self.source_frames = None
+        self.active_images = None
         self._fresh_key = None
         self._train_stamp = 0
         self._dropout_generator: Optional[torch.Generator] = None
@@ -338,10 +340,19 @@
             capi.require_device(dev, fresh_frames=fresh)
             if key != self._fresh_key:
                 fresh = None
-        capi.check(capi.lib.dfot_uvit_forward_cached_masks(self._handle, capi.ptr(xf, torch.float32, "x"),
-                                                           capi.ptr(kf, torch.float32, "noise_levels"), capi.ptr(out), b,
-                                                           capi.ptr(live, torch.uint8, "live_frames"),
-                                                           capi.ptr(fresh, torch.uint8, "fresh_frames"), capi.stream_ptr()))
+        source, active = self.source_frames, 0
+        if source is not None:
+            if tuple(source.shape) != (b, self.temporal_length) or source.dtype != torch.int32 or not source.is_contiguous():
+                raise ValueError(f"source_frames must be a contiguous int32 tensor of shape {(b, self.temporal_length)}")
+            capi.require_device(dev, source_frames=source)
+            if self.active_images is None or len(self.active_images) != 2:
+                raise ValueError("source_frames needs active_images = (images to compute with fresh_frames honoured, without)")
+            active = int(self.active_images[0 if fresh is not None else 1])
+        capi.check(capi.lib.dfot_uvit_forward_cached_shared(self._handle, capi.ptr(xf, torch.float32, "x"),
+                                                            capi.ptr(kf, torch.float32, "noise_levels"), capi.ptr(out), b,
+                                                            capi.ptr(live, torch.uint8, "live_frames"),
+                                                            capi.ptr(fresh, torch.uint8, "fresh_frames"),
+                                                            capi.ptr(source, torch.int32, "source_frames"), active, capi.stream_ptr()))
         self._fresh_key = key
         return out.to(x.dtype)
 
diff --git a/diffusion-forcing-transformer_amd/capi.py b/diffusion-forcing-transformer_amd/capi.py
--- a/diffusion-forcing-transformer_amd/capi.py
+++ b/diffusion-forcing-transformer_amd/capi.py
@@ -87,6 +87,7 @@
     "dfot_uvit_forward_cached": (_I, [_P, _P, _P, _P, _I, _P]),
     "dfot_uvit_forward_cached_live": (_I, [_P, _P, _P, _P, _I, _P, _P]),
     "dfot_uvit_forward_cached_masks": (_I, [_P, _P, _P, _P, _I, _P, _P, _P]),
+    "dfot_uvit_forward_cached_shared": (_I, [_P, _P, _P, _P, _I, _P, _P, _P, _I, _P]),
     "dfot_uvit_read_tap": (_I, [_P, C.c_char_p, _P, C.c_size_t, _P]),
     "dfot_dit_create": (_I, [C.POINTER(DiTConfig), C.POINTER(_P)]),
     "dfot_dit_create_f": (_I, [C.POINTER(DiTConfigF), C.POINTER(_P)]),
diff --git a/diffusion-forcing-transformer_amd/csrc/common.h b/diffusion-forcing-transformer_amd/csrc/common.h
--- a/diffusion-forcing-transformer_amd/csrc/common.h
+++ b/diffusion-forcing-transformer_amd/csrc/common.h
@@ -22,6 +22,12 @@
   if (!enable) return orig;
   const int q = nwg >> 3, r = nwg & 7, xcd = orig & 7;
   return (xcd < r ? xcd * (q + 1) : r * (q + 1) + (xcd - r) * q) + (orig >> 3);
+}
+
+__device__ __forceinline__ int xcd_remap_images(int orig, int nwg, int tpi) {
+  if (tpi & 7) return xcd_remap(orig, nwg);
+  const int c = tpi >> 3, xcd = orig & 7, j = orig >> 3;
+  return (j / c) * tpi + xcd * c + j % c;
 }
 
 __device__ __forceinline__ float silu_f(float x) { return x * __builtin_amdgcn_rcpf(1.0f + __expf(-x)); }
diff --git a/diffusion-forcing-transformer_amd/csrc/gemm.h b/diffusion-forcing-transformer_amd/csrc/gemm.h
--- a/diffusion-forcing-transformer_amd/csrc/gemm.h
+++ b/diffusion-forcing-transformer_amd/csrc/gemm.h
@@ -46,6 +46,7 @@
   int dstride = 0;
   float eps = 1e-6f;
   int xcd = 1;
+  int img_spread = 0;
   int persist = 0;
   int ksplit = 1;
   long slice_stride = 0;
diff --git a/diffusion-forcing-transformer_amd/csrc/gemm.hip b/diffusion-forcing-transformer_amd/csrc/gemm.hip
--- a/diffusion-forcing-transformer_amd/csrc/gemm.hip
+++ b/diffusion-forcing-transformer_amd/csrc/gemm.hip
@@ -65,7 +65,10 @@
   const int tiles_n = (g.N + BN_T - 1) / BN_T;
   const int ksplit = (EPI == E_F32 && (AMODE == A_DENSE || g.slice_stride > 0) && g.ksplit > 1) ? g.ksplit : 1;
   const int kslice = ksplit > 1 ? tile_index % ksplit : 0;
-  const int bid = ksplit > 1 ? xcd_remap(tile_index / ksplit, tile_count / ksplit, g.xcd) : xcd_remap(tile_index, tile_count, g.xcd);
+  int bid = ksplit > 1 ? xcd_remap(tile_index / ksplit, tile_count / ksplit, g.xcd) : xcd_remap(tile_index, tile_count, g.xcd);
+  if constexpr (AMODE == A_CONV3) {
+    if (g.img_spread && ksplit == 1) bid = xcd_remap_images(tile_index, tile_count, (g.H * g.Wd / BM_T) * tiles_n);
+  }
   const int tn = bid % tiles_n, tm = bid / tiles_n;
   const int m0 = tm * BM_T, n0 = tn * BN_T;
   if constexpr (AMODE == A_CONV3) {
@@ -858,6 +861,7 @@
   DFOT_REQUIRE((epi == E_QKV || epi == E_QKV_DIT || g.ldo % (epi == E_F32 ? 4 : 8) == 0) && (epi != E_QKV || (g.ldo2 % 8 == 0 && g.split % 64 == 0)),
                DFOT_ERR_SHAPE, "gemm: output row strides must be multiples of %d", epi == E_F32 ? 4 : 8);
   DFOT_REQUIRE(g.ldw == 0 || (amode == A_DENSE && g.ldw >= g.K && g.ldw % 8 == 0), DFOT_ERR_SHAPE, "gemm: ldw=%ld must be >= K and a multiple of 8 (dense A only)", g.ldw);
+  DFOT_REQUIRE(!g.img_spread || (amode == A_CONV3 && g.live), DFOT_ERR_ARG, "gemm: the per-image tile order belongs to a convolution with image flags");
   if (amode == A_CONV3) {
     DFOT_REQUIRE(g.Cin % BK == 0 && g.K == 9 * g.Cin, DFOT_ERR_SHAPE, "conv3x3: Cin=%d must be a multiple of %d", g.Cin, BK);
     DFOT_REQUIRE(g.zeros != nullptr, DFOT_ERR_ARG, "conv3x3: zero page missing");
diff --git a/diffusion-forcing-transformer_amd/csrc/uvit.hip b/diffusion-forcing-transformer_amd/csrc/uvit.hip
--- a/diffusion-forcing-transformer_amd/csrc/uvit.hip
+++ b/diffusion-forcing-transformer_amd/csrc/uvit.hip
@@ -105,6 +105,8 @@
   int pend_lvl = 0, pend_c = 0, pend_slices = 2;
   long pend_m = 0;
   int last_batch = 0;
+  uint8_t* down_flags = nullptr;
+  int *share_pairs = nullptr, *share_count = nullptr;
   const float* xin[4] = {nullptr, nullptr, nullptr, nullptr};
   bf16* XB[4] = {nullptr, nullptr, nullptr, nullptr};
   bool xin_bf[4] = {false, false, false, false};
@@ -345,7 +347,7 @@
   if (i < n) o[i] = a[i] + b[i];
 }
 
-static int run_res_block(dfot_uvit_s* h, const ResW& w, int lvl, int bt, hipStream_t s, const uint8_t* live = nullptr) {
+static int run_res_block(dfot_uvit_s* h, const ResW& w, int lvl, int bt, hipStream_t s, const uint8_t* live = nullptr, bool spread = false) {
   const int c = w.c, rr = h->r[lvl], pix = rr * rr;
   const int m = bt * pix;
   const int slots = pix / 64;
@@ -364,7 +366,7 @@
   if ((rc = launch_gn_apply_silu_bf16in(xb, h->gn_stats, w.g1, w.be1, h->s1, bt, pix, c, s, live))) return rc;
   GemmArgs g;
   g.A = h->s1; g.W = w.w1; g.M = m; g.N = c; g.K = 9 * c; g.H = rr; g.Wd = rr; g.Cin = c; g.zeros = h->zeros;
-  g.bias = w.bias1; g.out_bf16 = h->hbf; g.ldo = c; g.live = live;
+  g.bias = w.bias1; g.out_bf16 = h->hbf; g.ldo = c; g.live = live; g.img_spread = live && spread;
   g.gn_part = h->gn_partial2; g.gn_rows_per_bt = pix; g.gn_cpg = c / 32;
   if ((rc = launch_gemm(A_CONV3, E_BF16, h->gemm_variant, g, s))) return rc;
   if ((rc = launch_gn_finalize(h->gn_partial2, h->gn_stats, bt, slots, pix, c, h->cfg.eps, s))) return rc;
@@ -373,7 +375,7 @@
     return rc;
   GemmArgs o;
   o.A = h->s1; o.W = w.w2; o.M = m; o.N = c; o.K = 9 * c; o.H = rr; o.Wd = rr; o.Cin = c; o.zeros = h->zeros;
-  o.bias = w.bias2; o.out_bf16 = xb; o.ldo = c; o.live = live;
+  o.bias = w.bias2; o.out_bf16 = xb; o.ldo = c; o.live = live; o.img_spread = live && spread;
   o.resid_bf = xb;
   o.gn_part = h->gn_partial; o.gn_rows_per_bt = pix; o.gn_cpg = c / 32;
   if ((rc = launch_gemm(A_CONV3, E_BF16, h->gemm_variant, o, s))) return rc;
@@ -507,7 +509,7 @@
   return launch_gemm(A_CONV3, E_F32, h->gemm_variant, g, s);
 }
 
-static int run_down(dfot_uvit_s* h, int l, int bt, hipStream_t s, const uint8_t* live = nullptr) {
+static int run_down(dfot_uvit_s* h, int l, int bt, hipStream_t s, const uint8_t* live = nullptr, bool spread = false) {
   const int rr = h->r[l], cin = h->ch[l], cout = h->ch[l + 1];
   int rc = 0;
   if ((rc = h->xin_bf[l] ? launch_pool2_bf16_bf16in(h->XB[l], h->s1, bt, rr, rr, cin, s) : launch_pool2_bf16(h->xin[l], h->s1, bt, rr, rr, cin, s)))
@@ -516,6 +518,7 @@
   g.A = h->s1; g.W = h->down_conv[l].w; g.M = bt * (rr / 2) * (rr / 2); g.N = cout; g.K = 9 * cin; g.H = rr / 2; g.Wd = rr / 2;
   g.Cin = cin; g.zeros = h->zeros; g.bias = h->down_conv[l].b; g.out_f32 = h->HSA[l]; g.ldo = cout;
   g.live = live;
+  g.img_spread = live && spread;
   const bool next_is_res = l + 1 < 2;
   if (next_is_res) {
     g.gn_part = h->gn_partial; g.gn_rows_per_bt = (rr / 2) * (rr / 2); g.gn_cpg = cout / 32;
@@ -545,6 +548,80 @@
     return DFOT_ERR_STATE;
   }
   return launch_upsample_add_bf16(h->tmp, h->XB[l], h->XB[l], bt, rr, rr, cout, s, live);
+}
+
+__global__ void shared_frames_prepare_kernel(const uint8_t* __restrict__ fresh, const uint8_t* __restrict__ live, const int* __restrict__ source,
+                                             int bt, uint8_t* __restrict__ down_flag, int* __restrict__ pairs, int* __restrict__ count) {
+  __shared__ int n;
+  if (threadIdx.x == 0) n = 0;
+  __syncthreads();
+  for (int i = threadIdx.x; i < bt; i += blockDim.x) {
+    const int src = source[i];
+    bool shared = src >= 0 && src < bt && src != i;
+    if (shared) {
+      const int up = source[src];
+      if (up >= 0 && up != src) shared = false;
+      if (fresh && !fresh[src] && (!live || live[i])) shared = false;
+    }
+    down_flag[i] = (!shared && (!fresh || fresh[i])) ? 1 : 0;
+    if (shared) {
+      const int k = atomicAdd(&n, 1);
+      pairs[2 * k] = i;
+      pairs[2 * k + 1] = src;
+    }
+  }
+  __syncthreads();
+  if (threadIdx.x == 0) *count = n;
+}
+
+struct SharedSegs {
+  void* p[4];
+  unsigned n16[4];
+};
+__global__ __launch_bounds__(256) void shared_frames_copy_kernel(SharedSegs sg, const int* __restrict__ pairs, const int* __restrict__ count, unsigned total16) {
+  typedef __attribute__((ext_vector_type(4))) unsigned u4;
+  const int n = *count;
+  const unsigned e0 = sg.n16[0], e1 = e0 + sg.n16[1], e2 = e1 + sg.n16[2];
+  for (int k = blockIdx.y; k < n; k += gridDim.y) {
+    const size_t dst = (size_t)pairs[2 * k], src = (size_t)pairs[2 * k + 1];
+    const u4* from[4];
+    u4* to[4];
+    u4 val[4];
+#pragma unroll
+    for (int j = 0; j < 4; ++j) {
+      const unsigned u = (blockIdx.x * 4 + j) * 256 + threadIdx.x;
+      from[j] = nullptr;
+      if (u >= total16) continue;
+      u4* base;
+      unsigned off, per;
+      if (u < e0) { base = (u4*)sg.p[0]; off = u; per = sg.n16[0]; }
+      else if (u < e1) { base = (u4*)sg.p[1]; off = u - e0; per = sg.n16[1]; }
+      else if (u < e2) { base = (u4*)sg.p[2]; off = u - e1; per = sg.n16[2]; }
+      else { base = (u4*)sg.p[3]; off = u - e2; per = sg.n16[3]; }
+      from[j] = base + src * per + off;
+      to[j] = base + dst * per + off;
+    }
+#pragma unroll
+    for (int j = 0; j < 4; ++j)
+      if (from[j]) val[j] = *from[j];
+#pragma unroll
+    for (int j = 0; j < 4; ++j)
+      if (from[j]) *to[j] = val[j];
+  }
+}
+
+static int copy_shared_frames(dfot_uvit_s* h, int bt, int active_images, hipStream_t s) {
+  SharedSegs sg;
+  sg.p[0] = h->XB[0]; sg.n16[0] = (unsigned)((size_t)h->r[0] * h->r[0] * h->ch[0] * sizeof(bf16) / 16);
+  sg.p[1] = h->HSA[0]; sg.n16[1] = (unsigned)((size_t)h->r[1] * h->r[1] * h->ch[1] * sizeof(float) / 16);
+  sg.p[2] = h->XB[1]; sg.n16[2] = (unsigned)((size_t)h->r[1] * h->r[1] * h->ch[1] * sizeof(bf16) / 16);
+  sg.p[3] = h->HSA[1]; sg.n16[3] = (unsigned)((size_t)h->r[2] * h->r[2] * h->ch[2] * sizeof(float) / 16);
+  const unsigned total16 = sg.n16[0] + sg.n16[1] + sg.n16[2] + sg.n16[3];
+  const int idle = bt - active_images;
+  hipLaunchKernelGGL(shared_frames_copy_kernel, dim3(cdiv((long)total16, 1024), idle > 0 ? idle : 1), dim3(256), 0, s, sg, h->share_pairs, h->share_count,
+                     total16);
+  DFOT_CHECK_HIP(hipGetLastError());
+  return DFOT_OK;
 }
 
 }
@@ -716,6 +793,9 @@
     DFOT_CHECK_HIP(hipMemcpy(h->film_table, table.data(), table.size() * sizeof(FilmChunk), hipMemcpyHostToDevice));
     h->film_chunks = (int)table.size();
     if ((rc = dev_alloc(h, &h->cond_mask, (size_t)max_batch, true))) return rc;
+    if ((rc = dev_alloc(h, &h->down_flags, bt, true))) return rc;
+    if ((rc = dev_alloc(h, &h->share_pairs, 2 * bt, true))) return rc;
+    if ((rc = dev_alloc(h, &h->share_count, 1, true))) return rc;
     h->cond_batch = 0;
   }
   if ((rc = dev_alloc(h, &h->cat, mc * 5, true))) return rc;
@@ -844,7 +924,14 @@
 
 int dfot_uvit_forward_cached_masks(dfot_uvit_t h, const float* x, const float* noise_levels, float* out, int batch, const uint8_t* live_frames,
                                    const uint8_t* fresh_frames, void* stream) {
+  return dfot_uvit_forward_cached_shared(h, x, noise_levels, out, batch, live_frames, fresh_frames, nullptr, 0, stream);
+}
+
+int dfot_uvit_forward_cached_shared(dfot_uvit_t h, const float* x, const float* noise_levels, float* out, int batch, const uint8_t* live_frames,
+                                    const uint8_t* fresh_frames, const int32_t* source_frames, int active_images, void* stream) {
   DFOT_REQUIRE(h && x && noise_levels && out, DFOT_ERR_ARG, "forward: null argument");
+  DFOT_REQUIRE(!source_frames || (batch > 0 && active_images > 0 && active_images <= batch * h->T), DFOT_ERR_ARG,
+               "forward: %d active images of %d (shared frames need the number of images that run the down path)", active_images, batch * h->T);
   DFOT_REQUIRE(!fresh_frames || h->last_batch == batch, DFOT_ERR_STATE,
                "forward: frozen frames need the previous forward of this handle to have run the same batch (%d, now %d)", h->last_batch, batch);
   DFOT_REQUIRE(!fresh_frames || live_frames, DFOT_ERR_ARG, "forward: frozen frames must also be dead frames (live_frames is null)");
@@ -865,12 +952,24 @@
   h->xin_bf[0] = true;
   h->xin_bf[1] = h->xin_bf[2] = h->xin_bf[3] = false;
 
-  if (fresh_frames && (h->gemm_variant != GEMM_AUTO || (h->r[2] * h->r[2]) % 512 != 0)) fresh_frames = nullptr;
+  if (h->gemm_variant != GEMM_AUTO || (h->r[2] * h->r[2]) % 512 != 0) {
+    fresh_frames = nullptr;
+    source_frames = nullptr;
+  }
+  const uint8_t* down = fresh_frames;
+  const bool spread = source_frames != nullptr;
+  if (source_frames) {
+    hipLaunchKernelGGL(shared_frames_prepare_kernel, dim3(1), dim3(256), 0, s, fresh_frames, live_frames, source_frames, bt, h->down_flags, h->share_pairs,
+                       h->share_count);
+    DFOT_CHECK_HIP(hipGetLastError());
+    down = h->down_flags;
+  }
   for (int l = 0; l < 2; ++l) {
     for (const ResW& w : h->down_res[l])
-      if ((rc = run_res_block(h, w, l, bt, s, fresh_frames))) return rc;
-    if ((rc = run_down(h, l, bt, s, fresh_frames))) return rc;
-  }
+      if ((rc = run_res_block(h, w, l, bt, s, down, spread))) return rc;
+    if ((rc = run_down(h, l, bt, s, down, spread))) return rc;
+  }
+  if (source_frames && (rc = copy_shared_frames(h, bt, active_images, s))) return rc;
   h->pend_bias = nullptr;
   for (const TrW& w : h->down_tr)
     if ((rc = run_tr_block(h, w, 2, batch, s))) return rc;
diff --git a/diffusion-forcing-transformer_amd/sampler.py b/diffusion-forcing-transformer_amd/sampler.py
--- a/diffusion-forcing-transformer_amd/sampler.py
+++ b/diffusion-forcing-transformer_amd/sampler.py
@@ -59,6 +59,7 @@
         self.dry_run = False
         self.use_graph = True
         self.skip_frozen_frames = True
+        self.skip_shared_frames = True
         self.skip_dead_frames = True
         self.graph_replays = 0
         self.graph_captures = 0
@@ -308,6 +309,7 @@
                     parallel.branch_group(n_)
                     split_nfe.add(n_)
         if self.dry_run:
+            self.trace[-1]["plans"] = plans
             for p_ in plans:
                 if p_["nfe"] in split_nfe:
                     hb = parallel.world_info()[1] % p_["nfe"]
@@ -371,11 +373,24 @@
                     p_["cond"] = by_mask[key]
             finally:
                 self._interpolate_masked_poses = False
-        fresh_dev = torch.from_numpy(np.concatenate([a.ravel() for a in self._fresh_flags(plans, batch_size, horizon)])).cuda()
+        fresh_host = self._fresh_flags(plans, batch_size, horizon)
+        fresh_dev = torch.from_numpy(np.concatenate([a.ravel() for a in fresh_host])).cuda()
         foff = 0
-        for p_ in plans:
+        for p_, fr in zip(plans, fresh_host):
+            p_["fresh"] = fr
             p_["fresh_dev"] = fresh_dev[foff:foff + p_["bm"] * horizon].view(p_["bm"], horizon)
             foff += p_["bm"] * horizon
+        skip_shared = self.skip_shared_frames and hasattr(self.model, "source_frames")
+        shared = self._source_frames(plans, batch_size, horizon) if skip_shared else []
+        if any((a >= 0).any() for a in shared):
+            source_dev = torch.from_numpy(np.concatenate([a.ravel() for a in shared])).cuda()
+            soff = 0
+            for p_, a in zip(plans, shared):
+                p_["source_dev"] = source_dev[soff:soff + a.size].view(p_["bm"], horizon)
+                soff += a.size
+                p_["active"] = (int(((a < 0) & (p_["fresh"] != 0)).sum()), int((a < 0).sum()))
+        else:
+            skip_shared = False
         xs = xs.contiguous()
         s = capi.stream_ptr
         branch_cache: Dict[tuple, tuple] = {}
@@ -383,7 +398,7 @@
         skip_dead = self.skip_dead_frames and hasattr(self.model, "live_frames")
         skip_frozen = skip_dead and self.skip_frozen_frames and hasattr(self.model, "fresh_frames")
 
-        def step(p_, xs, noise, tables, gen_dev, xs_next=None, live_dev=None, fresh_dev=None):
+        def step(p_, xs, noise, tables, gen_dev, xs_next=None, live_dev=None, fresh_dev=None, source_dev=None, active=None):
             nonlocal cond_rep, cond_nfe
             nfe, bm = p_["nfe"], p_["bm"]
             x_in = torch.empty(bm, horizon, *x_shape, device="cuda", dtype=torch.float32)
@@ -421,6 +436,9 @@
                     self.model.live_frames = live_dev if live_dev is not None else p_["live_dev"]
                 if skip_frozen:
                     self.model.fresh_frames = fresh_dev if fresh_dev is not None else p_["fresh_dev"]
+                if skip_shared:
+                    self.model.source_frames = source_dev if source_dev is not None else p_["source_dev"]
+                    self.model.active_images = active if active is not None else p_["active"]
                 try:
                     v = self.model(x_in, lvl, cond_rep, p_["cmask_dev"])
                 finally:
@@ -428,6 +446,8 @@
                         self.model.live_frames = None
                     if skip_frozen:
                         self.model.fresh_frames = None
+                    if skip_shared:
+                        self.model.source_frames = self.model.active_images = None
             step_noise = None
             if strict or p_["sigma"] is not None:
                 step_noise = self.noise_fn("ddim", (bm, horizon, *x_shape))
@@ -532,6 +552,30 @@
             prev = p_
         return out
 
+    @staticmethod
+    def _source_frames(plans, batch_size: int, horizon: int):
+        out = []
+        for p_ in plans:
+            bm, nfe = p_["bm"], p_["nfe"]
+            src = np.full((bm, horizon), -1, np.int32)
+            if not p_.get("renoise") and nfe > 1 and "cond" not in p_:
+                qa, qb, lvl, cm = p_["tables"][0], p_["tables"][1], p_["tables"][7], p_["cmask"]
+                frames = np.arange(horizon, dtype=np.int32)
+                for b in range(batch_size):
+                    for j in range(1, nfe):
+                        r = b * nfe + j
+                        for j0 in range(j):
+                            r0 = b * nfe + j0
+                            if cm is not None and cm[r] != cm[r0]:
+                                continue
+                            same = ((qb[r] == 0) & (qb[r0] == 0) & (qa[r] == qa[r0]) & (lvl[r] == lvl[r0]) & (src[r] < 0) & (src[r0] < 0))
+                            src[r] = np.where(same, r0 * horizon + frames, src[r])
+            flat = src.ravel()
+            if not (flat[flat[flat >= 0]] < 0).all():
+                raise RuntimeError("a shared frame's source has a source of its own")
+            out.append(src)
+        return out
+
     def _run_steps_graph(self, plans, xs, draw_noise, step, flat_dev, gens_dev, horizon):
         p0 = plans[0]
         bm, n_steps, nfe = p0["bm"], len(plans), p0["nfe"]
@@ -544,14 +588,16 @@
             self._graphs.clear()
             self._graphs_generation = gen
         cond_src = p0.get("cond_src")
+        sharing = "source_dev" in p0
         key = (bm, n_steps, nfe, horizon, tuple(xs.shape), need_noise, None if p0["cmask"] is None else p0["cmask"].tobytes(),
-               id(self.model), None if cond_src is None else (tuple(cond_src.shape), cond_src.dtype))
+               id(self.model), None if cond_src is None else (tuple(cond_src.shape), cond_src.dtype), sharing)
         ent = self._graphs.get(key)
         if ent is None:
             ent = dict(tables=torch.empty(n_steps, 8, bm, horizon, device="cuda", dtype=torch.float32),
                        gens=torch.empty_like(gens_dev), weights=torch.empty_like(p0["weights_dev"]),
                        lives=torch.empty(n_steps, bm, horizon, device="cuda", dtype=torch.uint8),
                        fresh=torch.empty(n_steps, bm, horizon, device="cuda", dtype=torch.uint8),
+                       source=torch.empty(n_steps, bm, horizon, device="cuda", dtype=torch.int32) if sharing else None,
                        noise=torch.empty(n_steps, bm, *xs.shape[1:], device="cuda") if need_noise else None,
                        xs=torch.empty_like(xs), out=None, graph=None,
                        cond=None if cond_src is None else torch.empty_like(cond_src))
@@ -559,6 +605,9 @@
         ent["gens"].copy_(gens_dev)
         ent["lives"].copy_(gens_dev if nfe == 1 else gens_dev.repeat_interleave(nfe, dim=1))
         ent["fresh"].copy_(torch.stack([p_["fresh_dev"] for p_ in plans]))
+        if sharing:
+            ent["source"].copy_(torch.stack([p_["source_dev"] for p_ in plans]))
+        src = lambda i: ent["source"][i] if sharing else None
         ent["weights"].copy_(p0["weights_dev"])
         if need_noise:
             for i, p_ in enumerate(plans):
@@ -571,7 +620,7 @@
             ent["cond"].copy_(cond_src)
             p_static["cond"] = ent["cond"]
         ent["xs"].copy_(step(p_static, xs, None if not need_noise else ent["noise"][0], ent["tables"][0], ent["gens"][0], live_dev=ent["lives"][0],
-                            fresh_dev=ent["fresh"][0]))
+                            fresh_dev=ent["fresh"][0], source_dev=src(0), active=plans[0].get("active")))
         if ent["graph"] is None:
             torch.cuda.synchronize()
             graph = torch.cuda.CUDAGraph()
@@ -579,7 +628,7 @@
                 x = ent["xs"]
                 for i in range(1, n_steps):
                     x = step(p_static, x, ent["noise"][i] if need_noise else None, ent["tables"][i], ent["gens"][i], live_dev=ent["lives"][i],
-                             fresh_dev=ent["fresh"][i])
+                             fresh_dev=ent["fresh"][i], source_dev=src(i), active=plans[i].get("active"))
                 ent["out"] = x
             ent["graph"] = graph
             if len(self._graphs) >= 4:
diff --git a/include/dfot_hip.h b/include/dfot_hip.h
--- a/include/dfot_hip.h
+++ b/include/dfot_hip.h
@@ -61,6 +61,9 @@
                                   const uint8_t* live_frames, void* stream);
 int dfot_uvit_forward_cached_masks(dfot_uvit_t h, const float* x, const float* noise_levels, float* out, int batch,
                                    const uint8_t* live_frames, const uint8_t* fresh_frames, void* stream);
+int dfot_uvit_forward_cached_shared(dfot_uvit_t h, const float* x, const float* noise_levels, float* out, int batch,
+                                    const uint8_t* live_frames, const uint8_t* fresh_frames, const int32_t* source_frames,
+                                    int active_images, void* stream);
 int dfot_uvit_read_tap(dfot_uvit_t h, const char* name, float* out, size_t capacity_floats, void* stream);
 
 typedef struct dfot_dit_s* dfot_dit_t;
```
